# Ericonaldo/ILSwiss

Hardware: AMD Instinct MI355X
Metric: env-steps/s + SAC grad-steps/s, Hopper-v2 4096 envs (higher is better)
Workload: dtype f32

## Files before the change

### ilswiss_amd/csrc/fwd_split_tile.inc

```
  constexpr bool FINS = FIN_CT > 0;
  constexpr int NTH = 4 * H / CS, NWV = NTH / 64, NC = H / 16, SLW = H / CS, NCS = SLW / 16;
  constexpr int NT0 = PH == 1 ? 1 : CS;
  constexpr int LDH = H + ILSX_LDS_PAD, LDSL = SLW + ILSX_LDS_PAD;
  constexpr int MT = 1;
  constexpr int MR = 16;
  static_assert(NCS == NWV, "one k16 chunk of the slice per wave in the head phase");
  const DevScalars* scal = GRP ? GP->scal : A.scal;
  const NetView& N = T.net;
  int KP = N.KP;
  if constexpr (FINS) XCH_PIN(KP);
  const int LDX = KP + ILSX_LDS_PAD, NO = N.NO, NCH0 = KP >> 4, NOT = (NO + 15) >> 4;
  float* xs = smem;
  float* h0 = xs + MR * LDX;
  float* hs = h0 + MR * LDH;
  float* red = hs + MR * LDSL;
  constexpr int RNT = 4;
  if (bx & ((1u << A.xs) - 1u)) return;
  if ((int)(bx >> A.xs) * (A.rt > 0 ? A.rt : 1) * MR >= A.rows) return;
  const int tid = threadIdx.x, lane = tid & 63, wave = tid >> 6, li = lane & 15, g = lane >> 4;
  const int rows = A.rows;
  const int RT = A.rt > 0 ? A.rt : 1;
  const bool lead = cs == 0;
  ILSX_STAMP(A.dbg, 0);

  const int ct0 = PH == 1 ? cs * NWV + wave : wave * CS;
  const float* w0p = N.base + N.off_W[0] + (size_t)ct0 * NCH0 * 256 + 4 * lane;
  constexpr int L0D = 8;
  float4 b0[NT0], b0first[NT0];
  float4 l0first[PH == 1 ? L0D : 1];
  float bias0[NT0];
  if constexpr (PH == 1) {
#pragma unroll
    for (int d = 0; d < L0D; ++d) l0first[d] = *reinterpret_cast<const float4*>(w0p + (size_t)(d < NCH0 ? d : 0) * 256);
  }
  if constexpr (PH != 2) {
#pragma unroll
    for (int i = 0; i < NT0; ++i) b0[i] = *reinterpret_cast<const float4*>(w0p + (size_t)i * NCH0 * 256);
#pragma unroll
    for (int i = 0; i < NT0; ++i) b0first[i] = b0[i];
#pragma unroll
    for (int i = 0; i < NT0; ++i) bias0[i] = (N.base + N.off_b[0])[(ct0 + i) * 16 + li];
  }
  const int lc = wave * 16 + li, col1 = cs * SLW + lc;
  float bias1 = 0.0f;
  float4 whf[4];
  float4 wreg[NC];
  constexpr bool LATEW = GRP == 3 && PH == 0;
  if constexpr (PH != 1) {
    bias1 = (N.base + N.off_b[1])[col1];
#pragma unroll
    for (int t = 0; t < 4; ++t) {
      const int j = 16 * t + li;
      whf[t] = (t < NOT && j < NO) ? *reinterpret_cast<const float4*>(N.base + N.off_Wh + (size_t)j * H + cs * SLW + 16 * wave + 4 * g)
                                   : make_float4(0.f, 0.f, 0.f, 0.f);
    }
    if constexpr (!LATEW) {
      const float* wp = N.base + N.off_W[1] + (size_t)(cs * NWV + wave) * NC * 256 + 4 * lane;
#pragma unroll
      for (int c = 0; c < NC; ++c) wreg[c] = *reinterpret_cast<const float4*>(wp + 256 * c);
    }
  }
#ifdef XCH_FINE_DBG
  ILSX_STAMP_SYNC(XCH_FINE_DBG, 6);
#endif
  const bool fin = FIN_CT >= 0 && (GRP ? GP->fin_on : A.fin_on) != 0 && !T.no_fin && T.d1 > 0;
  const GatherSpec& G = GRP ? GP->gather : A.gather;
  for (int rt = 0; rt < RT; ++rt) {
  const int r0 = ((bx >> A.xs) * RT + rt) * MR;
  if (r0 >= rows) break;
  const bool full_tile = r0 + MR <= rows;
  bool fin_logp = false;
  int sf_a = 0; float* sf_logp = nullptr;
  if constexpr (PH != 2) {
#pragma unroll
  for (int i = 0; i < NT0; ++i) b0[i] = b0first[i];
  if constexpr (FINS) {
    static_assert(PH == 0 && GRP == 0 && XCH, "the static epilogue is phase A's target-critic stage");
    const PolicyFinishArgs& FP = A.fin;
    const bool pub = lead && first_task;
    int sf_d0 = T.d0, sf_s0 = T.s0, sf_ps = FP.part_stride;
    const float* sf_x0 = T.x0; const float* sf_part = FP.part; float* sf_xsave = lead ? T.xsave : nullptr;
    float* sf_raw = pub ? FP.raw : nullptr; float* sf_action = pub ? FP.action : nullptr; float* sf_epss = pub ? FP.eps_save : nullptr;
    sf_a = FP.a; sf_logp = pub ? FP.logp : nullptr;
    XCH_PIN(sf_d0); XCH_PIN(sf_s0); XCH_PIN(sf_ps); XCH_PIN(sf_x0); XCH_PIN(sf_part); XCH_PIN(sf_xsave);
    XCH_PIN(sf_raw); XCH_PIN(sf_action); XCH_PIN(sf_epss); XCH_PIN(sf_a); XCH_PIN(sf_logp);
    const int a = sf_a, NOp = 2 * a;
    const int fr = tid / a, fj = tid - fr * a, fgr = r0 + fr;
    const bool fon = tid < MR * a && fgr < rows;
    float fep = 0.0f;
    if (fon) {
      const unsigned long long fstep = FP.scal ? (FP.use_gather_step ? FP.scal->gather_step : FP.scal->step) : FP.step_host;
      float z4[4];
      philox_normal4(FP.seed, fstep, FP.rng_stream, fgr, fj >> 2, z4);
      const int q = fj & 3;
      fep = q == 0 ? z4[0] : q == 1 ? z4[1] : q == 2 ? z4[2] : z4[3];
    }
    constexpr int STG = 2;
    int sr[STG], sk[STG];
#pragma unroll
    for (int t = 0; t < STG; ++t) { const int e = tid + t * NTH; sr[t] = e / KP; sk[t] = e - sr[t] * KP; }
    XCH_HOOK_STAGE
    {
      float sv[STG];
#pragma unroll
      for (int t = 0; t < STG; ++t) {
        const int gr = r0 + sr[t];
        sv[t] = (tid + t * NTH < MR * KP && gr < rows && sk[t] < sf_d0) ? xg<true>(sf_x0)[(size_t)gr * sf_s0 + sk[t]] : 0.0f;
      }
      float pm[4], pl[4];
#pragma unroll
      for (int c = 0; c < 4; ++c) {
        const size_t at = ((size_t)(c < CS ? c : 0) * sf_ps + (fon ? fgr : r0)) * NOp + fj;
        pm[c] = fon ? ldx<XCH>(xg<true>(sf_part + at)) : 0.0f;
        pl[c] = fon ? ldx<XCH>(xg<true>(sf_part + at + a)) : 0.0f;
      }
#pragma unroll
      for (int t = 0; t < STG; ++t) {
        const int gr = r0 + sr[t];
        const bool act_col = sk[t] >= sf_d0 && sk[t] < sf_d0 + a;
        if (tid + t * NTH < MR * KP && !act_col) {
          if (sf_xsave && gr < rows) xg<true>(sf_xsave)[(size_t)gr * KP + sk[t]] = sv[t];
          xs[sr[t] * LDX + sk[t]] = sv[t];
        }
      }
      for (int e = tid + STG * NTH; e < MR * KP; e += NTH) {
        const int r = e / KP, k = e - r * KP, gr = r0 + r;
        if (k >= sf_d0 && k < sf_d0 + a) continue;
        float v = 0.0f;
        if (gr < rows) {
          if (k < sf_d0) v = xg<true>(sf_x0)[(size_t)gr * sf_s0 + k];
          if (sf_xsave) xg<true>(sf_xsave)[(size_t)gr * KP + k] = v;
        }
        xs[r * LDX + k] = v;
      }
      float* lp3 = red;
      float act = 0.0f, c0 = 0.0f, c1 = 0.0f, c2 = 0.0f;
      if (fon) {
        float mu = 0.f, lsr = 0.f;
#pragma unroll
        for (int c = 0; c < 4; ++c) { mu += c < CS ? pm[c] : 0.0f; lsr += c < CS ? pl[c] : 0.0f; }
        const float ls = fminf(fmaxf(lsr, LOG_SIG_MIN), LOG_SIG_MAX);
        const float sd = expf(ls);
        const float z = fep * sd + mu;
        act = tanhf(z);
        const float dm = mu - z;
        c0 = dm * dm / expf(2.0f * ls); c1 = ls; c2 = logf(1.0f - act * act + TANH_EPS);
        if (sf_raw) { stx<XCH>(xg<true>(sf_raw + (size_t)fgr * NOp + fj), mu); stx<XCH>(xg<true>(sf_raw + (size_t)fgr * NOp + a + fj), lsr); }
        if (sf_xsave) xg<true>(sf_xsave)[(size_t)fgr * KP + sf_d0 + fj] = act;
        if (sf_action) stx<XCH>(xg<true>(sf_action + (size_t)fgr * a + fj), act);
        if (sf_epss) stx<XCH>(xg<true>(sf_epss + (size_t)fgr * a + fj), fep);
      }
      if (tid < MR * a) {
        xs[fr * LDX + sf_d0 + fj] = act;
        lp3[(fr * 32 + fj) * 3 + 0] = c0; lp3[(fr * 32 + fj) * 3 + 1] = c1; lp3[(fr * 32 + fj) * 3 + 2] = c2;
      }
      fin_logp = sf_logp != nullptr;
    }
  } else {
  XCH_HOOK_STAGE
  if constexpr (PH == 0) {
    long long* ridx0 = reinterpret_cast<long long*>(hs);
    if constexpr (GRP != 0) {
      if (G.on) {
        if (tid < MR) ridx0[tid] = r0 + tid < rows ? replay_draw(G.seed, scal->gather_step, G.stream, (uint32_t)(r0 + tid), G.st->size) : 0;
        lds_barrier();
      }
    }
    for (int e = tid; e < MR * KP; e += NTH) {
      const int r = e / KP, k = e - r * KP, gr = r0 + r;
      const bool act_col = k >= T.d0 && k < T.d0 + T.d1;
      if (fin && act_col) continue;
      float v = 0.0f;
      if (gr < rows) {
        if (G.on) {
          long long idx;
          if constexpr (GRP != 0) idx = ridx0[r];
          else idx = replay_draw(G.seed, scal->gather_step, G.stream, (uint32_t)gr, G.st->size);
          const float* rec = G.records + (size_t)idx * G.rec;
          if (k < T.d0) v = rec[T.g0_off + k];
          else if (act_col) v = rec[T.g1_off + (k - T.d0)];
          if (lead && T.publish == 1) {
            if (k < T.d0) G.s[(size_t)gr * G.o + k] = v;
            else if (act_col) G.a[(size_t)gr * G.adim + (k - T.d0)] = v;
            if (k == 0) { stx<XCH>(G.r + gr, rec[G.o + G.adim]); stx<XCH>(G.d + gr, rec[G.o + G.adim + 1]); }
          } else if (lead && T.publish == 2 && k < T.d0) {
            G.s2[(size_t)gr * G.o + k] = v;
          }
        } else {
          if (k < T.d0) v = T.x0[(size_t)gr * T.s0 + k];
          else if (act_col) v = T.x1[(size_t)gr * T.s1 + (k - T.d0)];
        }
        if (T.xsave && lead) T.xsave[(size_t)gr * KP + k] = v;
      }
      xs[r * LDX + k] = v;
    }
  } else {
    auto stage = [&](int r, int k, int gr, const float* rec) {
      const bool act_col = k >= T.d0 && k < T.d0 + T.d1;
      if (fin && act_col) return;
      float v = 0.0f;
      if (gr < rows) {
        if (G.on) {
          if (k < T.d0) v = rec[T.g0_off + k];
          else if (act_col) v = rec[T.g1_off + (k - T.d0)];
          if (lead && T.publish == 1) {
            if (k < T.d0) G.s[(size_t)gr * G.o + k] = v;
            else if (act_col) G.a[(size_t)gr * G.adim + (k - T.d0)] = v;
            if (k == 0) { G.r[gr] = rec[G.o + G.adim]; G.d[gr] = rec[G.o + G.adim + 1]; }
          } else if (lead && T.publish == 2 && k < T.d0) {
            G.s2[(size_t)gr * G.o + k] = v;
          }
        } else {
          if (k < T.d0) v = T.x0[(size_t)gr * T.s0 + k];
          else if (act_col) v = T.x1[(size_t)gr * T.s1 + (k - T.d0)];
        }
        if (T.xsave && lead) T.xsave[(size_t)gr * KP + k] = v;
      }
      xs[r * LDX + k] = v;
    };
    long long* ridx = reinterpret_cast<long long*>(hs);
    if (G.on) {
      if (tid < MR) ridx[tid] = r0 + tid < rows ? replay_draw(G.seed, scal->gather_step, G.stream, (uint32_t)(r0 + tid), G.st->size) : 0;
      lds_barrier();
    }
    if (KP <= 512 && T.d1 <= 64) {
      constexpr int RW = 16 / NWV, U = 8;
      const bool acts = T.d1 > 0 && !fin;
#pragma unroll
      for (int mt = 0; mt < MT; ++mt) {
      float vo[RW][U], va[RW];
#pragma unroll
      for (int rr = 0; rr < RW; ++rr) {
        const int r = 16 * mt + wave + NWV * rr, grc = r0 + r < rows ? r0 + r : rows - 1;
        const float* rec = G.on ? G.records + (size_t)ridx[r] * G.rec : nullptr;
        const float* s0p = G.on ? rec + T.g0_off : T.x0 + (size_t)grc * T.s0;
#pragma unroll
        for (int u = 0; u < U; ++u) { const int k = lane + 64 * u; vo[rr][u] = s0p[k < T.d0 ? k : T.d0 - 1]; }
        va[rr] = 0.0f;
        if (acts) { const float* s1p = G.on ? rec + T.g1_off : T.x1 + (size_t)grc * T.s1; va[rr] = s1p[lane < T.d1 ? lane : T.d1 - 1]; }
      }
#pragma unroll
      for (int rr = 0; rr < RW; ++rr) {
        const int r = 16 * mt + wave + NWV * rr, gr = r0 + r;
// ... 65 lines not shown
            const int q = j & 3;
            ep = q == 0 ? z4[0] : q == 1 ? z4[1] : q == 2 ? z4[2] : z4[3];
          }
        }
        if (det) {
          act = P.max_act * (P.head == HEAD_DET_LIN_NOISE ? mu : tanhf(mu));
          if (P.noise != 0.0f) act += fminf(fmaxf(P.noise * ep, -P.noise_clip), P.noise_clip);
          if (pub && P.raw) stx<XCH>(P.raw + (size_t)gr * a + j, mu);
        } else {
          const float ls = fminf(fmaxf(lsr, LOG_SIG_MIN), LOG_SIG_MAX);
          const float sd = expf(ls);
          const float z = ep * sd + mu;
          act = tanhf(z);
          const float dm = mu - z;
          c0 = dm * dm / expf(2.0f * ls); c1 = ls; c2 = logf(1.0f - act * act + TANH_EPS);
          if (pub && P.raw) { stx<XCH>(P.raw + (size_t)gr * NOp + j, mu); stx<XCH>(P.raw + (size_t)gr * NOp + a + j, lsr); }
        }
        if (T.xsave && lead) T.xsave[(size_t)gr * KP + T.d0 + j] = act;
        if (pub) {
          if (P.action) stx<XCH>(P.action + (size_t)gr * a + j, act);
          if (P.eps_save) stx<XCH>(P.eps_save + (size_t)gr * a + j, ep);
        }
      }
      xs[row * LDX + T.d0 + j] = act;
      lp3[(row * LPS + j) * 3 + 0] = c0; lp3[(row * LPS + j) * 3 + 1] = c1; lp3[(row * LPS + j) * 3 + 2] = c2;
    }
    fin_logp = pub && P.logp && !det;
  }
  }
  }
  else {
    const float* hsrc = T.hsave[0];
    for (int e = tid; e < MR * (H / 4); e += NTH) {
      const int row = e / (H / 4), c4 = e - row * (H / 4), gr = r0 + row;
      const float4 v = gr < rows ? *reinterpret_cast<const float4*>(hsrc + (size_t)gr * H + 4 * c4) : make_float4(0.f, 0.f, 0.f, 0.f);
      *reinterpret_cast<float4*>(h0 + row * LDH + 4 * c4) = v;
    }
  }
  lds_barrier();
  XCH_STAMP(1);
  if (fin_logp && tid < MR && r0 + tid < rows) {
    const PolicyFinishArgs& P = GRP ? GP->fin : A.fin;
    float q = 0.f, l = 0.f, jc = 0.f;
    const int pa = FINS ? sf_a : P.a;
    constexpr int LPS = 32;
    for (int j = 0; j < pa; ++j) { q += red[(tid * LPS + j) * 3]; l += red[(tid * LPS + j) * 3 + 1]; jc += red[(tid * LPS + j) * 3 + 2]; }
    stx<XCH>(xg<FINS>((FINS ? sf_logp : P.logp) + r0 + tid), -0.5f * q - (l + HALF_LOG_2PI) - jc);
  }
  if constexpr (PH == 1) {
    f32x4 acc = (f32x4){0.f, 0.f, 0.f, 0.f};
    const float* ap = xs + li * LDX + 4 * g;
    float4 cur[L0D], nxt[L0D];
#pragma unroll
    for (int d = 0; d < L0D; ++d) cur[d] = l0first[d];
    for (int cb = 0; cb < NCH0; cb += L0D) {
#pragma unroll
      for (int d = 0; d < L0D; ++d) {
        const int c = cb + L0D + d;
        nxt[d] = *reinterpret_cast<const float4*>(w0p + (size_t)(c < NCH0 ? c : 0) * 256);
      }
#pragma unroll
      for (int d = 0; d < L0D; ++d) {
        if (cb + d < NCH0) {
          const float4 a = *reinterpret_cast<const float4*>(ap + 16 * (cb + d));
          acc = MFMA16(a.x, cur[d].x, acc); acc = MFMA16(a.y, cur[d].y, acc);
          acc = MFMA16(a.z, cur[d].z, acc); acc = MFMA16(a.w, cur[d].w, acc);
        }
      }
#pragma unroll
      for (int d = 0; d < L0D; ++d) cur[d] = nxt[d];
    }
    float* hsv = T.hsave[0];
    const int col = ct0 * 16 + li;
#pragma unroll
    for (int v = 0; v < 4; ++v) {
      const int row = 4 * g + v;
      if (r0 + row < rows) hsv[(size_t)(r0 + row) * H + col] = act_fn<ACT>(acc[v] + bias0[0]);
    }
  } else if constexpr (PH != 2) {
    f32x4 acc[NT0];
#pragma unroll
    for (int i = 0; i < NT0; ++i) acc[i] = (f32x4){0.f, 0.f, 0.f, 0.f};
    const float* ap = xs + li * LDX + 4 * g;
    for (int kc = 0; kc < KP; kc += 16) {
      float4 bn[NT0];
#pragma unroll
      for (int i = 0; i < NT0; ++i) {
        bn[i] = b0[i];
        if (kc + 16 < KP) bn[i] = *reinterpret_cast<const float4*>(w0p + (size_t)i * NCH0 * 256 + (kc + 16) * 16);
      }
      const float4 a = *reinterpret_cast<const float4*>(ap + kc);
#pragma unroll
      for (int i = 0; i < NT0; ++i) acc[i] = MFMA16(a.x, b0[i].x, acc[i]);
#pragma unroll
      for (int i = 0; i < NT0; ++i) acc[i] = MFMA16(a.y, b0[i].y, acc[i]);
#pragma unroll
      for (int i = 0; i < NT0; ++i) acc[i] = MFMA16(a.z, b0[i].z, acc[i]);
#pragma unroll
      for (int i = 0; i < NT0; ++i) acc[i] = MFMA16(a.w, b0[i].w, acc[i]);
#pragma unroll
      for (int i = 0; i < NT0; ++i) b0[i] = bn[i];
    }
    float* hsv = (PH == 1 || lead) ? T.hsave[0] : nullptr;
    float* const hrow = hsv ? hsv + (size_t)(r0 + 4 * g) * H + ct0 * 16 + li : nullptr;
#pragma unroll
    for (int i = 0; i < NT0; ++i) {
      const int col = (ct0 + i) * 16 + li;
#pragma unroll
      for (int v = 0; v < 4; ++v) {
        const int row = 4 * g + v;
        const float h = act_fn<ACT>(acc[i][v] + bias0[i]);
        if constexpr (PH == 0) h0[row * LDH + col] = h;
        acc[i][v] = h;
      }
    }
    if (hsv) {
      if (full_tile) {
#pragma unroll
        for (int i = 0; i < NT0; ++i)
#pragma unroll
          for (int v = 0; v < 4; ++v) stx<XCH>(hrow + v * H + i * 16, acc[i][v]);
      } else {
#pragma unroll
        for (int i = 0; i < NT0; ++i)
#pragma unroll
          for (int v = 0; v < 4; ++v)
            if (r0 + 4 * g + v < rows) stx<XCH>(hrow + v * H + i * 16, acc[i][v]);
      }
    }
  }
  if constexpr (PH == 1) {
    lds_barrier();
    continue;
  }
  if constexpr (PH == 0) lds_barrier();
  XCH_STAMP(2);
  if constexpr (LATEW) {
    const float* wp = N.base + N.off_W[1] + (size_t)(cs * NWV + wave) * NC * 256 + 4 * lane;
#pragma unroll
    for (int c = 0; c < NC; ++c) wreg[c] = *reinterpret_cast<const float4*>(wp + 256 * c);
  }
  {
    f32x4 acc0[MT], acc1[MT];
#pragma unroll
    for (int m = 0; m < MT; ++m) { acc0[m] = (f32x4){0.f, 0.f, 0.f, 0.f}; acc1[m] = acc0[m]; }
    const float* ap = h0 + li * LDH + 4 * g;
#pragma unroll
    for (int c = 0; c < NC; ++c) {
#pragma unroll
      for (int m = 0; m < MT; ++m) {
        const float4 a = *reinterpret_cast<const float4*>(ap + m * 16 * LDH + 16 * c);
        acc0[m] = MFMA16(a.x, wreg[c].x, acc0[m]); acc1[m] = MFMA16(a.y, wreg[c].y, acc1[m]);
        acc0[m] = MFMA16(a.z, wreg[c].z, acc0[m]); acc1[m] = MFMA16(a.w, wreg[c].w, acc1[m]);
      }
    }
    float* hsv = T.hsave[1];
#pragma unroll
    for (int m = 0; m < MT; ++m) {
      float* const hrow = hsv ? hsv + (size_t)(r0 + 16 * m + 4 * g) * H + col1 : nullptr;
#pragma unroll
      for (int v = 0; v < 4; ++v) {
        const int row = 16 * m + 4 * g + v;
        const float h = act_fn<ACT>(acc0[m][v] + acc1[m][v] + bias1);
        hs[row * LDSL + lc] = h;
        acc0[m][v] = h;
      }
      if (hsv) {
        if (full_tile) {
#pragma unroll
          for (int v = 0; v < 4; ++v) stx<XCH>(hrow + v * H, acc0[m][v]);
        } else {
#pragma unroll
          for (int v = 0; v < 4; ++v)
            if (r0 + 16 * m + 4 * g + v < rows) stx<XCH>(hrow + v * H, acc0[m][v]);
        }
      }
    }
  }
  lds_barrier();
  XCH_STAMP(3);
#pragma unroll
  for (int m = 0; m < MT; ++m) {
    const float4 a = *reinterpret_cast<const float4*>(hs + (16 * m + li) * LDSL + 16 * wave + 4 * g);
#pragma unroll
    for (int t = 0; t < 4; ++t) {
      if (t < NOT) {
        f32x4 acc = (f32x4){0.f, 0.f, 0.f, 0.f};
        acc = MFMA16(a.x, whf[t].x, acc); acc = MFMA16(a.y, whf[t].y, acc);
        acc = MFMA16(a.z, whf[t].z, acc); acc = MFMA16(a.w, whf[t].w, acc);
#pragma unroll
        for (int v = 0; v < 4; ++v) red[(((m * RNT + t) * NWV + wave) * 4 + v) * 64 + lane] = acc[v];
      }
    }
  }
  lds_barrier();
  const float* bh = N.base + N.off_bh;
#pragma unroll
  for (int m = 0; m < MT; ++m)
  for (int e = tid; e < NOT * 256; e += NTH) {
    const int t = e >> 8, v = (e >> 6) & 3, ol = e & 63;
    float sum = 0.0f;
#pragma unroll
    for (int w2 = 0; w2 < NWV; ++w2) sum += red[(((m * RNT + t) * NWV + w2) * 4 + v) * 64 + ol];
    const int row = 16 * m + 4 * (ol >> 4) + v, j = 16 * t + (ol & 15), gr = r0 + row;
    if (j < NO && gr < rows) stx<XCH>(T.part + ((size_t)cs * A.part_stride + gr) * NO + j, sum + (lead ? bh[j] : 0.0f));
  }
  lds_barrier();
  }
  ILSX_STAMP(A.dbg, 7);
```

### ilswiss_amd/csrc/host_common.h

```cpp
#pragma once
#include <hip/hip_runtime.h>
#include <hip/hip_ext.h>

#include <cstdarg>
#include <cstdio>
#include <cstring>
#include <deque>
#include <string>
#include <utility>
#include <vector>

#include "../../include/ilsx.h"
#include "dev_owner.h"
#include "kernels.h"

#define ILSX_FAIL(code, ...)   \
  do {                         \
    ilsx_set_err(__VA_ARGS__); \
    return (code);             \
  } while (0)

#define HIPCHK(expr)                                                                              \
  do {                                                                                            \
    hipError_t e_ = (expr);                                                                       \
// ... 33 lines not shown
  bool prof_on = false;
  struct ProfRec { int kid; hipEvent_t a, b; };
  std::vector<ProfRec> prof_pending;
  std::vector<hipEvent_t> prof_free;
  double prof_ms[ILSX_K_COUNT] = {0};
  uint64_t prof_n[ILSX_K_COUNT] = {0};
  const char* prof_name[ILSX_K_COUNT] = {nullptr};
};

struct ProfScope {
  ilsx_ctx* c; int kid; hipEvent_t a = nullptr, b = nullptr; bool launched = false;
  ProfScope(ilsx_ctx* ctx, int k);
  ~ProfScope();
};
#define ILSX_LAUNCH(ps, kernel, grid, block, lds, stream, ...)                                            \
  do {                                                                                                    \
    if ((ps).a) {                                                                                         \
      (ps).c->prof_name[(ps).kid] = #kernel; (ps).launched = true;                                        \
      hipExtLaunchKernelGGL(kernel, grid, block, lds, stream, (ps).a, (ps).b, 0, __VA_ARGS__);            \
    } else {                                                                                              \
      hipLaunchKernelGGL(kernel, grid, block, lds, stream, __VA_ARGS__);                                  \
    }                                                                                                     \
  } while (0)

int comm_allreduce_sum(ilsx_ctx* c, float* buf, size_t n);
int ctx_stage(ilsx_ctx* c, size_t bytes, void** out);

struct NetLayout {
  ilsx_mlp_cfg cfg;
  int KP = 0, NO = 0;
  int off_W[ILSX_MAX_HID], off_Wb[ILSX_MAX_HID], off_b[ILSX_MAX_HID], ld[ILSX_MAX_HID];
  int off_Wh = 0, off_bh = 0;
  size_t n_int = 0;
  size_t n_flat = 0;
  int hl[ILSX_MAX_HID] = {0, 0, 0};
  int out_of(int l) const { return hl[l] > 0 ? hl[l] : cfg.hidden; }
  int in_of(int l) const { return l == 0 ? cfg.in_dim : out_of(l - 1); }
};
int net_layout_build(const ilsx_mlp_cfg& cfg, NetLayout* L);
void net_flat_to_internal(const NetLayout& L, const float* flat, float* internal);
void net_internal_to_flat(const NetLayout& L, const float* internal, float* flat);
NetView net_view(const NetLayout& L, float* base);

struct ilsx_net {
  ilsx_ctx* ctx = nullptr;
  NetLayout lay;
  float* base = nullptr;
  bool owns = true;
  float* ws_out = nullptr;
  int ws_rows = 0;
  bool noise_policy = false;
  float noise = 0.f, noise_clip = 0.f, max_act = 1.f;
  bool out_linear = false;
  bool categorical = false;
  bool egreedy = false;
  float epsilon = 0.f;
  bool discrete() const { return categorical || egreedy; }
};
int launch_categorical_act(ilsx_ctx* ctx, const float* z, int rows, int n, int deterministic, unsigned long long step, float* act, float* logp);
int launch_egreedy_act(ilsx_ctx* ctx, const float* z, int rows, int n, int deterministic, float epsilon, unsigned long long step, float* act);

int net_adopt(ilsx_net* n, float* arena);
void net_give_back(ilsx_net* n);

int net_upload_flat(ilsx_ctx* ctx, const NetLayout& L, float* dev_base, const float* src, size_t n, int src_is_device);
int net_download_flat(ilsx_ctx* ctx, const NetLayout& L, const float* dev_base, float* dst, size_t n, int dst_is_device);

int launch_fwd(ilsx_ctx* ctx, const FwdArgs& A, int H, int act, int KP, int cs = 1);
int launch_bwd_dx(ilsx_ctx* ctx, const BwdArgs& A, int H, int act, int cs = 1);
int launch_policy_finish(ilsx_ctx* ctx, const PolicyFinishArgs& P);
bool phase_fits(ilsx_ctx* ctx, int rows, int H, int cs, int ntasks, bool own_rows = false);
bool phase_own_rows(ilsx_ctx* ctx, int rows, int H, int cs, int ntasks);
struct PhaseConst {
  int slot = -1, device = 0;
  bool tried = false, valid_a = false, valid_c = false;
  unsigned long long key_a = 0, key_c = 0;
  PhaseAArgs a; PhaseCArgs c;
};
int phase_const_alloc(int device);
void phase_const_prepare(ilsx_ctx* ctx, PhaseConst* ct);
void phase_const_free(int device, int slot);
bool phase_a_static_ok(const PhaseAArgs& P, int H, int cs);
bool phase_c_static_ok(const PhaseCArgs& P, int H, int cs);
int launch_phase_a(ilsx_ctx* ctx, const PhaseAArgs& P, int H, int act, int KPmax, int cs, PhaseConst* ct = nullptr, unsigned long long key = 0, bool upload_only = false);
int launch_phase_c(ilsx_ctx* ctx, const PhaseCArgs& P, int H, int act, int KPmax, int cs, PhaseConst* ct = nullptr, unsigned long long key = 0, bool upload_only = false);
int device_cus(ilsx_ctx* ctx);
int grp_const_alloc(int device, bool fwd, int n, int* base);
void grp_const_free(int device, bool fwd, int base);
int grp_const_upload(ilsx_ctx* ctx, bool fwd, int base, const void* host_records, size_t count);
struct ilsx_sac;
int sac_staged_batch(ilsx_sac* s, int B, float** obs, float** act, float** rew, float** done, float** nobs);
int sac_step_staged(ilsx_sac* s, ilsx_sac_stats* stats);
int sac_dims(const ilsx_sac* s, int* o, int* a);
int sac_window_begin(ilsx_sac* s, int B);
int sac_window_step(ilsx_sac* s);
int sac_window_end(ilsx_sac* s, bool teardown = false);
#define ILSX_RETRY_WINDOW (-1000)
int sac_snapshot_take(ilsx_sac* s);
int sac_snapshot_restore(ilsx_sac* s);
bool sac_window_may_use_phase(ilsx_sac* s, int B);
int mlp2_split_factor(int n_hidden, int H);
int launch_bwd_dw(ilsx_ctx* ctx, DevOwner& owner, const DwArgs& table, int rows, const AdamFuse* fuse = nullptr);
int dw_table_add(DwArgs* T, const float* A, int lda, int NA, const float* Bm, int ldb, int NB, float* dW, float* dWb, int ldw,
                 float* db, int mode, int rows = 0, int bias_rows = 0);
int launch_adam(ilsx_ctx* ctx, const AdamArgs& A);
int build_dw_jobs(const NetLayout& L, float* gbase, const float* xsave, float* const* hsave,
                  float* const* dsave, const float* dhead, DwArgs* table);

struct ilsx_replay {
  ilsx_ctx* ctx = nullptr;
  int64_t cap = 0;
  int o = 0, a = 0, rec = 0;
  float* data = nullptr;
  DevReplayState* dstate = nullptr;
  bool dstate_stale = false;
  uint64_t seed = 0;
  uint32_t rng_stream = 0;
  unsigned long long sample_ctr = 0;
  int64_t top = 0, size = 0, cur_start = 0;
  std::deque<std::pair<int64_t, int64_t>> trajs;
  std::vector<uint8_t> start_flag;
};
int replay_flush_state(ilsx_replay* rb);
int replay_advance_device_rows(ilsx_replay* rb, int n);
int replay_insert_paths(ilsx_replay* rb, const float* stage, int stage_len, const int* envs, const int* lens, const uint8_t* last_terminal,
                        int n_paths);
int replay_launch_sample(ilsx_replay* rb, int B, const int64_t* idx, const DevScalars* scal,
                         unsigned long long step_host, float* obs, float* act, float* rew, float* done,
                         float* nobs, int64_t* idx_out);
```

### ilswiss_amd/csrc/ilsx_core.hip

```cpp
#include <algorithm>
#include <cmath>
#include <cstdlib>
#include <random>

#define ILSX_KERNEL_IMPL 1
#include <mutex>
#include "host_common.h"

static thread_local std::string g_err = "";

void ilsx_set_err(const char* fmt, ...) {
  char buf[1024];
  va_list ap;
  va_start(ap, fmt);
  vsnprintf(buf, sizeof buf, fmt, ap);
  va_end(ap);
  g_err = buf;
}

static int kernels_init_once();
extern "C" int ilsx_abi_version(void) { return ILSX_ABI_VERSION; }
extern "C" const char* ilsx_last_error(void) { return g_err.c_str(); }

int ctx_alloc(ilsx_ctx* c, size_t bytes, void** out, bool zero) {
// ... 382 lines not shown
  if (cs > 1) {
    const size_t lds = fwd_split_lds_bytes(H, KPmax, cs);
    if (lds > 160 * 1024) ILSX_FAIL(ILSX_ERR_UNSUPPORTED, "forward tile needs %zu B of LDS (> 160 KiB)", lds);
    A.xs = ctx->xcd_shift;
    if (A.rt <= 0) A.rt = (A.tasks && ctx->rt_grouped > 0) ? ctx->rt_grouped : ctx->rt_single;
    const int tiles = (A.rows + 15) / 16;
    dim3 grid(((((tiles + A.rt - 1) / A.rt) + 7) & ~7) << A.xs, A.ntasks, cs), block(4 * H / cs);
    if (A.tail_mode) { if (!A.tail || A.tail_n < 1 || A.tail_n > (int)(grid.x * grid.z)) ILSX_FAIL(ILSX_ERR_ARG, "deferred tail: bad record table"); grid.y += 1; }
    if (A.late < 0) A.late = (long)tiles * A.ntasks * cs > 2L * device_cus(ctx);
    if (H == 256 && cs == 4 && A.l0_split) {
      FwdArgs A2 = A;
      A2.tail_mode = 0; A2.tail = nullptr; A2.tail_n = 0; A2.dbg = ctx->dbg_next();
      dim3 grid2(grid.x, A.ntasks, cs);
#define L0_CALL(AA, GG) do { ILSX_LAUNCH(ps, (k_mlp2_fwd_split<256, AA, 4, GG, 1>), grid, block, lds, ctx->stream, A); \
                             ILSX_LAUNCH(ps, (k_mlp2_fwd_split<256, AA, 4, GG, 2>), grid2, block, lds, ctx->stream, A2); } while (0)
      const int gg = A.tasks ? (A.ctab ? 2 : 1) : 0;
      if (act == ILSX_ACT_RELU) { if (gg == 2) L0_CALL(ACT_RELU, 2); else if (gg == 1) L0_CALL(ACT_RELU, 1); else L0_CALL(ACT_RELU, 0); }
      else { if (gg == 2) L0_CALL(ACT_TANH, 2); else if (gg == 1) L0_CALL(ACT_TANH, 1); else L0_CALL(ACT_TANH, 0); }
#undef L0_CALL
    } else if (H == 256 && cs == 4) {
#define FWD_GRP_CALL(HH, AA, CC) do { if (A.tasks && A.ctab && A.late) ILSX_LAUNCH(ps, (k_mlp2_fwd_split<HH, AA, CC, 3>), grid, block, lds, ctx->stream, A); \
        else if (A.tasks && A.ctab) ILSX_LAUNCH(ps, (k_mlp2_fwd_split<HH, AA, CC, 2>), grid, block, lds, ctx->stream, A); \
        else if (A.tasks) ILSX_LAUNCH(ps, (k_mlp2_fwd_split<HH, AA, CC, 1>), grid, block, lds, ctx->stream, A); \
        else ILSX_LAUNCH(ps, (k_mlp2_fwd_split<HH, AA, CC, 0>), grid, block, lds, ctx->stream, A); } while (0)
      if (act == ILSX_ACT_RELU) FWD_GRP_CALL(256, ACT_RELU, 4); else FWD_GRP_CALL(256, ACT_TANH, 4);
    } else if (H == 128 && cs == 2) {
      if (act == ILSX_ACT_RELU) FWD_GRP_CALL(128, ACT_RELU, 2); else FWD_GRP_CALL(128, ACT_TANH, 2);
#undef FWD_GRP_CALL
    } else {
      ILSX_FAIL(ILSX_ERR_UNSUPPORTED, "no column-split forward kernel for H=%d cs=%d", H, cs);
    }
    HIPCHK(hipGetLastError());
    return ILSX_OK;
  }
  const size_t lds = fwd_lds_bytes(H, KPmax);
  if (lds > 160 * 1024) ILSX_FAIL(ILSX_ERR_UNSUPPORTED, "forward tile needs %zu B of LDS (> 160 KiB)", lds);
  dim3 grid((A.rows + 15) / 16, A.ntasks), block(4 * H);
#define CALL_FWD(HH, AA) ILSX_LAUNCH(ps, (k_mlp_fwd<HH, AA>), grid, block, lds, ctx->stream, A)
  DISPATCH_H_ACT(H, act, CALL_FWD);
#undef CALL_FWD
  HIPCHK(hipGetLastError());
  return ILSX_OK;
}

int device_cus(ilsx_ctx* ctx) {
  static int n_cu = 0;
  if (!n_cu) {
    hipDeviceProp_t pr;
    n_cu = hipGetDeviceProperties(&pr, ctx->device) == hipSuccess ? pr.multiProcessorCount : 1;
  }
  return n_cu;
}
static size_t phase_lds_bytes(int H, int KP, int cs) { return std::max(fwd_split_lds_bytes(H, KP, cs), bwd_split_lds_bytes(H, cs)); }
void phase_wgs_per_cu(int H, int cs, int* occ_a, int* occ_c) {
  static int oa[2] = {-1, -1}, oc[2] = {-1, -1};
  const int i = H == 256 ? 0 : 1;
  if (oa[i] < 0) {
    int a = 0, c = 0;
    const size_t lds = phase_lds_bytes(H, 32, cs);
    hipError_t e1, e2;
    if (H == 256) { e1 = hipOccupancyMaxActiveBlocksPerMultiprocessor(&a, (const void*)k_sac_phase_a<256, ACT_RELU, 4>, 4 * H / cs, lds);
                    e2 = hipOccupancyMaxActiveBlocksPerMultiprocessor(&c, (const void*)k_sac_phase_c<256, ACT_RELU, 4>, 4 * H / cs, lds); }
    else { e1 = hipOccupancyMaxActiveBlocksPerMultiprocessor(&a, (const void*)k_sac_phase_a<128, ACT_RELU, 2>, 4 * H / cs, lds);
           e2 = hipOccupancyMaxActiveBlocksPerMultiprocessor(&c, (const void*)k_sac_phase_c<128, ACT_RELU, 2>, 4 * H / cs, lds); }
    oa[i] = e1 == hipSuccess ? std::max(a, 1) : 1;
    oc[i] = e2 == hipSuccess ? std::max(c, 1) : 1;
  }
  *occ_a = oa[i]; *occ_c = oc[i];
}
bool phase_fits(ilsx_ctx* ctx, int rows, int H, int cs, int ntasks, bool own_rows) {
  const int n_cu = device_cus(ctx);
  if (!((H == 256 && cs == 4) || (H == 128 && cs == 2))) return false;
  const int tiles = (rows + 15) / 16, work = tiles * ntasks * cs;
  int occ_a = 1, occ_c = 1;
  phase_wgs_per_cu(H, cs, &occ_a, &occ_c);
  const int work_a = work + (own_rows ? tiles * 2 * cs : 0);
  return tiles <= PHASE_MAX_TILES && work <= n_cu && work_a + 1 <= occ_a * n_cu && tiles * 3 * cs <= occ_c * n_cu;
}
bool phase_own_rows(ilsx_ctx* ctx, int rows, int H, int cs, int ntasks) {
  const char* e = getenv("ILSX_PHASE_OWN_ROWS");
  return !(e && atoi(e) == 0) && phase_fits(ctx, rows, H, cs, ntasks, true);
}

static std::vector<bool> g_phase_slots[16];
static std::mutex g_phase_slots_mu;
int phase_const_alloc(int device) {
  static const bool off = []() { const char* e = getenv("ILSX_PHASE_CT"); return e && atoi(e) == 0; }();
  if (off || device < 0 || device >= 16) return -1;
  std::lock_guard<std::mutex> lock(g_phase_slots_mu);
  auto& u = g_phase_slots[device];
  if (u.empty()) u.assign(PHASE_CONST_SLOTS, false);
  for (int i = 0; i < PHASE_CONST_SLOTS; ++i) if (!u[i]) { u[i] = true; return i; }
  return -1;
}
void phase_const_free(int device, int slot) {
  if (device < 0 || device >= 16 || slot < 0 || slot >= PHASE_CONST_SLOTS) return;
  std::lock_guard<std::mutex> lock(g_phase_slots_mu);
  if (!g_phase_slots[device].empty()) g_phase_slots[device][slot] = false;
}
void phase_const_prepare(ilsx_ctx* ctx, PhaseConst* ct) {
  if (!ct || ct->tried) return;
  ct->tried = true;
  ct->device = ctx->device;
  ct->slot = phase_const_alloc(ctx->device);
  if (ct->slot >= 0) ctx->phase_slots.push_back(ct->slot);
}
template <class Blk>
static bool phase_const_ready(ilsx_ctx* ctx, PhaseConst* ct, const Blk& blk, unsigned long long key, Blk& held, bool& valid, unsigned long long& held_key,
                              const void* symbol) {
  phase_const_prepare(ctx, ct);
  if (!ct || ct->slot < 0 || blk.dbg || !key) return false;
  if (valid && held_key == key) return true;
  hipStreamCaptureStatus cap = hipStreamCaptureStatusNone;
  if (hipStreamIsCapturing(ctx->stream, &cap) != hipSuccess || cap != hipStreamCaptureStatusNone) return false;
  if (hipStreamSynchronize(ctx->stream) != hipSuccess) return false;
  valid = false;
  memcpy(&held, &blk, sizeof blk);
  if (hipMemcpyToSymbolAsync(symbol, &held, sizeof blk, (size_t)ct->slot * sizeof blk, hipMemcpyHostToDevice, ctx->stream) != hipSuccess ||
      hipStreamSynchronize(ctx->stream) != hipSuccess) { (void)hipGetLastError(); return false; }
  valid = true; held_key = key;
  return true;
}

bool phase_a_static_ok(const PhaseAArgs& P, int H, int cs) {
  const int nth = 4 * H / cs;
  for (int i = 0; i < 2; ++i) {
    const BwdTask& t = P.b1.t[i];
    if (t.loss != LOSS_SAC_CRITIC || t.net.NO != 1 || t.q.cs != cs || t.tq1.cs != cs || t.tq2.cs != cs) return false;
  }
  if (P.f1.fin_on) return false;
  const FwdArgs& f = P.f2;
  if (f.gather.on || !f.fin_on || f.fin.head != HEAD_TANH_SAMPLE || f.fin.cs != cs || f.fin.a < 1 || 16 * f.fin.a > nth) return false;
  if (f.fin.scal && !f.fin.use_gather_step) return false;
  if (f.fin.eps || P.fin_pi.eps) return false;
  for (int i = 0; i < 2; ++i) {
    const FwdTask& t = f.t[i];
    if (t.no_fin || t.d1 != f.fin.a || !t.x0) return false;
  }
  return true;
}
bool phase_c_static_ok(const PhaseCArgs& P, int H, int cs) {
  (void)H;
  if (P.f3.fin_on) return false;
  for (int i = 0; i < 2; ++i) {
    const BwdTask& t = P.b2.t[i];
    if (t.loss != LOSS_SAC_ACTORQ || t.net.NO != 1 || t.q1n.cs != cs || t.q2n.cs != cs) return false;
  }
  const BwdTask& t = P.b3.t[0];
  return t.loss == LOSS_SAC_POLICY && t.net.NO >= 2 && t.net.NO % 2 == 0 && P.b3.ga_parts == cs;
}
extern "C" int ilsx_debug_phase_static_ok(int stage, int loss_critic, int loss_policy, int no_critic, int slabs, int fin_head, int a, int H, int cs, int flags) {
  if (stage == 0) {
    PhaseAArgs P; memset(&P, 0, sizeof P);
    static const float x = 0.0f;
    for (int i = 0; i < 2; ++i) {
      BwdTask& t = P.b1.t[i];
      t.loss = loss_critic; t.net.NO = no_critic; t.q.cs = t.tq1.cs = t.tq2.cs = slabs;
      P.f2.t[i].d1 = a; P.f2.t[i].x0 = &x;
    }
    P.f2.fin_on = 1; P.f2.fin.head = fin_head; P.f2.fin.cs = slabs; P.f2.fin.a = a;
    if (flags & 1) P.f2.fin.eps = &x;
    return phase_a_static_ok(P, H, cs) ? 1 : 0;
  }
  PhaseCArgs P; memset(&P, 0, sizeof P);
  for (int i = 0; i < 2; ++i) { BwdTask& t = P.b2.t[i]; t.loss = loss_critic; t.net.NO = no_critic; t.q1n.cs = t.q2n.cs = slabs; }
  P.b3.t[0].loss = loss_policy; P.b3.t[0].net.NO = 2 * a; P.b3.ga_parts = slabs;
  if (flags & 2) P.f3.fin_on = 1;
  return phase_c_static_ok(P, H, cs) ? 1 : 0;
}

int launch_phase_a(ilsx_ctx* ctx, const PhaseAArgs& P0, int H, int act, int KPmax, int cs, PhaseConst* ct, unsigned long long key, bool upload_only) {
  PhaseAArgs P = P0;
  P.f1.xs = P.f2.xs = P.b1.xs = 0; P.f1.rt = P.f2.rt = 1;
  P.f1.dbg = P.f2.dbg = nullptr; P.b1.dbg = nullptr;
  P.dbg = upload_only ? nullptr : ctx->dbg_next();
  if (P.b1.ga_parts < 1) P.b1.ga_parts = 1;
  if (!phase_a_static_ok(P, H, cs)) ILSX_FAIL(ILSX_ERR_UNSUPPORTED, "launch_phase_a: the stages' descriptors are not what the phase kernel is compiled for (loss kind, head, slab count)");
  const int tiles = (P.f1.rows + 15) / 16;
  dim3 grid((tiles + 7) & ~7, P.own_rows ? 7 : 5, cs), block(4 * H / cs);
  const size_t lds = phase_lds_bytes(H, KPmax, cs);
  const bool use_ct = ct && phase_const_ready(ctx, ct, P, key, ct->a, ct->valid_a, ct->key_a, HIP_SYMBOL(g_phase_a_tab));
  if (upload_only) return ILSX_OK;
  const int slot = use_ct ? ct->slot : 0;
  static const bool trace = getenv("ILSX_PHASE_CT_TRACE") != nullptr;
  if (trace) { hipStreamCaptureStatus cap = hipStreamCaptureStatusNone; hipStreamIsCapturing(ctx->stream, &cap);
               fprintf(stderr, "launch_phase_a: %s, slot %d, capturing %d\n", use_ct ? "constant table" : "kernel arguments", ct ? ct->slot : -9, (int)cap); }
  ProfScope ps(ctx, ILSX_K_SAC_PHASE_A);
#define PHASE_A(HH, AA, CC) do { if (use_ct) ILSX_LAUNCH(ps, (k_sac_phase_a<HH, AA, CC, true>), grid, block, lds, ctx->stream, P, slot); \
                                 else ILSX_LAUNCH(ps, (k_sac_phase_a<HH, AA, CC>), grid, block, lds, ctx->stream, P, slot); } while (0)
  if (H == 256 && act == ILSX_ACT_RELU) PHASE_A(256, ACT_RELU, 4);
  else if (H == 256) PHASE_A(256, ACT_TANH, 4);
  else if (act == ILSX_ACT_RELU) PHASE_A(128, ACT_RELU, 2);
  else PHASE_A(128, ACT_TANH, 2);
#undef PHASE_A
  HIPCHK(hipGetLastError());
  return ILSX_OK;
}

int launch_phase_c(ilsx_ctx* ctx, const PhaseCArgs& P0, int H, int act, int KPmax, int cs, PhaseConst* ct, unsigned long long key, bool upload_only) {
  PhaseCArgs P = P0;
  P.f3.xs = P.b2.xs = P.b3.xs = 0; P.f3.rt = 1;
  P.f3.dbg = nullptr; P.b2.dbg = P.b3.dbg = nullptr;
  P.dbg = upload_only ? nullptr : ctx->dbg_next();
  if (P.b2.ga_parts < 1) P.b2.ga_parts = 1;
  if (P.b3.ga_parts < 1) P.b3.ga_parts = 1;
  if (!phase_c_static_ok(P, H, cs)) ILSX_FAIL(ILSX_ERR_UNSUPPORTED, "launch_phase_c: the stages' descriptors are not what the phase kernel is compiled for (loss kind, head, slab count)");
  const int tiles = (P.f3.rows + 15) / 16;
  dim3 grid((tiles + 7) & ~7, 4, cs), block(4 * H / cs);
  const size_t lds = phase_lds_bytes(H, KPmax, cs);
  const bool use_ct = ct && phase_const_ready(ctx, ct, P, key, ct->c, ct->valid_c, ct->key_c, HIP_SYMBOL(g_phase_c_tab));
  if (upload_only) return ILSX_OK;
  const int slot = use_ct ? ct->slot : 0;
  ProfScope ps(ctx, ILSX_K_SAC_PHASE_C);
#define PHASE_C(HH, AA, CC) do { if (use_ct) ILSX_LAUNCH(ps, (k_sac_phase_c<HH, AA, CC, true>), grid, block, lds, ctx->stream, P, slot); \
                                 else ILSX_LAUNCH(ps, (k_sac_phase_c<HH, AA, CC>), grid, block, lds, ctx->stream, P, slot); } while (0)
  if (H == 256 && act == ILSX_ACT_RELU) PHASE_C(256, ACT_RELU, 4);
  else if (H == 256) PHASE_C(256, ACT_TANH, 4);
  else if (act == ILSX_ACT_RELU) PHASE_C(128, ACT_RELU, 2);
  else PHASE_C(128, ACT_TANH, 2);
#undef PHASE_C
  HIPCHK(hipGetLastError());
  return ILSX_OK;
}

int launch_bwd_dx(ilsx_ctx* ctx, const BwdArgs& A0, int H, int act, int cs) {
  if (A0.rows <= 0) return ILSX_OK;
  BwdArgs A = A0;
  A.dbg = ctx->dbg_next();
  if (A.ga_parts < 1) A.ga_parts = 1;
  ProfScope ps(ctx, ILSX_K_MLP_BWD_DX);
  if (cs > 1) {
    const size_t lds = bwd_split_lds_bytes(H, cs);
    A.xs = ctx->xcd_shift;
    dim3 grid(((((A.rows + 15) / 16) + 7) & ~7) << A.xs, A.ntasks, cs), block(4 * H / cs);
    if (A.late < 0) A.late = (long)((A.rows + 15) / 16) * A.ntasks * cs > 2L * device_cus(ctx);
    if (H == 256 && cs == 4) {
#define BWD_GRP_CALL(HH, AA, CC) do { if (A.tasks && A.ctab && A.late) ILSX_LAUNCH(ps, (k_mlp2_bwd_split<HH, AA, CC, 3>), grid, block, lds, ctx->stream, A); \
        else if (A.tasks && A.ctab) ILSX_LAUNCH(ps, (k_mlp2_bwd_split<HH, AA, CC, 2>), grid, block, lds, ctx->stream, A); \
        else if (A.tasks) ILSX_LAUNCH(ps, (k_mlp2_bwd_split<HH, AA, CC, 1>), grid, block, lds, ctx->stream, A); \
        else ILSX_LAUNCH(ps, (k_mlp2_bwd_split<HH, AA, CC, 0>), grid, block, lds, ctx->stream, A); } while (0)
      if (act == ILSX_ACT_RELU) BWD_GRP_CALL(256, ACT_RELU, 4); else BWD_GRP_CALL(256, ACT_TANH, 4);
    } else if (H == 128 && cs == 2) {
      if (act == ILSX_ACT_RELU) BWD_GRP_CALL(128, ACT_RELU, 2); else BWD_GRP_CALL(128, ACT_TANH, 2);
#undef BWD_GRP_CALL
    } else {
      ILSX_FAIL(ILSX_ERR_UNSUPPORTED, "no column-split backward kernel for H=%d cs=%d", H, cs);
    }
    HIPCHK(hipGetLastError());
    return ILSX_OK;
  }
  const size_t lds = bwd_lds_bytes(H);
  dim3 grid((A.rows + 15) / 16, A.ntasks), block(4 * H);
#define CALL_BWD(HH, AA) ILSX_LAUNCH(ps, (k_mlp_bwd_dx<HH, AA>), grid, block, lds, ctx->stream, A)
  DISPATCH_H_ACT(H, act, CALL_BWD);
#undef CALL_BWD
  HIPCHK(hipGetLastError());
  return ILSX_OK;
}

int launch_policy_finish(ilsx_ctx* ctx, const PolicyFinishArgs& P) {
  if (P.rows <= 0) return ILSX_OK;
  ProfScope ps(ctx, ILSX_K_POLICY_FINISH);
  ILSX_LAUNCH(ps, k_policy_finish, dim3((P.rows + 63) / 64), dim3(64), 0, ctx->stream, P);
  HIPCHK(hipGetLastError());
  return ILSX_OK;
}

void dw_split_plan(int rows, bool big, int* splits, int* rows_per_split) {
  const int unit = big ? DWB_RC : 128, cap = big ? 64 : 32;
  int s = rows / 512;
  if (s > cap) s = cap;
  if (s < 1) s = 1;
  const int rps = ((rows + s - 1) / s + unit - 1) / unit * unit;
  *rows_per_split = rps;
  *splits = (rows + rps - 1) / rps;
}
extern "C" int ilsx_debug_dw_split(int rows, int big, int* splits, int* rows_per_split) {
  if (rows < 1 || !splits || !rows_per_split) ILSX_FAIL(ILSX_ERR_ARG, "ilsx_debug_dw_split: bad argument");
  dw_split_plan(rows, big != 0, splits, rows_per_split);
  return ILSX_OK;
}

int launch_bwd_dw(ilsx_ctx* ctx, DevOwner& owner, const DwArgs& table, int rows, const AdamFuse* fuse) {
  if (table.ntiles <= 0 || rows <= 0) return ILSX_OK;
  DwArgs D = table;
  D.rows_all = rows;
  memset(&D.F, 0, sizeof D.F);
  if (fuse) D.F = *fuse;
  D.dbg = ctx->dbg_next();
  D.xs = ctx->xcd_shift;
  D.splits = 1; D.rows_per_split = rows; D.scratch = nullptr; D.span = 0;
  bool stacked = false;
  for (int i = 0; i < D.nmat && !D.gtiles; ++i) stacked = stacked || D.m[i].rows > 0;
  if (rows >= DW_SPLIT_MIN_ROWS && D.g_lo && !stacked) {
    static const int big_env = []() { const char* e = getenv("ILSX_DW_BIG"); return e ? atoi(e) : 1; }();
    const bool big = big_env && rows >= DW_BIG_MIN_ROWS;
    int splits, rps;
    dw_split_plan(rows, big, &splits, &rps);
// ... 328 lines not shown
```

### ilswiss_amd/csrc/ilsx_sac.hip

```cpp
#include <cmath>
#include <cstdlib>

#include <algorithm>
#include "host_common.h"

enum { W_PI = 0, W_Q1 = 1, W_Q2 = 2, W_TQ1 = 3, W_TQ2 = 4 };

struct SacWs {
  float *s, *a, *r, *d, *s2, *eps1, *eps2;
  float *a2, *logp2, *q1, *q2, *tq1, *tq2;
  float *xq[2], *hq[2][ILSX_MAX_HID], *dq[2][ILSX_MAX_HID], *dhq[2];
  float *raw, *an, *logp, *epss, *q1n, *q2n, *ga[2];
  float *xp, *hp[ILSX_MAX_HID], *dp[ILSX_MAX_HID], *dhp;
  float* ppart;
  float* ppart2;
};

struct StatsArgs {
  PartVal q1, q2, tq1, tq2, q1n, q2n;
  const float *logp2, *r, *d, *logp, *raw;
  int B, a;
  float gamma, reward_scale, w_mu, w_std, target_entropy, inv_B;
  DevScalars* scal;
  float* alpha_grad_slot;
  int slot_given;
};

struct SacTailItem { StatsArgs S; int train_alpha; float lr, b1, b2, eps, qf_lr, policy_lr; };
struct SacLaunch {
  int kind;
  FwdArgs f; int KP; BwdArgs b; DwArgs d; AdamFuse F; SacTailItem t;
};
struct SacCollector { std::vector<SacLaunch> L; };

struct ilsx_sac {
  ilsx_ctx* ctx = nullptr;
  DevOwner own;
  SacCollector* col = nullptr;
  ilsx_sac_cfg cfg;
  ilsx_net *pi = nullptr, *q1 = nullptr, *q2 = nullptr;
  NetLayout Lq, Lp;
  int o = 0, a = 0;
  size_t nq = 0, np = 0;
  void* slab = nullptr;
  float *P = nullptr, *G = nullptr, *M = nullptr, *V = nullptr;
  DevScalars* scal = nullptr;
  SacWs ws;
  DwArgs jobs_q, jobs_p;
  ilsx_replay* gather_rb = nullptr;
  bool fuse_now = false;
  int cs = 1;
  float* h0scr = nullptr;
  int B = 0;
  bool eps_explicit = false;
  float target_entropy = 0.f;
  uint32_t rng_stream = 0;
  hipGraphExec_t graph = nullptr;
  ilsx_replay* graph_rb = nullptr;
  int graph_B = 0;
  bool graph_defer = false, graph_phase = false, graph_own = false;
  bool defer_tail = false;
  TailLite* tail_dev = nullptr;
  int tail_B = 0;
  ilsx_sac_stats stats_cache; bool stats_cached = false;
  bool tail_split = false;
  unsigned* phase_flags = nullptr;
  int* phase_err = nullptr;
  PhaseConst pct;
  bool phase_args_only = false;
  bool phase_now = false;
  bool phase_broken = false;
  bool phase_last = false;
  bool debug_break = false;
  bool phase_check_only = false;
  int static_heads = -1;
  int phase_fallbacks = 0;
  float* vote = nullptr;
  bool snap_valid = false;
  void* snap = nullptr;
  size_t snap_bytes = 0;
  float* base(int which) const {
    switch (which) {
      case W_Q1: return P;
      case W_Q2: return P + nq;
      case W_PI: return P + 2 * nq;
      case W_TQ1: return P + 2 * nq + np;
      default: return P + 3 * nq + np;
    }
  }
  PartVal pv(const float* p) const { return PartVal{p, cs, cfg.max_batch}; }
  float* gbase(int which) const { return which == W_Q1 ? G : which == W_Q2 ? G + nq : G + 2 * nq; }
  size_t trainable_off(int which) const { return which == W_Q1 ? 0 : which == W_Q2 ? nq : 2 * nq; }
};


__device__ __forceinline__ void sac_alpha_grad_dev(const StatsArgs& S) {
  __shared__ float sh2[4];
  float lpe = 0.f;
  for (int r = threadIdx.x; r < S.B; r += 256) lpe += S.logp[r] + S.target_entropy;
  lpe = block256_sum(lpe, sh2);
  if (threadIdx.x == 0) {
    S.scal->alpha_used = S.scal->alpha;
    S.scal->log_alpha_used = S.scal->log_alpha;
    if (!S.slot_given) {
      S.alpha_grad_slot[0] = -lpe * S.inv_B;
      S.alpha_grad_slot[1] = 0.f; S.alpha_grad_slot[2] = 0.f; S.alpha_grad_slot[3] = 0.f;
    }
  }
}

__device__ __forceinline__ void sac_stats_dev(const StatsArgs& S) {
  __shared__ float sh[4];
  const float alpha = S.scal->alpha;
  float l1 = 0, l2 = 0, pl = 0, lp = 0, mu2 = 0, ls2 = 0, mus = 0, lss = 0, q1s = 0, q2s = 0, lpe = 0;
  float mx[5] = {-INFINITY, -INFINITY, -INFINITY, -INFINITY, -INFINITY}, mn[5] = {INFINITY, INFINITY, INFINITY, INFINITY, INFINITY};
  for (int r = threadIdx.x; r < S.B; r += 256) {
    const float y = S.reward_scale * S.r[r] +
                    (1.0f - S.d[r]) * S.gamma * (fminf(S.tq1.get(r), S.tq2.get(r)) - alpha * S.logp2[r]);
    const float q1v = S.q1.get(r), q2v = S.q2.get(r);
    const float e1 = q1v - y, e2 = q2v - y;
    l1 += e1 * e1; l2 += e2 * e2; q1s += q1v; q2s += q2v;
    mx[0] = fmaxf(mx[0], q1v); mn[0] = fminf(mn[0], q1v); mx[1] = fmaxf(mx[1], q2v); mn[1] = fminf(mn[1], q2v);
    mx[2] = fmaxf(mx[2], S.logp[r]); mn[2] = fminf(mn[2], S.logp[r]);
    pl += alpha * S.logp[r] - fminf(S.q1n.get(r), S.q2n.get(r));
    lp += S.logp[r];
    lpe += S.logp[r] + S.target_entropy;
    for (int j = 0; j < S.a; ++j) {
      const float mu = S.raw[(size_t)r * 2 * S.a + j];
      const float ls = fminf(fmaxf(S.raw[(size_t)r * 2 * S.a + S.a + j], LOG_SIG_MIN), LOG_SIG_MAX);
      mu2 += mu * mu; ls2 += ls * ls; mus += mu; lss += ls;
      mx[3] = fmaxf(mx[3], mu); mn[3] = fminf(mn[3], mu); mx[4] = fmaxf(mx[4], ls); mn[4] = fminf(mn[4], ls);
    }
  }
  l1 = block256_sum(l1, sh); l2 = block256_sum(l2, sh); pl = block256_sum(pl, sh); lp = block256_sum(lp, sh);
  mu2 = block256_sum(mu2, sh); ls2 = block256_sum(ls2, sh); mus = block256_sum(mus, sh); lss = block256_sum(lss, sh);
  q1s = block256_sum(q1s, sh); q2s = block256_sum(q2s, sh); lpe = block256_sum(lpe, sh);
#pragma unroll
  for (int i = 0; i < 5; ++i) {
    float a = mx[i], b = mn[i];
    for (int o = 32; o >= 1; o >>= 1) { a = fmaxf(a, __shfl_xor(a, o, 64)); b = fminf(b, __shfl_xor(b, o, 64)); }
    __syncthreads();
    if ((threadIdx.x & 63) == 0) sh[threadIdx.x >> 6] = a;
    __syncthreads();
// ... 12 lines not shown
    for (int j = 0; j < S.a; ++j) {
      const float dm = S.raw[(size_t)r * 2 * S.a + j] - means[3];
      const float dl = fminf(fmaxf(S.raw[(size_t)r * 2 * S.a + S.a + j], LOG_SIG_MIN), LOG_SIG_MAX) - means[4];
      cs[3] += dm * dm; cs[4] += dl * dl;
    }
  }
#pragma unroll
  for (int i = 0; i < 5; ++i) cs[i] = block256_sum(cs[i], sh);
  if (threadIdx.x == 0) {
    DevScalars* sc = S.scal;
    sc->qf1_loss = 0.5f * l1 * iB;
    sc->qf2_loss = 0.5f * l2 * iB;
    sc->policy_loss = pl * iB + S.w_mu * mu2 * iBa + S.w_std * ls2 * iBa;
    sc->alpha_loss = -(float)sc->log_alpha * (lpe * iB);
    sc->q1_mean = means[0]; sc->q2_mean = means[1]; sc->log_pi_mean = means[2];
    sc->mu_mean = means[3]; sc->log_std_mean = means[4];
    for (int i = 0; i < 5; ++i) {
      sc->ext_std[i] = sqrtf(cs[i] * (i < 3 ? iB : iBa));
      sc->ext_max[i] = mx[i]; sc->ext_min[i] = mn[i];
    }
    sc->alpha_used = alpha;
    sc->log_alpha_used = sc->log_alpha;
    if (!S.slot_given) {
      S.alpha_grad_slot[0] = -lpe * S.inv_B;
      S.alpha_grad_slot[1] = 0.f; S.alpha_grad_slot[2] = 0.f; S.alpha_grad_slot[3] = 0.f;
    }
  }
}

__global__ __launch_bounds__(256) void k_sac_stats(const StatsArgs S) { sac_stats_dev(S); }

__global__ void k_sac_finish(DevScalars* sc, const float* alpha_grad_slot, int train_alpha, float lr, float b1,
                             float b2, float eps, float qf_lr, float policy_lr) {
  sac_finish_dev(sc, alpha_grad_slot, train_alpha, lr, b1, b2, eps, qf_lr, policy_lr, 0);
}
__global__ __launch_bounds__(256) void k_sac_tail(const StatsArgs S, int train_alpha, float lr, float b1, float b2,
                                                  float eps, float qf_lr, float policy_lr, int deferred) {
  if (S.scal->want_stats) sac_stats_dev(S);
  else sac_alpha_grad_dev(S);
  if (threadIdx.x == 0) S.scal->want_stats = 0;
  if (threadIdx.x == 0) {
    sac_finish_dev(S.scal, S.alpha_grad_slot, train_alpha, lr, b1, b2, eps, qf_lr, policy_lr, deferred);
  }
}

__global__ __launch_bounds__(256) void k_sac_tail_group(const SacTailItem* items, int deferred) {
  const SacTailItem& T = items[blockIdx.x];
  if (T.S.scal->want_stats) sac_stats_dev(T.S);
  else sac_alpha_grad_dev(T.S);
  if (threadIdx.x == 0) {
    T.S.scal->want_stats = 0;
    sac_finish_dev(T.S.scal, T.S.alpha_grad_slot, T.train_alpha, T.lr, T.b1, T.b2, T.eps, T.qf_lr, T.policy_lr, deferred);
  }
}

__global__ void k_sac_refresh_adam(DevScalars* sc, float qf_lr, float policy_lr, float b1, float b2) {
  adam_scalars(qf_lr, b1, b2, sc->t_q + 1, &sc->adam_q_step, &sc->adam_q_bc2s);
  adam_scalars(policy_lr, b1, b2, sc->t_pi + 1, &sc->adam_pi_step, &sc->adam_pi_bc2s);
}
static int sac_refresh_adam(struct ilsx_sac* s);

static void sac_plan_ws(ilsx_sac* s, Slab& L) {
  const size_t B = (size_t)s->cfg.max_batch;
  const int o = s->o, a = s->a, H = s->Lq.cfg.hidden;
  SacWs& w = s->ws;
  auto A = [&](float** p, size_t n) { L.add(p, n); };
  A(&w.s, B * o); A(&w.a, B * a); A(&w.r, B); A(&w.d, B);
  A(&w.s2, B * o); A(&w.eps1, B * a); A(&w.eps2, B * a);
  const size_t CS = (size_t)s->cs;
  A(&w.a2, B * a); A(&w.logp2, B); A(&w.q1, CS * B); A(&w.q2, CS * B);
  A(&w.tq1, CS * B); A(&w.tq2, CS * B); A(&w.ppart, CS * B * 2 * a);
  A(&w.ppart2, CS * B * 2 * a);
  for (int i = 0; i < 2; ++i) {
    A(&w.xq[i], B * s->Lq.KP);
    for (int l = 0; l < s->Lq.cfg.n_hidden; ++l) { A(&w.hq[i][l], B * H); A(&w.dq[i][l], B * H); }
    A(&w.dhq[i], B * 4);
    A(&w.ga[i], CS * B * a);
  }
  A(&w.raw, B * 2 * a); A(&w.an, B * a); A(&w.logp, B); A(&w.epss, B * a);
  A(&w.q1n, CS * B); A(&w.q2n, CS * B);
  A(&w.xp, B * s->Lp.KP);
  for (int l = 0; l < s->Lp.cfg.n_hidden; ++l) { A(&w.hp[l], B * H); A(&w.dp[l], B * H); }
  A(&w.dhp, B * 2 * a);
  const char* e = getenv("ILSX_L0_SPLIT_KP");
  const int thr = e ? atoi(e) : 65;
  if (s->cs == 4 && H == 256 && std::max(s->Lq.KP, s->Lp.KP) >= thr) A(&s->h0scr, 4 * B * H);
}

static int sac_setup(ilsx_sac* s) {
  ilsx_net *pi = s->pi, *q1 = s->q1, *q2 = s->q2;
  hipStream_t st = s->ctx->stream;
  HIPCHK(hipMemcpyAsync(s->base(W_Q1), q1->base, s->nq * 4, hipMemcpyDeviceToDevice, st));
  HIPCHK(hipMemcpyAsync(s->base(W_Q2), q2->base, s->nq * 4, hipMemcpyDeviceToDevice, st));
  HIPCHK(hipMemcpyAsync(s->base(W_PI), pi->base, s->np * 4, hipMemcpyDeviceToDevice, st));
  HIPCHK(hipMemcpyAsync(s->base(W_TQ1), q1->base, s->nq * 4, hipMemcpyDeviceToDevice, st));
  HIPCHK(hipMemcpyAsync(s->base(W_TQ2), q2->base, s->nq * 4, hipMemcpyDeviceToDevice, st));
  HIPCHK(hipStreamSynchronize(st));
  ilsx_net* nets[3] = {pi, q1, q2};
  const int wh[3] = {W_PI, W_Q1, W_Q2};
  for (int i = 0; i < 3; ++i) ILSX_TRY(net_adopt(nets[i], s->base(wh[i])));
  DevScalars h;
  memset(&h, 0, sizeof h);
  h.log_alpha = std::log((double)s->cfg.alpha);
  h.alpha = (float)std::exp(h.log_alpha);
  h.alpha_used = h.alpha;
  h.log_alpha_used = h.log_alpha;
  HIPCHK(hipMemcpyAsync(s->scal, &h, sizeof h, hipMemcpyHostToDevice, st));
  HIPCHK(hipStreamSynchronize(st));
  ILSX_TRY(sac_refresh_adam(s));
  memset(&s->jobs_q, 0, sizeof s->jobs_q);
  memset(&s->jobs_p, 0, sizeof s->jobs_p);
  for (int i = 0; i < 2; ++i)
    ILSX_TRY(build_dw_jobs(s->Lq, s->gbase(i == 0 ? W_Q1 : W_Q2), s->ws.xq[i], s->ws.hq[i], s->ws.dq[i], s->ws.dhq[i], &s->jobs_q));
  ILSX_TRY(build_dw_jobs(s->Lp, s->gbase(W_PI), s->ws.xp, s->ws.hp, s->ws.dp, s->ws.dhp, &s->jobs_p));
  s->jobs_q.zero_flags = s->phase_flags;
  s->jobs_p.zero_flags = s->phase_flags;
  s->jobs_q.zero_err = s->phase_err; s->jobs_p.zero_err = s->phase_err;
  return ILSX_OK;
}

extern "C" int ilsx_sac_create(ilsx_ctx* ctx, const ilsx_sac_cfg* cfg, ilsx_net* pi, ilsx_net* q1, ilsx_net* q2,
                               ilsx_sac** out) {
  if (!ctx || !cfg || !pi || !q1 || !q2 || !out) ILSX_FAIL(ILSX_ERR_ARG, "ilsx_sac_create: NULL argument");
  if (pi->ctx != ctx || q1->ctx != ctx || q2->ctx != ctx) ILSX_FAIL(ILSX_ERR_ARG, "ilsx_sac_create: nets belong to another ctx");
  const ilsx_mlp_cfg &cp = pi->lay.cfg, &c1 = q1->lay.cfg, &c2 = q2->lay.cfg;
  if (cp.n_heads != 2) ILSX_FAIL(ILSX_ERR_ARG, "policy must have 2 heads (mean | log_std), policies.py:231-239");
  if (c1.n_heads != 1 || c1.out_dim != 1 || memcmp(&c1, &c2, sizeof c1) != 0)
    ILSX_FAIL(ILSX_ERR_ARG, "qf1/qf2 must be identical single-output FlattenMlp's");
  if (c1.in_dim != cp.in_dim + cp.out_dim) ILSX_FAIL(ILSX_ERR_ARG, "qf input %d != obs %d + act %d", c1.in_dim, cp.in_dim, cp.out_dim);
  if (c1.hidden != cp.hidden || c1.n_hidden != cp.n_hidden || c1.act != cp.act)
    ILSX_FAIL(ILSX_ERR_UNSUPPORTED, "policy and critics must share hidden width/depth/activation");
  if (!pi->owns || !q1->owns || !q2->owns) ILSX_FAIL(ILSX_ERR_STATE, "a network already belongs to an agent");
  if (cfg->max_batch < 1 || cfg->max_batch > (1 << 20)) ILSX_FAIL(ILSX_ERR_ARG, "max_batch=%d out of range", cfg->max_batch);
  HIPCHK(hipSetDevice(ctx->device));
  ilsx_sac* s = new ilsx_sac();
  s->ctx = s->own.ctx = ctx; s->cfg = *cfg; s->pi = pi; s->q1 = q1; s->q2 = q2;
  if (s->cfg.grad_world < 1) s->cfg.grad_world = 1;
  s->Lq = q1->lay; s->Lp = pi->lay;
  s->o = cp.in_dim; s->a = cp.out_dim;
  s->nq = s->Lq.n_int; s->np = s->Lp.n_int;
  s->cs = getenv("ILSX_NO_SPLIT") ? 1 : mlp2_split_factor(cp.n_hidden, cp.hidden);
  s->target_entropy = cfg->has_target_entropy ? cfg->target_entropy : -(float)s->a / 2.0f;
  s->rng_stream = ctx->next_rng_stream;
  ctx->next_rng_stream += 2;
  const size_t nP = 4 * s->nq + s->np, nT = 2 * s->nq + s->np;
  Slab L;
  L.add(&s->scal, 1);
  L.add(&s->P, nP); L.add(&s->G, nT + 4); L.add(&s->M, nT); L.add(&s->V, nT);
  L.add(&s->phase_flags, (size_t)PHASE_FLAG_WORDS); L.add(&s->phase_err, 32);
  sac_plan_ws(s, L);
  int rc = s->own.commit(L, &s->slab);
  if (rc == ILSX_OK) rc = sac_setup(s);
  if (rc != ILSX_OK) { ilsx_sac_destroy(s); return rc; }
  *out = s;
  return ILSX_OK;
}

extern "C" int ilsx_sac_destroy(ilsx_sac* s) {
  if (!s) return ILSX_OK;
  hipSetDevice(s->ctx->device);
  hipStreamSynchronize(s->ctx->stream);
  if (s->graph) hipGraphExecDestroy(s->graph);
  if (s->pct.slot >= 0) {
    phase_const_free(s->pct.device, s->pct.slot);
    auto& v = s->ctx->phase_slots;
    v.erase(std::remove(v.begin(), v.end(), s->pct.slot), v.end());
// ... 1 lines not shown
  }
  for (ilsx_net* n : {s->pi, s->q1, s->q2}) net_give_back(n);
  s->own.release();
  delete s;
  return ILSX_OK;
}

static float sac_inv_B(const ilsx_sac* s) { return 1.0f / ((float)s->B * (float)s->cfg.grad_world); }

static void sac_policy_task(ilsx_sac* s, FwdTask& t, const float* obs, const float* eps, uint32_t stream, bool save,
                            float* action, float* logp, float* part) {
  const SacWs& w = s->ws;
  t.net = net_view(s->Lp, s->base(W_PI));
  t.x0 = obs; t.d0 = s->o; t.s0 = s->o;
  if (save) {
    t.xsave = w.xp;
    for (int l = 0; l < s->Lp.cfg.n_hidden; ++l) t.hsave[l] = w.hp[l];
  }
  t.head = HEAD_TANH_SAMPLE; t.rng_stream = stream;
  if (s->cs > 1) {
    t.part = part;
  } else {
    t.eps = eps; t.action = action; t.logp = logp;
    if (save) { t.out = w.raw; t.eps_save = w.epss; }
  }
}
static void sac_policy_fin(ilsx_sac* s, FwdArgs& A, const float* eps, uint32_t stream, bool save, float* action, float* logp,
                           const float* part) {
  if (s->cs == 1) return;
  const SacWs& w = s->ws;
  PolicyFinishArgs& P = A.fin;
  memset(&P, 0, sizeof P);
  P.part = part; P.cs = s->cs; P.part_stride = s->cfg.max_batch; P.rows = s->B; P.a = s->a;
  P.head = HEAD_TANH_SAMPLE; P.rng_stream = stream; P.seed = s->ctx->seed; P.scal = s->scal;
  P.eps = eps; P.action = action; P.logp = logp;
  if (save) { P.raw = w.raw; P.eps_save = w.epss; }
  A.fin_on = 1;
}
static void sac_q_task(ilsx_sac* s, FwdTask& q, int which, const float* obs, const float* act, float* out, bool save_x,
                       bool save_h, int i) {
  const SacWs& w = s->ws;
  q.net = net_view(s->Lq, s->base(which));
  q.x0 = obs; q.d0 = s->o; q.s0 = s->o; q.x1 = act; q.d1 = s->a; q.s1 = s->a;
  if (save_x) q.xsave = w.xq[i];
  if (save_h) for (int l = 0; l < s->Lq.cfg.n_hidden; ++l) q.hsave[l] = w.hq[i][l];
  q.head = HEAD_RAW;
  if (s->cs > 1) q.part = out; else q.out = out;
}

static int sac_fwd(ilsx_sac* s, const FwdArgs& A0, int H, int act, int KP, int cs) {
  FwdArgs A = A0;
  if (s->h0scr) {
    A.l0_split = 1;
    for (int t = 0; t < A.ntasks; ++t)
      if (!A.t[t].hsave[0]) A.t[t].hsave[0] = s->h0scr + (size_t)t * s->cfg.max_batch * H;
  }
  if (!s->col) return launch_fwd(s->ctx, A, H, act, KP, cs);
  SacLaunch l; memset(&l, 0, sizeof l); l.kind = 0; l.f = A; l.KP = KP;
  s->col->L.push_back(l);
  return ILSX_OK;
}
static int sac_bwd(ilsx_sac* s, const BwdArgs& A, int H, int act, int cs) {
  if (!s->col) return launch_bwd_dx(s->ctx, A, H, act, cs);
  SacLaunch l; memset(&l, 0, sizeof l); l.kind = 1; l.b = A;
  s->col->L.push_back(l);
  return ILSX_OK;
}
static int sac_dw(ilsx_sac* s, const DwArgs& table, int rows, const AdamFuse* F) {
  if (!s->col) return launch_bwd_dw(s->ctx, s->own, table, rows, F);
  SacLaunch l; memset(&l, 0, sizeof l); l.kind = 2; l.d = table; l.F = *F;
  s->col->L.push_back(l);
  return ILSX_OK;
}

static bool sac_own_rows(const ilsx_sac* s) { return phase_own_rows(s->ctx, s->B, s->Lq.cfg.hidden, s->cs, 4); }
static unsigned long long sac_phase_key(const ilsx_sac* s) {
  unsigned long long k = 1469598103934665603ull;
  auto mix = [&k](unsigned long long v) { k = (k ^ v) * 1099511628211ull; };
  const ilsx_replay* rb = s->gather_rb;
  mix((unsigned long long)(uintptr_t)rb); mix(rb ? (unsigned long long)(uintptr_t)rb->data : 0); mix(rb ? (unsigned long long)(uintptr_t)rb->dstate : 0);
  mix(rb ? (unsigned long long)rb->rec : 0); mix(rb ? (unsigned long long)rb->seed : 0); mix(rb ? (unsigned long long)rb->rng_stream : 0);
  mix((unsigned long long)s->B); mix(s->defer_tail ? 1 : 0); mix(s->eps_explicit ? 1 : 0); mix(s->fuse_now ? 1 : 0); mix((unsigned long long)s->cs);
  mix((unsigned long long)(uintptr_t)s->tail_dev); mix((unsigned long long)(uintptr_t)s->slab);
  mix(sac_own_rows(s) ? 1 : 0);
  return k ? k : 1;
}

static int sac_critic_backward(ilsx_sac* s) {
  const SacWs& w = s->ws;
  const int B = s->B, H = s->Lq.cfg.hidden, act = s->Lq.cfg.act, cs = s->cs;
  const float* eps1 = s->eps_explicit ? w.eps1 : nullptr;
  const float* eps2 = s->eps_explicit ? w.eps2 : nullptr;
  PhaseAArgs PA;
  if (s->phase_now) memset(&PA, 0, sizeof PA);
  {
    FwdArgs A;
    memset(&A, 0, sizeof A);
    A.rows = B; A.ntasks = 4; A.seed = s->ctx->seed; A.scal = s->scal; A.part_stride = s->cfg.max_batch;
    sac_policy_task(s, A.t[0], w.s2, eps1, s->rng_stream, false, w.a2, w.logp2, w.ppart);
    sac_policy_task(s, A.t[3], w.s, eps2, s->rng_stream + 1, true, w.an, w.logp, w.ppart2);
    sac_q_task(s, A.t[1], W_Q1, w.s, w.a, w.q1, true, true, 0);
    sac_q_task(s, A.t[2], W_Q2, w.s, w.a, w.q2, true, true, 1);
    if (s->gather_rb && cs > 1) {
      ilsx_replay* rb = s->gather_rb;
      GatherSpec& G = A.gather;
      G.records = rb->data; G.st = rb->dstate; G.rec = rb->rec; G.seed = rb->seed; G.stream = rb->rng_stream;
      G.o = s->o; G.adim = s->a; G.on = 1;
      G.s = w.s; G.a = w.a; G.r = w.r; G.d = w.d; G.s2 = w.s2;
      A.t[0].g0_off = s->o + s->a + 2; A.t[0].publish = 2;
      A.t[1].g0_off = 0; A.t[1].g1_off = s->o; A.t[1].publish = 1;
      A.t[2].g0_off = 0; A.t[2].g1_off = s->o; A.t[2].publish = 0;
      A.t[3].g0_off = 0; A.t[3].publish = 0;
    }
    if (s->defer_tail) { A.tail = s->tail_dev; A.tail_mode = 1; A.tail_n = 1; }
    if (s->phase_now) PA.f1 = A;
    else ILSX_TRY(sac_fwd(s, A, H, act, std::max(s->Lq.KP, s->Lp.KP), cs));
  }
  {
    FwdArgs A;
    memset(&A, 0, sizeof A);
    A.rows = B; A.ntasks = 2; A.seed = s->ctx->seed; A.scal = s->scal; A.part_stride = s->cfg.max_batch;
    sac_q_task(s, A.t[0], W_TQ1, w.s2, w.a2, w.tq1, false, false, 0);
    sac_q_task(s, A.t[1], W_TQ2, w.s2, w.a2, w.tq2, false, false, 1);
    sac_policy_fin(s, A, eps1, s->rng_stream, false, w.a2, w.logp2, w.ppart);
    if (s->defer_tail) { A.tail = s->tail_dev; A.tail_mode = 2; A.tail_n = 1; }
    if (s->phase_now) {
      A.fin.use_gather_step = 1;
      A.tail_mode = 0;
      PA.f2 = A;
    } else {
      ILSX_TRY(sac_fwd(s, A, H, act, s->Lq.KP, cs));
    }
  }
  {
    BwdArgs A;
    memset(&A, 0, sizeof A);
    A.rows = B; A.ntasks = 2; A.inv_B = sac_inv_B(s);
    A.gamma = s->cfg.discount; A.reward_scale = s->cfg.reward_scale; A.scal = s->scal;
    A.part_stride = s->cfg.max_batch;
    for (int i = 0; i < 2; ++i) {
      BwdTask& t = A.t[i];
      t.net = net_view(s->Lq, s->base(i == 0 ? W_Q1 : W_Q2));
      for (int l = 0; l < s->Lq.cfg.n_hidden; ++l) { t.hsave[l] = w.hq[i][l]; t.dsave[l] = w.dq[i][l]; }
      t.dhead = w.dhq[i];
      t.loss = LOSS_SAC_CRITIC;
      t.q = s->pv(i == 0 ? w.q1 : w.q2); t.tq1 = s->pv(w.tq1); t.tq2 = s->pv(w.tq2);
      t.logp_next = w.logp2; t.rew = w.r; t.done = w.d;
    }
    if (s->phase_now) {
      PA.b1 = A; PA.flags = s->phase_flags; PA.err = s->phase_err;
      PA.own_rows = sac_own_rows(s) ? 1 : 0;
      {
        FwdArgs Fz;
        memset(&Fz, 0, sizeof Fz);
        sac_policy_fin(s, Fz, eps2, s->rng_stream + 1, true, w.an, w.logp, w.ppart2);
        PA.fin_pi = Fz.fin; PA.fin_pi.use_gather_step = 1; PA.fin_pi_on = 1;
      }
      ILSX_TRY(launch_phase_a(s->ctx, PA, H, act, std::max(s->Lq.KP, s->Lp.KP), cs, s->phase_check_only ? nullptr : &s->pct, sac_phase_key(s), s->phase_args_only));
      if (s->phase_args_only) return ILSX_OK;
    } else {
      ILSX_TRY(sac_bwd(s, A, H, act, cs));
    }
  }
  AdamFuse F;
  memset(&F, 0, sizeof F);
  if (s->fuse_now) {
    F.on = 1; F.Gbase = s->G; F.P = s->P; F.M = s->M; F.V = s->V; F.T = s->base(W_TQ1);
    F.b1 = s->cfg.beta_1; F.b2 = 0.999f; F.eps = 1e-8f; F.tau = s->cfg.soft_target_tau;
    F.step_size = &s->scal->adam_q_step; F.bc2_sqrt = &s->scal->adam_q_bc2s;
    if (s->phase_now) F.T = nullptr;
  }
  return sac_dw(s, s->jobs_q, B, &F);
}

static int sac_critic_update(ilsx_sac* s) {
  if (s->fuse_now) return ILSX_OK;
  AdamArgs A;
  A.p = s->P; A.g = s->G; A.m = s->M; A.v = s->V; A.tgt = s->base(W_TQ1);
  A.n = (int)(2 * s->nq);
  A.b1 = s->cfg.beta_1; A.b2 = 0.999f; A.eps = 1e-8f; A.tau = s->cfg.soft_target_tau;
  A.step_size = &s->scal->adam_q_step; A.bc2_sqrt = &s->scal->adam_q_bc2s;
  return launch_adam(s->ctx, A);
}

static StatsArgs sac_stats_args(ilsx_sac* s);
static int sac_actor_backward(ilsx_sac* s) {
  const SacWs& w = s->ws;
  const int B = s->B, H = s->Lq.cfg.hidden, act = s->Lq.cfg.act, cs = s->cs;
  const float* eps2 = s->eps_explicit ? w.eps2 : nullptr;
  PhaseCArgs PC;
  if (s->phase_now) memset(&PC, 0, sizeof PC);
  {
    FwdArgs A;
    memset(&A, 0, sizeof A);
    A.rows = B; A.ntasks = 2; A.seed = s->ctx->seed; A.scal = s->scal; A.part_stride = s->cfg.max_batch;
    sac_q_task(s, A.t[0], W_Q1, w.s, w.an, w.q1n, false, true, 0);
    sac_q_task(s, A.t[1], W_Q2, w.s, w.an, w.q2n, false, true, 1);
    if (!s->phase_now) sac_policy_fin(s, A, eps2, s->rng_stream + 1, true, w.an, w.logp, w.ppart2);
    if (s->phase_now) { A.tail = s->tail_dev; PC.f3 = A; }
    else ILSX_TRY(sac_fwd(s, A, H, act, s->Lq.KP, cs));
  }
  {
    BwdArgs A;
    memset(&A, 0, sizeof A);
    A.rows = B; A.ntasks = 2; A.inv_B = sac_inv_B(s); A.scal = s->scal; A.part_stride = s->cfg.max_batch;
    for (int i = 0; i < 2; ++i) {
      BwdTask& t = A.t[i];
      t.net = net_view(s->Lq, s->base(i == 0 ? W_Q1 : W_Q2));
      for (int l = 0; l < s->Lq.cfg.n_hidden; ++l) t.hsave[l] = w.hq[i][l];
      t.loss = LOSS_SAC_ACTORQ; t.which = i; t.q1n = s->pv(w.q1n); t.q2n = s->pv(w.q2n);
      t.dx = w.ga[i]; t.dx_col0 = s->o; t.dx_cols = s->a;
    }
    if (s->phase_now) PC.b2 = A;
    else ILSX_TRY(sac_bwd(s, A, H, act, cs));
  }
  {
    BwdArgs A;
    memset(&A, 0, sizeof A);
    A.rows = B; A.ntasks = 1; A.inv_B = sac_inv_B(s); A.scal = s->scal; A.part_stride = s->cfg.max_batch;
    A.w_mu = s->cfg.policy_mean_reg_weight; A.w_std = s->cfg.policy_std_reg_weight;
    A.ga_parts = cs; A.ga_stride = s->cfg.max_batch;
    BwdTask& t = A.t[0];
    t.net = net_view(s->Lp, s->base(W_PI));
    for (int l = 0; l < s->Lp.cfg.n_hidden; ++l) { t.hsave[l] = w.hp[l]; t.dsave[l] = w.dp[l]; }
    t.dhead = w.dhp;
    t.loss = LOSS_SAC_POLICY;
    t.raw = w.raw; t.eps = w.epss; t.action = w.an; t.ga1 = w.ga[0]; t.ga2 = w.ga[1];
    if (s->phase_now) {
      PC.b3 = A; PC.flags = s->phase_flags; PC.err = s->phase_err;
      if (s->fuse_now) { PC.polyak_T = s->base(W_TQ1); PC.polyak_P = s->base(W_Q1); PC.polyak_n = (int)(2 * s->nq); PC.polyak_tau = s->cfg.soft_target_tau; }
      else {
        PC.aslot = s->G + 2 * s->nq + s->np; PC.aslot_logp = w.logp; PC.aslot_B = B; PC.aslot_te = s->target_entropy; PC.aslot_invB = sac_inv_B(s);
      }
      ILSX_TRY(launch_phase_c(s->ctx, PC, H, act, std::max(s->Lq.KP, s->Lp.KP), cs, s->phase_check_only ? nullptr : &s->pct, sac_phase_key(s), s->phase_args_only));
      if (s->phase_args_only) return ILSX_OK;
    } else {
      ILSX_TRY(sac_bwd(s, A, H, act, cs));
    }
  }
  {
    AdamFuse F;
    memset(&F, 0, sizeof F);
    if (s->fuse_now) {
      F.on = 1; F.Gbase = s->G; F.P = s->P; F.M = s->M; F.V = s->V; F.T = nullptr;
      F.b1 = s->cfg.beta_1; F.b2 = 0.999f; F.eps = 1e-8f; F.tau = 0.f;
      F.step_size = &s->scal->adam_pi_step; F.bc2_sqrt = &s->scal->adam_pi_bc2s;
    }
    ILSX_TRY(sac_dw(s, s->jobs_p, B, &F));
  }
  if (s->fuse_now) return ILSX_OK;
  if (s->phase_now && s->defer_tail) return ILSX_OK;
  StatsArgs S = sac_stats_args(s);
  ProfScope ps(s->ctx, ILSX_K_SAC_STATS);
  ILSX_LAUNCH(ps, k_sac_stats, dim3(1), dim3(256), 0, s->ctx->stream, S);
  HIPCHK(hipGetLastError());
  return ILSX_OK;
}

static StatsArgs sac_stats_args(ilsx_sac* s) {
  const SacWs& w = s->ws;
  const int B = s->B;
  StatsArgs S;
  S.q1 = s->pv(w.q1); S.q2 = s->pv(w.q2); S.tq1 = s->pv(w.tq1); S.tq2 = s->pv(w.tq2);
  S.q1n = s->pv(w.q1n); S.q2n = s->pv(w.q2n);
  S.logp2 = w.logp2; S.r = w.r; S.d = w.d; S.logp = w.logp; S.raw = w.raw;
  S.B = B; S.a = s->a;
  S.gamma = s->cfg.discount; S.reward_scale = s->cfg.reward_scale;
  S.w_mu = s->cfg.policy_mean_reg_weight; S.w_std = s->cfg.policy_std_reg_weight;
  S.target_entropy = s->target_entropy; S.inv_B = sac_inv_B(s);
  S.scal = s->scal; S.alpha_grad_slot = s->G + 2 * s->nq + s->np;
  S.slot_given = 0;
  return S;
}

static int sac_actor_update(ilsx_sac* s) {
  AdamArgs A;
  const size_t off = 2 * s->nq;
  A.p = s->P + off; A.g = s->G + off; A.m = s->M + off; A.v = s->V + off; A.tgt = nullptr;
  A.n = (int)s->np;
  A.b1 = s->cfg.beta_1; A.b2 = 0.999f; A.eps = 1e-8f; A.tau = 0.f;
  A.step_size = &s->scal->adam_pi_step; A.bc2_sqrt = &s->scal->adam_pi_bc2s;
  if (s->fuse_now && s->col) {
    SacLaunch l; memset(&l, 0, sizeof l); l.kind = 3;
    l.t.S = sac_stats_args(s); l.t.train_alpha = s->cfg.train_alpha; l.t.lr = s->cfg.alpha_lr; l.t.b1 = s->cfg.beta_1;
    l.t.b2 = 0.999f; l.t.eps = 1e-8f; l.t.qf_lr = s->cfg.qf_lr; l.t.policy_lr = s->cfg.policy_lr;
    s->col->L.push_back(l);
    return ILSX_OK;
  }
  if (s->fuse_now && s->defer_tail) return ILSX_OK;
  if (s->fuse_now) {
    ProfScope ps(s->ctx, ILSX_K_SAC_FINISH);
    ILSX_LAUNCH(ps, k_sac_tail, dim3(1), dim3(256), 0, s->ctx->stream, sac_stats_args(s), s->cfg.train_alpha,
                       s->cfg.alpha_lr, s->cfg.beta_1, 0.999f, 1e-8f, s->cfg.qf_lr, s->cfg.policy_lr, 0);
    HIPCHK(hipGetLastError());
    return ILSX_OK;
  }
  ILSX_TRY(launch_adam(s->ctx, A));
  if (s->phase_now && s->defer_tail) return ILSX_OK;
  ProfScope ps(s->ctx, ILSX_K_SAC_FINISH);
  ILSX_LAUNCH(ps, k_sac_finish, dim3(1), dim3(1), 0, s->ctx->stream, s->scal, (const float*)(s->G + 2 * s->nq + s->np),
                     s->cfg.train_alpha, s->cfg.alpha_lr, s->cfg.beta_1, 0.999f, 1e-8f, s->cfg.qf_lr, s->cfg.policy_lr);
  HIPCHK(hipGetLastError());
  return ILSX_OK;
}

static int sac_refresh_adam(ilsx_sac* s) {
  hipLaunchKernelGGL(k_sac_refresh_adam, dim3(1), dim3(1), 0, s->ctx->stream, s->scal, s->cfg.qf_lr, s->cfg.policy_lr,
                     s->cfg.beta_1, 0.999f);
  HIPCHK(hipGetLastError());
  return ILSX_OK;
}

static bool sac_is_split(const ilsx_sac* s);
static TailLite sac_tail_lite(ilsx_sac* s, int B) {
  TailLite t;
  memset(&t, 0, sizeof t);
  const int keep = s->B;
  s->B = B;
  t.logp = s->ws.logp; t.B = B; t.target_entropy = s->target_entropy; t.inv_B = sac_inv_B(s);
  s->B = keep;
  t.alpha_grad_slot = s->G + 2 * s->nq + s->np; t.scal = s->scal;
  t.train_alpha = s->cfg.train_alpha; t.lr = s->cfg.alpha_lr; t.b1 = s->cfg.beta_1; t.b2 = 0.999f; t.eps = 1e-8f;
  t.qf_lr = s->cfg.qf_lr; t.policy_lr = s->cfg.policy_lr;
  t.slot_given = sac_is_split(s) ? 1 : 0;
  return t;
}
static int sac_split_on_phase(ilsx_sac* s, int B, bool* on) {
  const bool mine = getenv("ILSX_SPLIT_NO_PHASE") == nullptr && sac_window_may_use_phase(s, B);
  *on = mine;
  if (!(s->ctx->comm && s->ctx->comm_n > 1)) return ILSX_OK;
// ... 255 lines not shown
    }
  }
  return ILSX_OK;
}

static int sac_phase_const_prime(ilsx_sac* s, ilsx_replay* rb) {
  phase_const_prepare(s->ctx, &s->pct);
  if (s->pct.slot < 0 || s->cs <= 1) return ILSX_OK;
  static const bool no_fuse = getenv("ILSX_NO_FUSE") != nullptr;
  s->gather_rb = rb; s->phase_now = true; s->fuse_now = !no_fuse && !sac_is_split(s);
  s->phase_args_only = true;
  int rc = sac_critic_backward(s);
  if (rc == ILSX_OK) rc = sac_actor_backward(s);
  s->phase_args_only = false;
  s->gather_rb = nullptr; s->phase_now = false; s->fuse_now = false;
  return rc;
}

static int sac_sample_and_step(ilsx_sac* s, ilsx_replay* rb, int B) {
  const SacWs& w = s->ws;
  if (s->cs > 1) {
    s->gather_rb = rb;
    s->phase_now = sac_phase_ok(s, B);
    s->phase_last = s->phase_now;
    const int rc = sac_full_step(s);
    s->gather_rb = nullptr;
    s->phase_now = false;
    return rc;
  }
  ILSX_TRY(replay_launch_sample(rb, B, nullptr, s->scal, 0, w.s, w.a, w.r, w.d, w.s2, nullptr));
  return sac_full_step(s);
}

static int sac_train_from_replay_once(ilsx_sac* s, ilsx_replay* rb, int n_steps, int B, ilsx_sac_stats* stats);
extern "C" int ilsx_sac_train_from_replay(ilsx_sac* s, ilsx_replay* rb, int n_steps, int B, ilsx_sac_stats* stats) {
  if (stats && n_steps > 1) {
    ILSX_TRY(ilsx_sac_train_from_replay(s, rb, 1, B, stats));
    return ilsx_sac_train_from_replay(s, rb, n_steps - 1, B, nullptr);
  }
  int rc = sac_train_from_replay_once(s, rb, n_steps, B, stats);
  if (rc == ILSX_RETRY_WINDOW) {
    ILSX_TRY(sac_snapshot_restore(s));
    rc = sac_train_from_replay_once(s, rb, n_steps, B, stats);
    if (rc == ILSX_RETRY_WINDOW) ILSX_FAIL(ILSX_ERR_STATE, "ilsx_sac_train_from_replay: the fallback path asked for a retry");
  }
  return rc;
}
void phase_wgs_per_cu(int H, int cs, int* occ_a, int* occ_c);
extern "C" int ilsx_sac_phase_state(ilsx_sac* s, int* fallbacks, int* disabled, int* last_window_on_phase, int* wgs_per_cu_a, int* wgs_per_cu_c) {
  if (!s) ILSX_FAIL(ILSX_ERR_ARG, "ilsx_sac_phase_state: NULL agent");
  if (fallbacks) *fallbacks = s->phase_fallbacks;
  if (disabled) *disabled = s->phase_broken ? 1 : 0;
  if (last_window_on_phase) *last_window_on_phase = s->phase_last ? 1 : 0;
  int oa = 0, oc = 0;
  if (s->cs > 1 && (s->Lq.cfg.hidden == 256 || s->Lq.cfg.hidden == 128)) phase_wgs_per_cu(s->Lq.cfg.hidden, s->cs, &oa, &oc);
  if (wgs_per_cu_a) *wgs_per_cu_a = oa;
  if (wgs_per_cu_c) *wgs_per_cu_c = oc;
  return ILSX_OK;
}
extern "C" int ilsx_sac_debug_break_phase(ilsx_sac* s) {
  if (!s) ILSX_FAIL(ILSX_ERR_ARG, "ilsx_sac_debug_break_phase: NULL agent");
  static const int one = 1;
  HIPCHK(hipSetDevice(s->ctx->device));
  HIPCHK(hipMemcpyAsync(s->phase_err, &one, sizeof one, hipMemcpyHostToDevice, s->ctx->stream));
  s->debug_break = true;
  return ILSX_OK;
}
static int sac_train_from_replay_once(ilsx_sac* s, ilsx_replay* rb, int n_steps, int B, ilsx_sac_stats* stats) {
  if (!s || !rb || n_steps < 0) ILSX_FAIL(ILSX_ERR_ARG, "ilsx_sac_train_from_replay: bad argument");
  if (B < 1 || B > s->cfg.max_batch) ILSX_FAIL(ILSX_ERR_ARG, "batch %d not in 1..max_batch=%d", B, s->cfg.max_batch);
  if (rb->o != s->o || rb->a != s->a) ILSX_FAIL(ILSX_ERR_ARG, "replay dims (%d,%d) != agent dims (%d,%d)", rb->o, rb->a, s->o, s->a);
  if (rb->size < 1) ILSX_FAIL(ILSX_ERR_STATE, "replay buffer is empty");
  ILSX_TRY(sac_check_world(s, "ilsx_sac_train_from_replay"));
  HIPCHK(hipSetDevice(s->ctx->device));
  ILSX_TRY(replay_flush_state(rb));
  hipStream_t st = s->ctx->stream;
  s->B = B;
  s->eps_explicit = false;
  static const bool split_graph = getenv("ILSX_SPLIT_GRAPH") != nullptr;
  static const bool no_graph_env = getenv("ILSX_NO_GRAPH") != nullptr;
  const bool no_graph = no_graph_env || (sac_is_split(s) && !split_graph);
  if (n_steps == 0) return stats ? sac_read_stats(s, stats) : ILSX_OK;
  ILSX_TRY(sac_defer_begin(s, B));
  struct DeferGuard { ilsx_sac* s; ~DeferGuard() { s->defer_tail = false; } } guard{s};
  const bool deferred = s->defer_tail;
  if (deferred && sac_window_may_use_phase(s, B)) ILSX_TRY(sac_snapshot_take(s));
  if (no_graph || s->ctx->prof_on) {
    for (int i = 0; i < n_steps; ++i) {
      if (stats && i == n_steps - 1) ILSX_TRY(sac_request_stats(s));
      const int rc = sac_sample_and_step(s, rb, B);
      if (rc != ILSX_OK) return rc;
    }
  } else {
    const bool phase = sac_phase_ok(s, B);
    s->phase_last = phase;
    const bool own = phase && sac_own_rows(s);
    static const bool no_reprime = getenv("ILSX_PHASE_CT_NO_REPRIME") != nullptr;
    const bool rebuild = !s->graph || s->graph_rb != rb || s->graph_B != B || s->graph_defer != s->defer_tail || s->graph_phase != phase || s->graph_own != own;
    if (phase && (rebuild || !no_reprime)) ILSX_TRY(sac_phase_const_prime(s, rb));
    if (rebuild) {
      if (s->graph) { hipGraphExecDestroy(s->graph); s->graph = nullptr; }
      hipGraph_t g = nullptr;
      HIPCHK(hipStreamBeginCapture(st, hipStreamCaptureModeThreadLocal));
      int rc = sac_sample_and_step(s, rb, B);
      hipError_t e = hipStreamEndCapture(st, &g);
      if (rc != ILSX_OK) { if (g) hipGraphDestroy(g); return rc; }
      if (e != hipSuccess) ILSX_FAIL(ILSX_ERR_HIP, "hipStreamEndCapture failed: %s", hipGetErrorString(e));
      e = hipGraphInstantiate(&s->graph, g, nullptr, nullptr, 0);
      hipGraphDestroy(g);
      if (e != hipSuccess) { s->graph = nullptr; ILSX_FAIL(ILSX_ERR_HIP, "hipGraphInstantiate failed: %s", hipGetErrorString(e)); }
      s->graph_rb = rb; s->graph_B = B; s->graph_defer = s->defer_tail; s->graph_phase = phase; s->graph_own = own;
    }
    for (int i = 0; i < n_steps; ++i) {
      if (stats && i == n_steps - 1) ILSX_TRY(sac_request_stats(s));
      HIPCHK(hipGraphLaunch(s->graph, st));
    }
  }
  s->defer_tail = false;
  ILSX_TRY(sac_flush_tail(s, deferred));
  ILSX_TRY(sac_phase_check(s, B, deferred, "ilsx_sac_train_from_replay"));
  if (stats) return sac_read_stats(s, stats);
  return ILSX_OK;
}

static const NetLayout* sac_layout(const ilsx_sac* s, int which) { return which == W_PI ? &s->Lp : &s->Lq; }

extern "C" int ilsx_sac_get_params(ilsx_sac* s, int which, float* dst, size_t n, int dst_is_device) {
  if (!s || !dst || which < 0 || which > 4) ILSX_FAIL(ILSX_ERR_ARG, "ilsx_sac_get_params: bad argument");
  HIPCHK(hipSetDevice(s->ctx->device));
  return net_download_flat(s->ctx, *sac_layout(s, which), s->base(which), dst, n, dst_is_device);
}
extern "C" int ilsx_sac_set_params(ilsx_sac* s, int which, const float* src, size_t n, int src_is_device) {
  if (!s || !src || which < 0 || which > 4) ILSX_FAIL(ILSX_ERR_ARG, "ilsx_sac_set_params: bad argument");
  HIPCHK(hipSetDevice(s->ctx->device));
  return net_upload_flat(s->ctx, *sac_layout(s, which), s->base(which), src, n, src_is_device);
}
extern "C" int ilsx_sac_get_grads(ilsx_sac* s, int which, float* dst, size_t n, int dst_is_device) {
  if (!s || !dst || which < 0 || which > 2) ILSX_FAIL(ILSX_ERR_ARG, "ilsx_sac_get_grads: bad argument");
  HIPCHK(hipSetDevice(s->ctx->device));
  return net_download_flat(s->ctx, *sac_layout(s, which), s->gbase(which), dst, n, dst_is_device);
}
extern "C" int ilsx_sac_grads_ptr(ilsx_sac* s, int segment, float** dev_ptr, size_t* n) {
  if (!s || !dev_ptr || !n || segment < 0 || segment > 1) ILSX_FAIL(ILSX_ERR_ARG, "ilsx_sac_grads_ptr: bad argument");
  if (segment == 0) { *dev_ptr = s->G; *n = 2 * s->nq; }
  else { *dev_ptr = s->G + 2 * s->nq; *n = s->np + 4; }
  return ILSX_OK;
}
extern "C" int ilsx_sac_get_log_alpha(ilsx_sac* s, double* out) {
  if (!s || !out) ILSX_FAIL(ILSX_ERR_ARG, "NULL argument");
  HIPCHK(hipSetDevice(s->ctx->device));
  DevScalars h;
  HIPCHK(hipMemcpyAsync(&h, s->scal, sizeof h, hipMemcpyDeviceToHost, s->ctx->stream));
  HIPCHK(hipStreamSynchronize(s->ctx->stream));
  *out = h.log_alpha;
  return ILSX_OK;
}
extern "C" int ilsx_sac_set_log_alpha(ilsx_sac* s, double v) {
  if (!s) ILSX_FAIL(ILSX_ERR_ARG, "NULL argument");
  HIPCHK(hipSetDevice(s->ctx->device));
  DevScalars h;
  HIPCHK(hipMemcpyAsync(&h, s->scal, sizeof h, hipMemcpyDeviceToHost, s->ctx->stream));
  HIPCHK(hipStreamSynchronize(s->ctx->stream));
  h.log_alpha = v;
  h.alpha = (float)std::exp(v);
  HIPCHK(hipMemcpyAsync(s->scal, &h, sizeof h, hipMemcpyHostToDevice, s->ctx->stream));
  HIPCHK(hipStreamSynchronize(s->ctx->stream));
  return ILSX_OK;
}
extern "C" int ilsx_sac_get_adam(ilsx_sac* s, int which, float* m_host, float* v_host, size_t n, int64_t* t) {
  if (!s || !m_host || !v_host || which < 0 || which > 2) ILSX_FAIL(ILSX_ERR_ARG, "ilsx_sac_get_adam: bad argument");
  HIPCHK(hipSetDevice(s->ctx->device));
  const size_t off = s->trainable_off(which);
  ILSX_TRY(net_download_flat(s->ctx, *sac_layout(s, which), s->M + off, m_host, n, 0));
  ILSX_TRY(net_download_flat(s->ctx, *sac_layout(s, which), s->V + off, v_host, n, 0));
  if (t) {
    DevScalars h;
    HIPCHK(hipMemcpyAsync(&h, s->scal, sizeof h, hipMemcpyDeviceToHost, s->ctx->stream));
    HIPCHK(hipStreamSynchronize(s->ctx->stream));
    *t = which == W_PI ? h.t_pi : h.t_q;
  }
  return ILSX_OK;
}
extern "C" int ilsx_sac_set_adam(ilsx_sac* s, int which, const float* m_host, const float* v_host, size_t n, int64_t t) {
  if (!s || !m_host || !v_host || which < 0 || which > 2) ILSX_FAIL(ILSX_ERR_ARG, "ilsx_sac_set_adam: bad argument");
  HIPCHK(hipSetDevice(s->ctx->device));
  const size_t off = s->trainable_off(which);
  ILSX_TRY(net_upload_flat(s->ctx, *sac_layout(s, which), s->M + off, m_host, n, 0));
  ILSX_TRY(net_upload_flat(s->ctx, *sac_layout(s, which), s->V + off, v_host, n, 0));
  DevScalars h;
  HIPCHK(hipMemcpyAsync(&h, s->scal, sizeof h, hipMemcpyDeviceToHost, s->ctx->stream));
  HIPCHK(hipStreamSynchronize(s->ctx->stream));
  if (which == W_PI) h.t_pi = (int)t; else h.t_q = (int)t;
  HIPCHK(hipMemcpyAsync(s->scal, &h, sizeof h, hipMemcpyHostToDevice, s->ctx->stream));
  HIPCHK(hipStreamSynchronize(s->ctx->stream));
// ... 377 lines not shown
```

### ilswiss_amd/csrc/kernels.h

```cpp
#pragma once
#include <hip/hip_runtime.h>
#include <stdint.h>

typedef float f32x4 __attribute__((ext_vector_type(4)));

#define ILSX_LDS_PAD 4
#ifndef ILSX_LATE_WAVES
#define ILSX_LATE_WAVES 4
#endif
#define ILSX_MAX_HID 3
#define ILSX_MAX_NO 64

enum { HEAD_RAW = 0, HEAD_TANH_SAMPLE = 1, HEAD_TANH_DET = 2, HEAD_TANH_LOGP_OF_ACT = 3,
       HEAD_GAUSS_SAMPLE = 4, HEAD_GAUSS_LOGP_OF_ACT = 5,
       HEAD_DET_TANH_NOISE = 6,
       HEAD_DET_LIN_NOISE = 7 };
enum { LOSS_GIVEN = 0, LOSS_SAC_CRITIC = 1, LOSS_SAC_ACTORQ = 2, LOSS_SAC_POLICY = 3, LOSS_MSE = 4, LOSS_PPO_POLICY = 5,
       LOSS_TD_CRITIC = 6, LOSS_SACV_VALUE = 7, LOSS_CONST = 8, LOSS_TD3_POLICY = 9, LOSS_BC_MLE = 10, LOSS_BC_MSE = 11 };
enum { ACT_RELU = 0, ACT_TANH = 1 };

#define LOG_SIG_MIN (-20.0f)
#define LOG_SIG_MAX (2.0f)
#define TANH_EPS (1e-6f)
#define HALF_LOG_2PI (0.91893853320467274178f)
// ... 98 lines not shown
  if (T.scal->gather_step != T.scal->step + 1) return;
  float lpe = 0.f;
  if (!T.slot_given) {
    for (int r = threadIdx.x; r < T.B; r += 256) lpe += T.logp[r] + T.target_entropy;
    lpe = block256_sum(lpe, sh4);
  }
  if (threadIdx.x == 0) {
    T.scal->alpha_used = T.scal->alpha;
    T.scal->log_alpha_used = T.scal->log_alpha;
    if (!T.slot_given) {
      T.alpha_grad_slot[0] = -lpe * T.inv_B;
      T.alpha_grad_slot[1] = 0.f; T.alpha_grad_slot[2] = 0.f; T.alpha_grad_slot[3] = 0.f;
    }
    sac_finish_dev(T.scal, T.alpha_grad_slot, T.train_alpha, T.lr, T.b1, T.b2, T.eps, T.qf_lr, T.policy_lr, 1);
  }
}

template <int ACT> __device__ __forceinline__ float act_fn(float z) {
  if (ACT == ACT_RELU) return fmaxf(z, 0.0f);
  return tanhf(z);
}
template <int ACT> __device__ __forceinline__ float act_grad_from_out(float h) {
  if (ACT == ACT_RELU) return h > 0.0f ? 1.0f : 0.0f;
  return 1.0f - h * h;
}


#define ILSX_TRACE_SLOTS 8
#define ILSX_TRACE_MAXWG 2048
#define ILSX_WG_LINEAR (blockIdx.x + gridDim.x * (blockIdx.y + gridDim.y * blockIdx.z))
#if defined(ILSX_STAMPS) && defined(ILSX_STAMPS_FINE)
#define ILSX_STAMP_SYNC(dbg, i) do { asm volatile("s_waitcnt vmcnt(0) lgkmcnt(0)" ::: "memory"); if ((dbg) && threadIdx.x == 0 && ILSX_WG_LINEAR < ILSX_TRACE_MAXWG) (dbg)[(size_t)ILSX_WG_LINEAR * ILSX_TRACE_SLOTS + (i)] = wall_clock64(); asm volatile("" ::: "memory"); } while (0)
#else
#define ILSX_STAMP_SYNC(dbg, i) ((void)0)
#endif
#ifdef ILSX_STAMPS
#define ILSX_STAMP(dbg, i) do { if ((dbg) && threadIdx.x == 0 && ILSX_WG_LINEAR < ILSX_TRACE_MAXWG) (dbg)[(size_t)ILSX_WG_LINEAR * ILSX_TRACE_SLOTS + (i)] = wall_clock64(); } while (0)
#else
#define ILSX_STAMP(dbg, i) ((void)0)
#endif

__host__ __device__ __forceinline__ int pack_f(int n, int k, int K) {
  return (((n >> 4) * (K >> 4) + (k >> 4)) * 64 + ((k & 15) >> 2) * 16 + (n & 15)) * 4 + (k & 3);
}
__host__ __device__ __forceinline__ int pack_b(int n, int k, int N) {
  return (((k >> 4) * (N >> 4) + (n >> 4)) * 64 + ((n & 15) >> 2) * 16 + (k & 15)) * 4 + (n & 3);
}

#define MFMA16(a, b, c) __builtin_amdgcn_mfma_f32_16x16x4f32((a), (b), (c), 0, 0, 0)

template <int CTL> __device__ __forceinline__ float wave_dpp(float v) {
  return __int_as_float(__builtin_amdgcn_update_dpp(0, __float_as_int(v), CTL, 0xf, 0xf, false));
}
__device__ __forceinline__ float wave_sum(float v) {
  v += wave_dpp<0xB1>(v);
  v += wave_dpp<0x4E>(v);
  v += wave_dpp<0x141>(v);
  v += wave_dpp<0x140>(v);
  const int b = __float_as_int(v);
  const float r0 = __int_as_float(__builtin_amdgcn_readlane(b, 0)), r1 = __int_as_float(__builtin_amdgcn_readlane(b, 16));
  const float r2 = __int_as_float(__builtin_amdgcn_readlane(b, 32)), r3 = __int_as_float(__builtin_amdgcn_readlane(b, 48));
  return ((r0 + r1) + r2) + r3;
}
template <int N> __device__ __forceinline__ void load_vec(const float* p, float (&v)[N]) {
  if constexpr (N == 4) { const float4 t = *reinterpret_cast<const float4*>(p); v[0] = t.x; v[1] = t.y; v[2] = t.z; v[3] = t.w; }
  else if constexpr (N == 2) { const float2 t = *reinterpret_cast<const float2*>(p); v[0] = t.x; v[1] = t.y; }
  else { v[0] = p[0]; }
}

struct DevReplayState {
  long long size, top;
};
__device__ __forceinline__ long long replay_draw(uint64_t seed, uint64_t step, uint32_t stream, uint32_t r, long long size) {
  uint32_t c[4] = {r >> 2, 0x52425546u , (uint32_t)step, (uint32_t)(step >> 32) ^ (stream * 0x9E3779B9u)};
  philox4x32_10(c, (uint32_t)seed, (uint32_t)(seed >> 32) ^ stream);
  const uint32_t u = c[r & 3];
  return (long long)(((unsigned long long)u * (unsigned long long)size) >> 32);
}
struct GatherSpec {
  const float* records; const DevReplayState* st;
  float *s, *a, *r, *d, *s2;
  uint64_t seed; uint32_t stream; int rec, o, adim, on;
};

struct FwdTask {
  NetView net;
  const float* x0; const float* x1;
  int d0, s0, d1, s1;
  float* xsave;
  float* hsave[ILSX_MAX_HID];
  float* out;
  int head;
  uint32_t rng_stream;
  const float* eps;
  const float* act_in;
  float* eps_save;
  float* action;
  float* logp;
  union {
    struct {
      float* part;
      int g0_off, g1_off;
    };
    struct {
      uint64_t seed_t, step_t;
    };
  };
  int publish;
  const int* rows_idx;
  const float* log_std;
  float noise, noise_clip, max_act;
  int no_fin;
  int agent, first;
  int out_cols;
};
static_assert(offsetof(FwdTask, step_t) == offsetof(FwdTask, g0_off) && sizeof(float*) == 8, "FwdTask: the generic kernel's per-task key overlays part | g0_off | g1_off");
typedef __attribute__((address_space(1))) float gfloat;
template <bool X> __device__ __forceinline__ float ldx(const float* p) { return *p; }
template <bool X> __device__ __forceinline__ void stx(float* p, float v) { *p = v; }
template <bool X> __device__ __forceinline__ float ldx(const gfloat* p) { return *p; }
template <bool X> __device__ __forceinline__ void stx(gfloat* p, float v) { *p = v; }
template <bool X> __device__ __forceinline__ float ldx_uniform(const float* p) {
  if constexpr (X) return __hip_atomic_load(p, __ATOMIC_RELAXED, __HIP_MEMORY_SCOPE_AGENT);
  else return *p;
}
struct PartVal {
  const float* p; int cs; int stride;
  template <bool X = false>
  __device__ __forceinline__ float get(int r) const {
    const float v0 = ldx<X>(p + r);
    const float v1 = cs > 1 ? ldx<X>(p + (size_t)stride + r) : 0.0f;
    const float v2 = cs > 2 ? ldx<X>(p + (size_t)2 * stride + r) : 0.0f;
    const float v3 = cs > 3 ? ldx<X>(p + (size_t)3 * stride + r) : 0.0f;
    float s = v0;
    if (cs > 1) s += v1;
    if (cs > 2) s += v2;
    if (cs > 3) s += v3;
    return s;
  }
};
template <bool X, int CSV>
__device__ __forceinline__ float partval_get(const float* pp, int stride, int r) {
  static_assert(CSV >= 1 && CSV <= 4, "cs <= 4");
  const gfloat* p = (const gfloat*)pp;
  const float v0 = ldx<X>(p + r);
  const float v1 = CSV > 1 ? ldx<X>(p + (size_t)stride + r) : 0.0f;
  const float v2 = CSV > 2 ? ldx<X>(p + (size_t)2 * stride + r) : 0.0f;
  const float v3 = CSV > 3 ? ldx<X>(p + (size_t)3 * stride + r) : 0.0f;
  float s = v0;
  if (CSV > 1) s += v1;
  if (CSV > 2) s += v2;
  if (CSV > 3) s += v3;
  return s;
}
#define XCH_PIN(v) asm volatile("" : "+s"(v))
template <bool G> __device__ __forceinline__ auto xg(const float* p) { if constexpr (G) return (const gfloat*)p; else return p; }
template <bool G> __device__ __forceinline__ auto xg(float* p) { if constexpr (G) return (gfloat*)p; else return p; }
struct PolicyFinishArgs {
  const float* part; int cs, part_stride, rows, a, head;
  uint32_t rng_stream; uint64_t seed; const DevScalars* scal; uint64_t step_host;
  const float* eps; const float* act_in;
  float *raw, *eps_save, *action, *logp;
  float noise, noise_clip, max_act;
  int use_gather_step;
};
struct FwdGroup;
struct FwdArgs {
  FwdTask t[4];
  int rows, ntasks;
  uint64_t seed;
  const DevScalars* scal;
  uint64_t step_host;
  unsigned long long* dbg;
  int part_stride;
  int fin_on;
  PolicyFinishArgs fin;
  GatherSpec gather;
  int xs;
  const struct FwdTaskG* tasks;
  int rt;
  const struct TailLite* tail;
  int tail_mode, tail_n;
  int l0_split;
  int reserved_mt[7];
  int ctab;
  int late;
};
static_assert(sizeof(FwdArgs) == 1456 && offsetof(FwdArgs, ctab) == 1448, "FwdArgs keeps the layout it had with the macro-tile fields (reserved_mt)");
struct FwdGroup { PolicyFinishArgs fin; GatherSpec gather; const DevScalars* scal; int fin_on; };
struct FwdTaskG { FwdTask t; FwdGroup g; };

#ifdef ILSX_KERNEL_IMPL
template <int H>
__device__ __forceinline__ void fwd_heads_row(const float* hrow, const float* Wh, const float* bh, int NO, float* hout_row, int lane) {
  constexpr int KPL = H / 64;
  float hv[KPL];
  load_vec<KPL>(hrow + KPL * lane, hv);
  for (int j0 = 0; j0 < NO; j0 += 4) {
    float s[4];
#pragma unroll
    for (int u = 0; u < 4; ++u) {
      const int j = min(j0 + u, NO - 1);
      float wv[KPL];
      load_vec<KPL>(Wh + (size_t)j * H + KPL * lane, wv);
      float t = 0.0f;
#pragma unroll
      for (int c = 0; c < KPL; ++c) t = fmaf(hv[c], wv[c], t);
      s[u] = t;
    }
#pragma unroll
    for (int u = 0; u < 4; ++u) s[u] = wave_sum(s[u]);
    if (lane == 0) {
#pragma unroll
      for (int u = 0; u < 4; ++u)
        if (j0 + u < NO) hout_row[j0 + u] = s[u] + bh[j0 + u];
    }
  }
}
__device__ __forceinline__ void fwd_head_row(const FwdTask& T, const FwdArgs& A, const float* ho, int gr, int lane, int NO) {
  const int oc = T.out_cols > 0 ? T.out_cols : NO;
  if (T.out && lane < oc) T.out[(size_t)gr * oc + lane] = ho[lane];
  if (T.head == HEAD_RAW) return;
  if (T.head == HEAD_DET_TANH_NOISE || T.head == HEAD_DET_LIN_NOISE) {
    const int j = lane;
    if (j < NO && T.action) {
      float act = T.max_act * (T.head == HEAD_DET_LIN_NOISE ? ho[j] : tanhf(ho[j]));
      if (T.noise != 0.0f) {
        float e;
        if (T.eps) {
          e = T.eps[(size_t)gr * NO + j];
        } else {
          float z4[4];
          philox_normal4(T.step_t ? T.seed_t : A.seed, T.step_t ? T.step_t : (A.scal ? A.scal->step : A.step_host), T.rng_stream, gr, j >> 2, z4);
          const int qd = j & 3;
          e = qd == 0 ? z4[0] : qd == 1 ? z4[1] : qd == 2 ? z4[2] : z4[3];
        }
        act += fminf(fmaxf(T.noise * e, -T.noise_clip), T.noise_clip);
      }
      T.action[(size_t)gr * NO + j] = act;
    }
    return;
  }
  if (T.head >= HEAD_GAUSS_SAMPLE) {
    const bool cond = T.log_std == nullptr;
    const int a = cond ? NO >> 1 : NO, j = lane;
    float q = 0.f, l = 0.f;
    if (j < a) {
      const float mu = ho[j], ls = cond ? fminf(fmaxf(ho[a + j], LOG_SIG_MIN), LOG_SIG_MAX) : T.log_std[j];
      float act;
      if (T.head == HEAD_GAUSS_LOGP_OF_ACT) {
        const size_t sr = T.rows_idx ? (size_t)T.rows_idx[gr] : (size_t)gr;
        act = T.act_in[sr * a + j];
      } else {
        float e;
        if (T.eps) {
          e = T.eps[(size_t)gr * a + j];
        } else {
          float z4[4];
          philox_normal4(T.step_t ? T.seed_t : A.seed, T.step_t ? T.step_t : (A.scal ? A.scal->step : A.step_host), T.rng_stream, gr, j >> 2, z4);
          const int qd = j & 3;
          e = qd == 0 ? z4[0] : qd == 1 ? z4[1] : qd == 2 ? z4[2] : z4[3];
        }
        act = e * expf(ls) + mu;
        if (T.action) T.action[(size_t)gr * a + j] = act;
      }
      const float dm = mu - act;
      q = dm * dm / expf(2.0f * ls);
// ... 372 lines not shown
    const int col = c0 + li;
    float hpv[4];
    {
      const float* const hpp = T.hsave[l - 1] + (size_t)(r0 + 4 * g) * H + col;
#pragma unroll
      for (int v = 0; v < 4; ++v) hpv[v] = (full_tile || r0 + 4 * g + v < rows) ? hpp[(size_t)v * H] : 0.0f;
    }
    f32x4 acc0 = (f32x4){0.f, 0.f, 0.f, 0.f}, acc1 = acc0;
    const float* ap = cur + li * LDH + 4 * g;
#pragma unroll
    for (int c = 0; c < NC; ++c) {
      const float4 a = *reinterpret_cast<const float4*>(ap + 16 * c);
      acc0 = MFMA16(a.x, wreg[c].x, acc0); acc1 = MFMA16(a.y, wreg[c].y, acc1);
      acc0 = MFMA16(a.z, wreg[c].z, acc0); acc1 = MFMA16(a.w, wreg[c].w, acc1);
    }
    if (l - 1 >= 1) {
      const float* wp = N.base + N.off_Wb[l - 1] + (size_t)wave * NC * 256 + 4 * lane;
#pragma unroll
      for (int c = 0; c < NC; ++c) wreg[c] = *reinterpret_cast<const float4*>(wp + 256 * c);
    }
    float* ds = T.dsave[l - 1];
    float* const dsp = ds ? ds + (size_t)(r0 + 4 * g) * H + col : nullptr;
#pragma unroll
    for (int v = 0; v < 4; ++v) {
      const int row = 4 * g + v;
      const bool ok = full_tile || r0 + row < rows;
      const float dv = ok ? (acc0[v] + acc1[v]) * act_grad_from_out<ACT>(hpv[v]) : 0.0f;
      if (ds && ok) dsp[(size_t)v * H] = dv;
      nxt[row * LDH + col] = dv;
    }
    lds_barrier();
    cur = nxt;
  }

  if (T.dx) {
    const float* W0 = N.base + N.off_W[0];
    const int ld0 = N.ld[0];
#pragma unroll
    for (int rr = 0; rr < RPW; ++rr) {
      const int row = wave * RPW + rr, gr = r0 + row;
      float dv[KPL];
#pragma unroll
      for (int i = 0; i < KPL; ++i) dv[i] = cur[row * LDH + lane + 64 * i];
      for (int c = 0; c < T.dx_cols; ++c) {
        float s = 0.0f;
#pragma unroll
        for (int i = 0; i < KPL; ++i) s = fmaf(dv[i], W0[pack_f(lane + 64 * i, T.dx_col0 + c, ld0)], s);
        s = wave_sum(s);
        if (lane == 0 && gr < rows) T.dx[(size_t)gr * T.dx_cols + c] = s;
      }
    }
  }
}
#endif

#define GRP_CONST_SLOTS 768
#ifdef ILSX_KERNEL_IMPL
__constant__ FwdTaskG g_fwd_tab[GRP_CONST_SLOTS];
__constant__ BwdTask g_bwd_tab[GRP_CONST_SLOTS];
#endif
#ifdef ILSX_KERNEL_IMPL
template <int H, int ACT, int CS, int GRP, int PH = 0>
__global__ __launch_bounds__(4 * H / CS, (GRP == 3 ? ILSX_LATE_WAVES : 1)) void k_mlp2_fwd_split(const FwdArgs A) {
  extern __shared__ __attribute__((aligned(16))) float smem[];
  if (A.tail_mode && (int)blockIdx.y == A.ntasks) {
    const int ag = blockIdx.x + gridDim.x * blockIdx.z;
    if (ag < A.tail_n) {
      const TailLite& TL = A.tail[ag];
      if (A.tail_mode == 1) tail_lite_run(TL, smem);
      else if (threadIdx.x == 0) TL.scal->gather_step += 1;
    }
    return;
  }
  FwdTaskG Rg;
  const int ty = (int)blockIdx.y;
  if (GRP == 1) Rg = A.tasks[ty];
  const FwdTaskG& Rc = g_fwd_tab[GRP >= 2 ? A.ctab - 1 + ty : 0];
  const FwdTask& T = GRP >= 2 ? Rc.t : GRP == 1 ? Rg.t : A.t[ty];
  const FwdGroup* GP = GRP >= 2 ? &Rc.g : GRP == 1 ? &Rg.g : nullptr;
  constexpr bool XCH = false;
  const int bx = (int)blockIdx.x, cs = (int)blockIdx.z;
  const bool first_task = ty == 0;
  constexpr int FIN_CT = 0;
#define XCH_HOOK_STAGE
#define XCH_HOOK_FIN
#define XCH_STAMP(i) ILSX_STAMP(A.dbg, i)
#include "fwd_split_tile.inc"
#undef XCH_STAMP
#undef XCH_HOOK_STAGE
#undef XCH_HOOK_FIN
}
#endif
#ifdef ILSX_KERNEL_IMPL
__global__ __launch_bounds__(64) void k_policy_finish(const PolicyFinishArgs P) {
  const int gr = blockIdx.x * 64 + threadIdx.x;
  if (gr >= P.rows) return;
  const int a = P.a, NO = 2 * a;
  float lp_quad = 0.f, lp_ls = 0.f, lp_jac = 0.f;
  const uint64_t step = P.scal ? P.scal->step : P.step_host;
  for (int j0 = 0; j0 < a; j0 += 4) {
    float z4[4] = {0.f, 0.f, 0.f, 0.f};
    if (P.head == HEAD_TANH_SAMPLE && !P.eps) philox_normal4(P.seed, step, P.rng_stream, gr, j0 >> 2, z4);
    for (int jj = 0; jj < 4 && j0 + jj < a; ++jj) {
      const int j = j0 + jj;
      float mu = 0.f, lsr = 0.f;
      for (int c = 0; c < P.cs; ++c) {
        mu += P.part[((size_t)c * P.part_stride + gr) * NO + j];
        lsr += P.part[((size_t)c * P.part_stride + gr) * NO + a + j];
      }
      if (P.raw) { P.raw[(size_t)gr * NO + j] = mu; P.raw[(size_t)gr * NO + a + j] = lsr; }
      const float ls = fminf(fmaxf(lsr, LOG_SIG_MIN), LOG_SIG_MAX);
      const float sd = expf(ls);
      float e = 0.f, z, act;
      if (P.head == HEAD_TANH_DET) {
        z = mu; act = tanhf(mu);
      } else if (P.head == HEAD_TANH_LOGP_OF_ACT) {
        act = P.act_in[(size_t)gr * a + j];
        z = 0.5f * (logf(1.0f + act + TANH_EPS) - logf(1.0f - act + TANH_EPS));
      } else {
        e = P.eps ? P.eps[(size_t)gr * a + j] : z4[jj];
        z = e * sd + mu;
        act = tanhf(z);
      }
      const float dm = mu - z;
      lp_quad += dm * dm / expf(2.0f * ls);
      lp_ls += ls;
      lp_jac += logf(1.0f - act * act + TANH_EPS);
      if (P.action) P.action[(size_t)gr * a + j] = act;
      if (P.eps_save) P.eps_save[(size_t)gr * a + j] = e;
    }
  }
  if (P.logp) P.logp[gr] = -0.5f * lp_quad - (lp_ls + HALF_LOG_2PI) - lp_jac;
}

template <int H, int ACT, int CS, int GRP>
__global__ __launch_bounds__(4 * H / CS, (GRP == 3 ? ILSX_LATE_WAVES : 1)) void k_mlp2_bwd_split(const BwdArgs A) {
  extern __shared__ __attribute__((aligned(16))) float smem[];
  const int ty = (int)blockIdx.y;
  BwdTask Tg;
  if (GRP == 1) Tg = A.tasks[ty];
  const BwdTask& T = GRP >= 2 ? g_bwd_tab[A.ctab - 1 + ty] : GRP == 1 ? Tg : A.t[ty];
  constexpr bool XCH = false;
  const int bx = (int)blockIdx.x, cs = (int)blockIdx.z;
  constexpr int LOSS_CT = -1, NO_CT = 0;
#define XCH_HOOK_ACT
#define XCH_HOOK_HEAD
#define XCH_STAMP(i) ILSX_STAMP(A.dbg, i)
#include "bwd_split_tile.inc"
#undef XCH_STAMP
#undef XCH_HOOK_ACT
#undef XCH_HOOK_HEAD
}
#endif

#define PHASE_MAX_TILES 64
#define PHASE_TAIL_FLAG (3 * PHASE_MAX_TILES)
#define PHASE_NFLAGS (3 * PHASE_MAX_TILES + 1)
#define PHASE_MASK_WORD(t) ((PHASE_NFLAGS + (t)) * 32)
#define PHASE_FLAG_WORDS ((PHASE_NFLAGS + PHASE_MAX_TILES) * 32)
struct PhaseAArgs {
  FwdArgs f1, f2; BwdArgs b1; unsigned* flags; int* err; unsigned long long* dbg;
  PolicyFinishArgs fin_pi; int fin_pi_on;
  int own_rows;
};
struct PhaseCArgs {
  FwdArgs f3; BwdArgs b2, b3; unsigned* flags; int* err; unsigned long long* dbg;
// ... 10 lines not shown
#endif

#ifdef ILSX_KERNEL_IMPL
__device__ __forceinline__ void xch_arrive(unsigned* flag) {
  asm volatile("s_waitcnt vmcnt(0)" ::: "memory");
  __syncthreads();
  if (threadIdx.x == 0) __hip_atomic_fetch_add(flag, 1u, __ATOMIC_RELAXED, __HIP_MEMORY_SCOPE_AGENT);
}
#define PHASE_FLAG_DEAD 0x40000000u
__device__ __forceinline__ void xch_wait(const unsigned* flag, unsigned target, int* err) {
  if (threadIdx.x == 0) {
    int spins = 0;
    while (__hip_atomic_load(flag, __ATOMIC_RELAXED, __HIP_MEMORY_SCOPE_AGENT) < target) {
      __builtin_amdgcn_s_sleep(2);
      if (++spins > (1 << 16)) { __hip_atomic_store(err, 1, __ATOMIC_RELAXED, __HIP_MEMORY_SCOPE_AGENT); break; }
    }
  }
  __syncthreads();
  asm volatile("buffer_inv sc0" ::: "memory");
}
__device__ __forceinline__ unsigned xcc_id() {
  unsigned v;
  asm volatile("s_getreg_b32 %0, hwreg(HW_REG_XCC_ID)" : "=s"(v));
  return v & 15u;
}
__device__ __forceinline__ unsigned cu_key() {
  unsigned v;
  asm volatile("s_getreg_b32 %0, hwreg(HW_REG_HW_ID)" : "=s"(v));
  return (xcc_id() << 8) | ((v >> 8) & 255u);
}
__device__ __forceinline__ void xch_mark_xcd(unsigned* mask) {
  if (threadIdx.x == 0) __hip_atomic_fetch_or(mask, 1u << xcc_id(), __ATOMIC_RELAXED, __HIP_MEMORY_SCOPE_AGENT);
}

__device__ __forceinline__ void policy_fin_tile(const PolicyFinishArgs& P, int r0, int rows, float* lp3, int nth) {
  const int a = P.a, NOp = 2 * a, tid = threadIdx.x;
  const unsigned long long fstep = P.scal ? (P.use_gather_step ? P.scal->gather_step : P.scal->step) : P.step_host;
  for (int e = tid; e < 16 * a; e += nth) {
    const int row = e / a, j = e - row * a, gr = r0 + row;
    float c0 = 0.0f, c1 = 0.0f, c2 = 0.0f;
    if (gr < rows) {
      float pm[4], pl[4];
#pragma unroll
      for (int c = 0; c < 4; ++c) {
        const size_t at = ((size_t)(c < P.cs ? c : 0) * P.part_stride + gr) * NOp + j;
        pm[c] = P.part[at];
        pl[c] = P.part[at + a];
      }
      float mu = 0.f, lsr = 0.f;
#pragma unroll
      for (int c = 0; c < 4; ++c) { mu += c < P.cs ? pm[c] : 0.0f; lsr += c < P.cs ? pl[c] : 0.0f; }
      float ep;
      if (P.eps) {
        ep = P.eps[(size_t)gr * a + j];
      } else {
        float z4[4];
        philox_normal4(P.seed, fstep, P.rng_stream, gr, j >> 2, z4);
        const int q = j & 3;
        ep = q == 0 ? z4[0] : q == 1 ? z4[1] : q == 2 ? z4[2] : z4[3];
      }
      const float ls = fminf(fmaxf(lsr, LOG_SIG_MIN), LOG_SIG_MAX);
      const float sd = expf(ls);
      const float z = ep * sd + mu;
      const float act = tanhf(z);
      const float dm = mu - z;
      c0 = dm * dm / expf(2.0f * ls); c1 = ls; c2 = logf(1.0f - act * act + TANH_EPS);
      if (P.raw) { P.raw[(size_t)gr * NOp + j] = mu; P.raw[(size_t)gr * NOp + a + j] = lsr; }
      if (P.action) P.action[(size_t)gr * a + j] = act;
      if (P.eps_save) P.eps_save[(size_t)gr * a + j] = ep;
    }
    lp3[(row * 32 + j) * 3 + 0] = c0; lp3[(row * 32 + j) * 3 + 1] = c1; lp3[(row * 32 + j) * 3 + 2] = c2;
  }
  lds_barrier();
  if (P.logp && tid < 16 && r0 + tid < rows) {
    float q = 0.f, l = 0.f, jc = 0.f;
    for (int j = 0; j < a; ++j) { q += lp3[(tid * 32 + j) * 3]; l += lp3[(tid * 32 + j) * 3 + 1]; jc += lp3[(tid * 32 + j) * 3 + 2]; }
    P.logp[r0 + tid] = -0.5f * q - (l + HALF_LOG_2PI) - jc;
  }
  lds_barrier();
}

template <int H, int ACT, int CS, bool CT = false>
__global__ __launch_bounds__(4 * H / CS) void k_sac_phase_a(const PhaseAArgs Pk, int slot) {
  const PhaseAArgs& P = CT ? g_phase_a_tab[slot] : Pk;
  constexpr int GRP = 0; constexpr bool XCH = true;
  constexpr int PH = 0;
  extern __shared__ __attribute__((aligned(16))) float smem[];
  const FwdGroup* GP = nullptr;
  const int bx = blockIdx.x, cs = blockIdx.z, y = blockIdx.y;
  unsigned* tflag = P.flags + PHASE_TAIL_FLAG * 32;
  if (y == 4) {
    if (bx == 0 && cs == 0) {
      const TailLite& TL = P.f1.tail[0];
      tail_lite_run(TL, smem);
      if (threadIdx.x == 0) {
        __hip_atomic_store(&TL.scal->alpha, TL.scal->alpha, __ATOMIC_RELAXED, __HIP_MEMORY_SCOPE_AGENT);
        asm volatile("s_waitcnt vmcnt(0)" ::: "memory");
        __hip_atomic_store(tflag, 1u, __ATOMIC_RELAXED, __HIP_MEMORY_SCOPE_AGENT);
      }
    }
    return;
  }
  if (bx * 16 >= P.f1.rows) return;
  unsigned* f1 = P.flags + (3 * bx) * 32;
  unsigned* f2 = P.flags + (3 * bx + 1) * 32;
  unsigned* f0 = P.flags + (3 * bx + 2) * 32;
  const bool own = y >= 5;
  ILSX_STAMP(P.dbg, 0);
#if defined(ILSX_STAMPS) && defined(ILSX_STAMPS_FINE)
  if (P.dbg && threadIdx.x == 0 && (y == 1 || y == 2)) P.dbg[(size_t)ILSX_WG_LINEAR * ILSX_TRACE_SLOTS + 5] = clock64();
#endif
  xch_mark_xcd(P.flags + PHASE_MASK_WORD(bx));
#if defined(ILSX_STAMPS) && !defined(ILSX_STAMPS_FINE)
  if (P.dbg && threadIdx.x == 0 && ILSX_WG_LINEAR < ILSX_TRACE_MAXWG) P.dbg[(size_t)ILSX_WG_LINEAR * ILSX_TRACE_SLOTS + 7] = 0x10000u | cu_key();
#endif
  if (!own) {
    {
      const FwdArgs& A = P.f1;
      const FwdTask& T = A.t[y];
      const bool first_task = y == 0;
      constexpr int FIN_CT = -1;
#define XCH_HOOK_STAGE
#define XCH_HOOK_FIN
#define XCH_STAMP(i) ((void)0)
#include "fwd_split_tile.inc"
#undef XCH_STAMP
#undef XCH_HOOK_STAGE
#undef XCH_HOOK_FIN
    }
    ILSX_STAMP(P.dbg, 1);
    if (y == 0) {
      asm volatile("s_waitcnt vmcnt(0)" ::: "memory");
      __syncthreads();
      if (threadIdx.x == 0) {
        __hip_atomic_fetch_add(f0, 1u, __ATOMIC_RELAXED, __HIP_MEMORY_SCOPE_AGENT);
        __hip_atomic_fetch_add(f1, 1u, __ATOMIC_RELAXED, __HIP_MEMORY_SCOPE_AGENT);
      }
    } else {
      xch_arrive(f1);
    }
    ILSX_STAMP(P.dbg, 2);
    if (P.own_rows && (y == 0 || y == 3)) return;
  }
  if (y == 0 || y == 3 || own) {
    {
      const FwdArgs& A = P.f2;
      const int tq = own ? y - 5 : (y == 0 ? 0 : 1);
      const FwdTask& T = A.t[tq];
      const bool first_task = tq == 0;
      constexpr int FIN_CT = 1;
#define XCH_HOOK_STAGE ILSX_STAMP_SYNC(P.dbg, 7); xch_wait(f0, CS, P.err); ILSX_STAMP(P.dbg, 3);
#define XCH_HOOK_FIN
#define XCH_FINE_DBG P.dbg
#define XCH_STAMP(i) do { if (own) ILSX_STAMP(P.dbg, (i) == 3 ? 6 : (i)); } while (0)
#include "fwd_split_tile.inc"
#undef XCH_STAMP
#undef XCH_FINE_DBG
#undef XCH_HOOK_STAGE
#undef XCH_HOOK_FIN
    }
    ILSX_STAMP(P.dbg, 4);
    xch_arrive(f2);
    ILSX_STAMP(P.dbg, 5);
  } else {
    xch_wait(f1, 4 * CS, P.err);
    xch_wait(tflag, 1u, P.err);
    if (P.fin_pi_on && y == 1 && cs == 0) {
      policy_fin_tile(P.fin_pi, bx * 16, P.f1.rows, smem, 4 * H / CS);
    }
    {
      const BwdArgs& A = P.b1;
      const BwdTask& T = A.t[y - 1];
      constexpr int LOSS_CT = LOSS_SAC_CRITIC, NO_CT = 1;
#define XCH_HOOK_ACT
#define XCH_HOOK_HEAD xch_wait(f2, 2 * CS, P.err); ILSX_STAMP(P.dbg, 3);
#if defined(ILSX_STAMPS_FINE)
#define XCH_STAMP(i) ((void)0)
#else
#define XCH_STAMP(i) do { if ((i) < 3) ILSX_STAMP(P.dbg, 4 + (i)); } while (0)
#endif
#include "bwd_split_tile.inc"
#undef XCH_STAMP
#undef XCH_HOOK_ACT
#undef XCH_HOOK_HEAD
    }
    ILSX_STAMP(P.dbg, 4);
#if defined(ILSX_STAMPS) && defined(ILSX_STAMPS_FINE)
    if (P.dbg && threadIdx.x == 0) P.dbg[(size_t)ILSX_WG_LINEAR * ILSX_TRACE_SLOTS + 6] = clock64();
#endif
  }
}

template <int H, int ACT, int CS, bool CT = false>
__global__ __launch_bounds__(4 * H / CS) void k_sac_phase_c(const PhaseCArgs Pk, int slot) {
  const PhaseCArgs& P = CT ? g_phase_c_tab[slot] : Pk;
  constexpr int GRP = 0; constexpr bool XCH = true;
  constexpr int PH = 0;
  extern __shared__ __attribute__((aligned(16))) float smem[];
  const FwdGroup* GP = nullptr;
  const int bx = blockIdx.x, cs = blockIdx.z, y = blockIdx.y;
  if (y == 3) {
    if (bx == 0 && cs == 0 && threadIdx.x == 0) P.f3.tail[0].scal->gather_step += 1;
    if (P.aslot && bx == 1 && cs == 0) alpha_slot_run(P.aslot_logp, P.aslot_B, P.aslot_te, P.aslot_invB, P.aslot, smem);
    const float tau = P.polyak_tau;
    for (int i = ((int)(cs * gridDim.x + bx) * (int)blockDim.x + (int)threadIdx.x) * 4; i < P.polyak_n; i += (int)(gridDim.x * gridDim.z * blockDim.x) * 4) {
      const float4 p = *reinterpret_cast<const float4*>(P.polyak_P + i);
      float4 t = *reinterpret_cast<const float4*>(P.polyak_T + i);
      t.x = t.x * (1.0f - tau) + p.x * tau; t.y = t.y * (1.0f - tau) + p.y * tau;
      t.z = t.z * (1.0f - tau) + p.z * tau; t.w = t.w * (1.0f - tau) + p.w * tau;
      *reinterpret_cast<float4*>(P.polyak_T + i) = t;
    }
    return;
  }
  if (bx * 16 >= P.f3.rows) return;
  unsigned* f1 = P.flags + (3 * bx) * 32;
  unsigned* f2 = P.flags + (3 * bx + 1) * 32;
  ILSX_STAMP(P.dbg, 0);
  xch_mark_xcd(P.flags + PHASE_MASK_WORD(bx));
  if (y == 2) {
    {
      const BwdArgs& A = P.b3;
      const BwdTask& T = A.t[0];
      constexpr int LOSS_CT = LOSS_SAC_POLICY, NO_CT = 0;
#define XCH_HOOK_ACT
#define XCH_HOOK_HEAD xch_wait(f2, 2 * CS, P.err); ILSX_STAMP(P.dbg, 4);
#define XCH_STAMP(i) ILSX_STAMP(P.dbg, i)
#include "bwd_split_tile.inc"
#undef XCH_STAMP
#undef XCH_HOOK_ACT
#undef XCH_HOOK_HEAD
    }
    ILSX_STAMP(P.dbg, 5);
    return;
  }
  {
    const FwdArgs& A = P.f3;
    const FwdTask& T = A.t[y];
    const bool first_task = y == 0;
    constexpr int FIN_CT = -1;
#define XCH_HOOK_STAGE
#define XCH_HOOK_FIN
#define XCH_STAMP(i) ((void)0)
#include "fwd_split_tile.inc"
#undef XCH_STAMP
#undef XCH_HOOK_STAGE
#undef XCH_HOOK_FIN
  }
  ILSX_STAMP(P.dbg, 1);
  xch_arrive(f1);
  {
    const BwdArgs& A = P.b2;
    const BwdTask& T = A.t[y];
    constexpr int LOSS_CT = LOSS_SAC_ACTORQ, NO_CT = 1;
#define XCH_HOOK_ACT xch_wait(f1, 2 * CS, P.err); ILSX_STAMP(P.dbg, 2);
#define XCH_HOOK_HEAD
#define XCH_STAMP(i) ILSX_STAMP(P.dbg, 3 + (i))
#include "bwd_split_tile.inc"
#undef XCH_STAMP
#undef XCH_HOOK_ACT
#undef XCH_HOOK_HEAD
  }
  ILSX_STAMP(P.dbg, 3);
  xch_arrive(f2);
}
#endif

enum { DW_OUT_NATURAL = 0, DW_OUT_PACK_F = 1, DW_OUT_PACK_FB = 2 };
struct DwMat {
  const float* A; const float* Bm; float* dW; float* dWb; float* db;
  int lda, NA, ldb, NB, ldw, mode;
  int rows, bias_rows;
  int tile0, ktiles;
  int agent;
};
#define DW_MAX_MATS 10
struct AdamFuse {
  const float* Gbase; float* P; float* M; float* V; float* T;
  float b1, b2, eps, tau;
  const float* step_size; const float* bc2_sqrt;
  int on;
  float l2x2;
};
struct DwArgs {
  DwMat m[DW_MAX_MATS];
  int nmat, rows_all, ntiles, pad;
  AdamFuse F;
  unsigned long long* dbg;
  int xs;
  int splits, rows_per_split;
  float* g_lo; float* g_hi;
  float* scratch; size_t span;
  const struct DwTileG* gtiles;
  unsigned* zero_flags;
  const int* zero_err;
  int tile_nh, tile_kt;
  int reserved_strip;
};
static_assert(sizeof(DwArgs) == 1072 && offsetof(DwArgs, reserved_strip) == 1064, "DwArgs keeps the layout it had with the strip flag (reserved_strip)");
struct DwTileG { DwMat J; AdamFuse F; };
#define DW_SPLIT_MIN_ROWS 1024
#define DW_BIG_MIN_ROWS 4096
#define DW_TILE_N 32
#define DW_TILE_K 64

#ifdef ILSX_KERNEL_IMPL
#define ILSX_ST(ptr, val) (*(ptr) = (val))
typedef float __attribute__((address_space(1))) ilsx_gfloat;
#ifdef ILSX_FLAT_TABLE_PTRS
#define ILSX_G(G) false
#else
#define ILSX_G(G) (G)
#endif
template <bool G>
__device__ __forceinline__ float ld_f(const float* p) {
  if (ILSX_G(G)) return *(const ilsx_gfloat*)p;
  return *p;
}
template <bool G>
__device__ __forceinline__ void st_f(float* p, float v) {
  if (ILSX_G(G)) *(ilsx_gfloat*)p = v;
  else ILSX_ST(p, v);
}
struct AdamOperands { float p, m, v, t; };
template <bool G = false>
__device__ __forceinline__ AdamOperands adam_prefetch(const AdamFuse& F, size_t i0) {
  AdamOperands o;
  o.p = ld_f<G>(F.P + i0); o.m = ld_f<G>(F.M + i0); o.v = ld_f<G>(F.V + i0); o.t = F.T ? ld_f<G>(F.T + i0) : 0.0f;
  return o;
}
template <bool G = false>
__device__ __forceinline__ void adam_apply(const AdamFuse& F, float step, float bc2s, const AdamOperands& o, size_t i0,
                                           size_t i1, bool two, float g) {
  g = g + F.l2x2 * o.p;
  const float m = o.m * F.b1 + (1.0f - F.b1) * g;
  const float v = o.v * F.b2 + (1.0f - F.b2) * g * g;
  const float p = o.p - step * (m / (sqrtf(v) / bc2s + F.eps));
  st_f<G>(F.M + i0, m); st_f<G>(F.V + i0, v); st_f<G>(F.P + i0, p);
  float tg = 0.0f;
  if (F.T) { tg = o.t * (1.0f - F.tau) + p * F.tau; st_f<G>(F.T + i0, tg); }
  if (two) {
    st_f<G>(F.M + i1, m); st_f<G>(F.V + i1, v); st_f<G>(F.P + i1, p);
    if (F.T) st_f<G>(F.T + i1, tg);
  }
}

#define DW_LDS_BYTES_OF(NH, KT) ((8 * (NH) * 4 * (KT) * 64 + 8 * (NH) * 16) * 4)
template <bool GRP, int NH, int KT, bool LOW>
__device__ __forceinline__ void dw_tile_body(const DwArgs& D, float* smem) {
  constexpr int NW = 8 * NH, NT = 512 * NH, TN = 16 * NH, TK = 16 * KT, EPT = (KT + 1) / 2;
  float* part = smem;
  float* bpart = smem + NW * 4 * KT * 64;
  if (blockIdx.x & ((1u << D.xs) - 1u)) return;
  const int bx = blockIdx.x >> D.xs;
  if (D.zero_flags && bx == 0 && blockIdx.y == 0 && threadIdx.x < PHASE_NFLAGS)
    D.zero_flags[threadIdx.x * 32] = (D.zero_err && *D.zero_err) ? PHASE_FLAG_DEAD : 0u;
  int mi = 0;
  if (!GRP) {
#pragma unroll
    for (int i = 1; i < DW_MAX_MATS; ++i)
      if (i < D.nmat && bx >= D.m[i].tile0) mi = i;
  }
  DwTileG Rg;
  if (GRP) {
    Rg = D.gtiles[bx];
  } else { Rg.J = D.m[mi]; Rg.F = D.F; }
  const DwMat& J = Rg.J;
  const AdamFuse& F = Rg.F;
  const int local = bx - J.tile0;
  const int n0 = (local / J.ktiles) * TN, k0 = (local % J.ktiles) * TK;
  int rows = J.rows > 0 ? J.rows : D.rows_all, brows = J.rows > 0 ? J.bias_rows : D.rows_all;
  int r_begin = 0;
  float* out_shift = nullptr;
  if (D.splits > 1) {
    r_begin = blockIdx.y * D.rows_per_split;
    rows = min(rows, r_begin + D.rows_per_split);
    brows = rows;
    out_shift = D.scratch + (size_t)blockIdx.y * D.span;
  }
  const int tid = threadIdx.x, lane = tid & 63, wave = tid >> 6, li = lane & 15, g = lane >> 4;
  const int wn = wave % NH, wr = wave / NH;
  const int nsub = n0 + 16 * wn;
  const bool n_ok = nsub + li < J.NA;
  int ntk = (J.NB - k0 + 15) / 16;
  if (ntk > KT) ntk = KT;
  ILSX_STAMP(D.dbg, 0);
  const bool packed = J.mode != DW_OUT_NATURAL;
  float* g0p[EPT]; float* g1p[EPT]; bool live[EPT];
  AdamOperands ao[EPT];
  float ad_step = 0.f, ad_bc2s = 1.f;
  bool bias_thread = false;
  float* gbp = nullptr;
  AdamOperands aob;
#define DW_OUTPUT_ELEMS()                                                                                                          \
  {                                                                                                                                \
    if (F.on) { ad_step = ld_f<GRP>(F.step_size); ad_bc2s = ld_f<GRP>(F.bc2_sqrt); }                                                                   \
    _Pragma("unroll") for (int h = 0; h < EPT; ++h) {                                                                              \
      const int e = tid + NT * h, ee = e % (256 * NH * KT);                                                                        \
      const int on = ee / (256 * KT), rest = ee % (256 * KT), t = rest >> 8, q = rest & 255;                                       \
                                                                                                   \
      const int v = packed ? (q >> 2) & 3 : (q >> 6) & 3;                                                                          \
      const int ol = packed ? ((q >> 4) & 3) * 16 + 4 * (q >> 6) + (q & 3) : q & 63;                                               \
      const int n = n0 + 16 * on + 4 * (ol >> 4) + v, k = k0 + 16 * t + (ol & 15);                                                 \
      live[h] = e < 256 * NH * KT && t < ntk && n < J.NA && k < J.NB;                                                              \
      g0p[h] = nullptr; g1p[h] = nullptr;                                                                                          \
      if (live[h]) {                                                                                                               \
        g0p[h] = J.mode == DW_OUT_NATURAL ? J.dW + (size_t)n * J.ldw + k : J.dW + pack_f(n, k, J.ldw);                             \
        g1p[h] = J.mode == DW_OUT_PACK_FB ? J.dWb + pack_b(n, k, J.NA) : nullptr;                                                  \
        if (out_shift) {                                                                                                           \
          g0p[h] = out_shift + (g0p[h] - D.g_lo);                                                                                  \
          if (g1p[h]) g1p[h] = out_shift + (g1p[h] - D.g_lo);                                                                      \
        }                                                                                                                          \
        if (F.on) ao[h] = adam_prefetch<GRP>(F, (size_t)(g0p[h] - F.Gbase));                                                            \
      }                                                                                                                            \
    }                                                                                                                              \
    bias_thread = J.db && k0 == 0 && tid < 16 * NH && n0 + 16 * (tid >> 4) + (tid & 15) < J.NA;                                    \
    gbp = bias_thread ? J.db + n0 + 16 * (tid >> 4) + (tid & 15) : nullptr;                                                        \
    if (gbp && out_shift) gbp = out_shift + (gbp - D.g_lo);                                                                        \
    if (bias_thread && F.on) aob = adam_prefetch<GRP>(F, (size_t)(gbp - F.Gbase));                                                      \
  }
  if (!LOW) DW_OUTPUT_ELEMS();

  f32x4 acc[KT];
#pragma unroll
  for (int t = 0; t < KT; ++t) acc[t] = (f32x4){0.f, 0.f, 0.f, 0.f};
  float bsum = 0.0f;
  bool k_ok[KT];
#pragma unroll
  for (int t = 0; t < KT; ++t) k_ok[t] = k0 + 16 * t + li < J.NB;
  const bool tile_in = n0 + TN <= J.NA && k0 + TK <= J.NB;
  for (int rc = r_begin + 16 * wr; rc < rows; rc += 256) {
    float a[2][4], b[2][KT][4];
    const int rbase = rc - 16 * wr;
    if (tile_in && rbase + 256 <= rows && rbase + 256 <= brows) {
      const float* const pa = J.A + (size_t)(rc + 4 * g) * J.lda + nsub + li;
      const float* const pb = J.Bm + (size_t)(rc + 4 * g) * J.ldb + k0 + li;
      if (LOW) {
#pragma unroll
        for (int u = 0; u < 2; ++u) {
// ... 336 lines not shown
```

Before: 20090.

## Pre-stage replay rows into dense buffers ahead of the phase kernels

Replay-buffer gathering is moved out of the phase-A first stage. Rows for the next step are staged into dense workspace buffers (ns/na/nr/nd/ns2) by phase C's idle y==3 blocks, or by a standalone staging kernel at the start of the window. A specialised row path (SROW) in the forward tile then loads plain rows into registers early, peels the layer-0 K loop, and preloads head bias. The goal is to take random-gather latency off phase A's critical path, at the cost of extra workspace, extra template instantiations, and a gather-step bump moved into the dw kernel that must stay consistent.

```diff
diff --git a/ilswiss_amd/csrc/fwd_split_tile.inc b/ilswiss_amd/csrc/fwd_split_tile.inc
--- a/ilswiss_amd/csrc/fwd_split_tile.inc
+++ b/ilswiss_amd/csrc/fwd_split_tile.inc
@@ -1,4 +1,6 @@
   constexpr bool FINS = FIN_CT > 0;
+  constexpr bool SROW = ROWS_CT == 1;
+  constexpr bool BHPRE = ROWS_CT > 0;
   constexpr int NTH = 4 * H / CS, NWV = NTH / 64, NC = H / 16, SLW = H / CS, NCS = SLW / 16;
   constexpr int NT0 = PH == 1 ? 1 : CS;
   constexpr int LDH = H + ILSX_LDS_PAD, LDSL = SLW + ILSX_LDS_PAD;
@@ -19,9 +21,27 @@
   if ((int)(bx >> A.xs) * (A.rt > 0 ? A.rt : 1) * MR >= A.rows) return;
   const int tid = threadIdx.x, lane = tid & 63, wave = tid >> 6, li = lane & 15, g = lane >> 4;
   const int rows = A.rows;
-  const int RT = A.rt > 0 ? A.rt : 1;
+  const int RT = SROW ? 1 : (A.rt > 0 ? A.rt : 1);
   const bool lead = cs == 0;
   ILSX_STAMP(A.dbg, 0);
+
+  constexpr int SRT = 2;
+  float srv[SRT];
+  if constexpr (SROW) {
+    static_assert(FIN_CT == -1 && PH == 0 && GRP == 0 && NTH == 16 * MR, "plain rows of a phase kernel's first stage, one 16 x 16 block of the tile per trip");
+    const int sgr = (int)(bx >> A.xs) * MR + (tid >> 4);
+#pragma unroll
+    for (int t = 0; t < SRT; ++t) {
+      const int k = (tid & 15) + 16 * t;
+      const float* src = k < T.d0 ? T.x0 + (size_t)sgr * T.s0 + k : T.x1 + (size_t)sgr * T.s1 + (k - T.d0);
+      srv[t] = (k < T.d0 + T.d1 && sgr < rows) ? *src : 0.0f;
+    }
+  }
+  const bool spub = SROW && lead && T.publish == 1 && (tid & 15) == 0 && (int)(bx >> A.xs) * MR + (tid >> 4) < rows;
+  float spr = 0.0f, spd = 0.0f;
+  if constexpr (SROW) {
+    if (spub) { spr = A.stg_r[(int)(bx >> A.xs) * MR + (tid >> 4)]; spd = A.stg_d[(int)(bx >> A.xs) * MR + (tid >> 4)]; }
+  }
 
   const int ct0 = PH == 1 ? cs * NWV + wave : wave * CS;
   const float* w0p = N.base + N.off_W[0] + (size_t)ct0 * NCH0 * 256 + 4 * lane;
@@ -46,18 +66,29 @@
   float4 whf[4];
   float4 wreg[NC];
   constexpr bool LATEW = GRP == 3 && PH == 0;
+  float bhv[4] = {0.0f, 0.0f, 0.0f, 0.0f};
+  if constexpr (BHPRE) {
+    static_assert(NTH == 256 && PH == 0, "one head-output tile per trip of the final sum");
+#pragma unroll
+    for (int i = 0; i < 4; ++i) { const int j = 16 * i + (tid & 15); bhv[i] = (N.base + N.off_bh)[j < NO ? j : NO - 1]; }
+  }
   if constexpr (PH != 1) {
     bias1 = (N.base + N.off_b[1])[col1];
 #pragma unroll
     for (int t = 0; t < 4; ++t) {
       const int j = 16 * t + li;
+      if constexpr (SROW) whf[t] = *reinterpret_cast<const float4*>(N.base + N.off_Wh + (size_t)(j < NO ? j : NO - 1) * H + cs * SLW + 16 * wave + 4 * g);
+      else
       whf[t] = (t < NOT && j < NO) ? *reinterpret_cast<const float4*>(N.base + N.off_Wh + (size_t)j * H + cs * SLW + 16 * wave + 4 * g)
                                    : make_float4(0.f, 0.f, 0.f, 0.f);
     }
     if constexpr (!LATEW) {
       const float* wp = N.base + N.off_W[1] + (size_t)(cs * NWV + wave) * NC * 256 + 4 * lane;
 #pragma unroll
-      for (int c = 0; c < NC; ++c) wreg[c] = *reinterpret_cast<const float4*>(wp + 256 * c);
+      for (int c = 0; c < NC; ++c) {
+        wreg[c] = *reinterpret_cast<const float4*>(wp + 256 * c);
+        if constexpr (SROW) asm volatile("" ::: "memory");
+      }
     }
   }
 #ifdef XCH_FINE_DBG
@@ -158,7 +189,39 @@
     }
   } else {
   XCH_HOOK_STAGE
-  if constexpr (PH == 0) {
+  if constexpr (SROW) {
+    const int r = tid >> 4, gr = r0 + r;
+    float* const xsv = (T.xsave && lead && gr < rows) ? T.xsave + (size_t)gr * KP : nullptr;
+    const int pub = (lead && gr < rows) ? T.publish : 0;
+    auto publish = [&](int k, float v) {
+      if (pub == 1) {
+        if (k < T.d0) G.s[(size_t)gr * G.o + k] = v;
+        else if (k < T.d0 + T.d1) G.a[(size_t)gr * G.adim + (k - T.d0)] = v;
+      } else if (pub == 2 && k < T.d0) {
+        G.s2[(size_t)gr * G.o + k] = v;
+      }
+    };
+#pragma unroll
+    for (int t = 0; t < SRT; ++t) {
+      const int k = (tid & 15) + 16 * t;
+      if (k < KP) {
+        if (xsv) xsv[k] = srv[t];
+        xs[r * LDX + k] = srv[t];
+        publish(k, srv[t]);
+      }
+    }
+    if (spub) { stx<XCH>(G.r + gr, spr); stx<XCH>(G.d + gr, spd); }
+    for (int k = (tid & 15) + 16 * SRT; k < KP; k += 16) {
+      float v = 0.0f;
+      if (gr < rows) {
+        if (k < T.d0) v = T.x0[(size_t)gr * T.s0 + k];
+        else if (k < T.d0 + T.d1) v = T.x1[(size_t)gr * T.s1 + (k - T.d0)];
+        if (xsv) xsv[k] = v;
+        publish(k, v);
+      }
+      xs[r * LDX + k] = v;
+    }
+  } else if constexpr (PH == 0) {
     long long* ridx0 = reinterpret_cast<long long*>(hs);
     if constexpr (GRP != 0) {
       if (G.on) {
@@ -390,6 +453,30 @@
 #pragma unroll
     for (int i = 0; i < NT0; ++i) acc[i] = (f32x4){0.f, 0.f, 0.f, 0.f};
     const float* ap = xs + li * LDX + 4 * g;
+    auto l0_chunk = [&](int kc) {
+      const float4 a = *reinterpret_cast<const float4*>(ap + kc);
+#pragma unroll
+      for (int i = 0; i < NT0; ++i) acc[i] = MFMA16(a.x, b0[i].x, acc[i]);
+#pragma unroll
+      for (int i = 0; i < NT0; ++i) acc[i] = MFMA16(a.y, b0[i].y, acc[i]);
+#pragma unroll
+      for (int i = 0; i < NT0; ++i) acc[i] = MFMA16(a.z, b0[i].z, acc[i]);
+#pragma unroll
+      for (int i = 0; i < NT0; ++i) acc[i] = MFMA16(a.w, b0[i].w, acc[i]);
+    };
+    if (SROW && KP == 16) {
+      l0_chunk(0);
+    } else if constexpr (SROW) {
+      for (int kc = 0; kc + 16 < KP; kc += 16) {
+        float4 bn[NT0];
+#pragma unroll
+        for (int i = 0; i < NT0; ++i) bn[i] = *reinterpret_cast<const float4*>(w0p + (size_t)i * NCH0 * 256 + (kc + 16) * 16);
+        l0_chunk(kc);
+#pragma unroll
+        for (int i = 0; i < NT0; ++i) b0[i] = bn[i];
+      }
+      l0_chunk(KP - 16);
+    } else
     for (int kc = 0; kc < KP; kc += 16) {
       float4 bn[NT0];
 #pragma unroll
@@ -503,6 +590,20 @@
   }
   lds_barrier();
   const float* bh = N.base + N.off_bh;
+  if constexpr (BHPRE) {
+#pragma unroll
+    for (int i = 0; i < 4; ++i) {
+      if (i < NOT) {
+        const int e = tid + 256 * i;
+        const int t = e >> 8, v = (e >> 6) & 3, ol = e & 63;
+        float sum = 0.0f;
+#pragma unroll
+        for (int w2 = 0; w2 < NWV; ++w2) sum += red[((t * NWV + w2) * 4 + v) * 64 + ol];
+        const int row = 4 * (ol >> 4) + v, j = 16 * t + (ol & 15), gr = r0 + row;
+        if (j < NO && gr < rows) stx<XCH>(T.part + ((size_t)cs * A.part_stride + gr) * NO + j, sum + (lead ? bhv[i] : 0.0f));
+      }
+    }
+  } else
 #pragma unroll
   for (int m = 0; m < MT; ++m)
   for (int e = tid; e < NOT * 256; e += NTH) {
diff --git a/ilswiss_amd/csrc/host_common.h b/ilswiss_amd/csrc/host_common.h
--- a/ilswiss_amd/csrc/host_common.h
+++ b/ilswiss_amd/csrc/host_common.h
@@ -139,6 +139,7 @@
 void phase_const_free(int device, int slot);
 bool phase_a_static_ok(const PhaseAArgs& P, int H, int cs);
 bool phase_c_static_ok(const PhaseCArgs& P, int H, int cs);
+bool phase_staged_rows();
 int launch_phase_a(ilsx_ctx* ctx, const PhaseAArgs& P, int H, int act, int KPmax, int cs, PhaseConst* ct = nullptr, unsigned long long key = 0, bool upload_only = false);
 int launch_phase_c(ilsx_ctx* ctx, const PhaseCArgs& P, int H, int act, int KPmax, int cs, PhaseConst* ct = nullptr, unsigned long long key = 0, bool upload_only = false);
 int device_cus(ilsx_ctx* ctx);
diff --git a/ilswiss_amd/csrc/ilsx_core.hip b/ilswiss_amd/csrc/ilsx_core.hip
--- a/ilswiss_amd/csrc/ilsx_core.hip
+++ b/ilswiss_amd/csrc/ilsx_core.hip
@@ -488,6 +488,11 @@
   return !(e && atoi(e) == 0) && phase_fits(ctx, rows, H, cs, ntasks, true);
 }
 
+bool phase_staged_rows() {
+  const char* e = getenv("ILSX_PHASE_STAGED_ROWS");
+  return !(e && atoi(e) == 0);
+}
+
 static std::vector<bool> g_phase_slots[16];
 static std::mutex g_phase_slots_mu;
 int phase_const_alloc(int device) {
@@ -546,8 +551,8 @@
   return true;
 }
 bool phase_c_static_ok(const PhaseCArgs& P, int H, int cs) {
-  (void)H;
   if (P.f3.fin_on) return false;
+  if (P.f3.gather.on == 1 || 4 * H / cs != 256) return false;
   for (int i = 0; i < 2; ++i) {
     const BwdTask& t = P.b2.t[i];
     if (t.loss != LOSS_SAC_ACTORQ || t.net.NO != 1 || t.q1n.cs != cs || t.q2n.cs != cs) return false;
@@ -592,8 +597,11 @@
   if (trace) { hipStreamCaptureStatus cap = hipStreamCaptureStatusNone; hipStreamIsCapturing(ctx->stream, &cap);
                fprintf(stderr, "launch_phase_a: %s, slot %d, capturing %d\n", use_ct ? "constant table" : "kernel arguments", ct ? ct->slot : -9, (int)cap); }
   ProfScope ps(ctx, ILSX_K_SAC_PHASE_A);
-#define PHASE_A(HH, AA, CC) do { if (use_ct) ILSX_LAUNCH(ps, (k_sac_phase_a<HH, AA, CC, true>), grid, block, lds, ctx->stream, P, slot); \
-                                 else ILSX_LAUNCH(ps, (k_sac_phase_a<HH, AA, CC>), grid, block, lds, ctx->stream, P, slot); } while (0)
+  const bool rows_first = phase_staged_rows() && !P.f1.gather.on;
+#define PHASE_A(HH, AA, CC) do { if (use_ct && rows_first) ILSX_LAUNCH(ps, (k_sac_phase_a<HH, AA, CC, true>), grid, block, lds, ctx->stream, P, slot); \
+                                 else if (rows_first) ILSX_LAUNCH(ps, (k_sac_phase_a<HH, AA, CC>), grid, block, lds, ctx->stream, P, slot); \
+                                 else if (use_ct) ILSX_LAUNCH(ps, (k_sac_phase_a_late<HH, AA, CC, true>), grid, block, lds, ctx->stream, P, slot); \
+                                 else ILSX_LAUNCH(ps, (k_sac_phase_a_late<HH, AA, CC>), grid, block, lds, ctx->stream, P, slot); } while (0)
   if (H == 256 && act == ILSX_ACT_RELU) PHASE_A(256, ACT_RELU, 4);
   else if (H == 256) PHASE_A(256, ACT_TANH, 4);
   else if (act == ILSX_ACT_RELU) PHASE_A(128, ACT_RELU, 2);
@@ -618,8 +626,12 @@
   if (upload_only) return ILSX_OK;
   const int slot = use_ct ? ct->slot : 0;
   ProfScope ps(ctx, ILSX_K_SAC_PHASE_C);
-#define PHASE_C(HH, AA, CC) do { if (use_ct) ILSX_LAUNCH(ps, (k_sac_phase_c<HH, AA, CC, true>), grid, block, lds, ctx->stream, P, slot); \
-                                 else ILSX_LAUNCH(ps, (k_sac_phase_c<HH, AA, CC>), grid, block, lds, ctx->stream, P, slot); } while (0)
+  const bool rows_first = phase_staged_rows();
+  if (P.f3.gather.on == 2 && !rows_first) ILSX_FAIL(ILSX_ERR_STATE, "launch_phase_c: a staging spec with ILSX_PHASE_STAGED_ROWS=0");
+#define PHASE_C(HH, AA, CC) do { if (use_ct && rows_first) ILSX_LAUNCH(ps, (k_sac_phase_c<HH, AA, CC, true>), grid, block, lds, ctx->stream, P, slot); \
+                                 else if (rows_first) ILSX_LAUNCH(ps, (k_sac_phase_c<HH, AA, CC>), grid, block, lds, ctx->stream, P, slot); \
+                                 else if (use_ct) ILSX_LAUNCH(ps, (k_sac_phase_c_late<HH, AA, CC, true>), grid, block, lds, ctx->stream, P, slot); \
+                                 else ILSX_LAUNCH(ps, (k_sac_phase_c_late<HH, AA, CC>), grid, block, lds, ctx->stream, P, slot); } while (0)
   if (H == 256 && act == ILSX_ACT_RELU) PHASE_C(256, ACT_RELU, 4);
   else if (H == 256) PHASE_C(256, ACT_TANH, 4);
   else if (act == ILSX_ACT_RELU) PHASE_C(128, ACT_RELU, 2);
diff --git a/ilswiss_amd/csrc/ilsx_sac.hip b/ilswiss_amd/csrc/ilsx_sac.hip
--- a/ilswiss_amd/csrc/ilsx_sac.hip
+++ b/ilswiss_amd/csrc/ilsx_sac.hip
@@ -14,6 +14,7 @@
   float *xp, *hp[ILSX_MAX_HID], *dp[ILSX_MAX_HID], *dhp;
   float* ppart;
   float* ppart2;
+  float *ns, *na, *nr, *nd, *ns2;
 };
 
 struct StatsArgs {
@@ -47,6 +48,7 @@
   DevScalars* scal = nullptr;
   SacWs ws;
   DwArgs jobs_q, jobs_p;
+  bool staged_now = false;
   ilsx_replay* gather_rb = nullptr;
   bool fuse_now = false;
   int cs = 1;
@@ -58,7 +60,7 @@
   hipGraphExec_t graph = nullptr;
   ilsx_replay* graph_rb = nullptr;
   int graph_B = 0;
-  bool graph_defer = false, graph_phase = false, graph_own = false;
+  bool graph_defer = false, graph_phase = false, graph_own = false, graph_rows_first = false;
   bool defer_tail = false;
   TailLite* tail_dev = nullptr;
   int tail_B = 0;
@@ -237,6 +239,7 @@
   A(&w.xp, B * s->Lp.KP);
   for (int l = 0; l < s->Lp.cfg.n_hidden; ++l) { A(&w.hp[l], B * H); A(&w.dp[l], B * H); }
   A(&w.dhp, B * 2 * a);
+  A(&w.ns, B * o); A(&w.na, B * a); A(&w.nr, B); A(&w.nd, B); A(&w.ns2, B * o);
   const char* e = getenv("ILSX_L0_SPLIT_KP");
   const int thr = e ? atoi(e) : 65;
   if (s->cs == 4 && H == 256 && std::max(s->Lq.KP, s->Lp.KP) >= thr) A(&s->h0scr, 4 * B * H);
@@ -404,7 +407,7 @@
   mix(rb ? (unsigned long long)rb->rec : 0); mix(rb ? (unsigned long long)rb->seed : 0); mix(rb ? (unsigned long long)rb->rng_stream : 0);
   mix((unsigned long long)s->B); mix(s->defer_tail ? 1 : 0); mix(s->eps_explicit ? 1 : 0); mix(s->fuse_now ? 1 : 0); mix((unsigned long long)s->cs);
   mix((unsigned long long)(uintptr_t)s->tail_dev); mix((unsigned long long)(uintptr_t)s->slab);
-  mix(sac_own_rows(s) ? 1 : 0);
+  mix(sac_own_rows(s) ? 1 : 0); mix(s->staged_now ? 1 : 0);
   return k ? k : 1;
 }
 
@@ -415,19 +418,22 @@
   const float* eps2 = s->eps_explicit ? w.eps2 : nullptr;
   PhaseAArgs PA;
   if (s->phase_now) memset(&PA, 0, sizeof PA);
+  const bool staged = s->staged_now && s->phase_now && s->gather_rb && cs > 1;
+  const float* in_s = staged ? w.ns : w.s; const float* in_a = staged ? w.na : w.a; const float* in_s2 = staged ? w.ns2 : w.s2;
   {
     FwdArgs A;
     memset(&A, 0, sizeof A);
     A.rows = B; A.ntasks = 4; A.seed = s->ctx->seed; A.scal = s->scal; A.part_stride = s->cfg.max_batch;
-    sac_policy_task(s, A.t[0], w.s2, eps1, s->rng_stream, false, w.a2, w.logp2, w.ppart);
-    sac_policy_task(s, A.t[3], w.s, eps2, s->rng_stream + 1, true, w.an, w.logp, w.ppart2);
-    sac_q_task(s, A.t[1], W_Q1, w.s, w.a, w.q1, true, true, 0);
-    sac_q_task(s, A.t[2], W_Q2, w.s, w.a, w.q2, true, true, 1);
+    sac_policy_task(s, A.t[0], in_s2, eps1, s->rng_stream, false, w.a2, w.logp2, w.ppart);
+    sac_policy_task(s, A.t[3], in_s, eps2, s->rng_stream + 1, true, w.an, w.logp, w.ppart2);
+    sac_q_task(s, A.t[1], W_Q1, in_s, in_a, w.q1, true, true, 0);
+    sac_q_task(s, A.t[2], W_Q2, in_s, in_a, w.q2, true, true, 1);
     if (s->gather_rb && cs > 1) {
       ilsx_replay* rb = s->gather_rb;
       GatherSpec& G = A.gather;
       G.records = rb->data; G.st = rb->dstate; G.rec = rb->rec; G.seed = rb->seed; G.stream = rb->rng_stream;
-      G.o = s->o; G.adim = s->a; G.on = 1;
+      G.o = s->o; G.adim = s->a; G.on = staged ? 0 : 1;
+      if (staged) { A.stg_r = w.nr; A.stg_d = w.nd; }
       G.s = w.s; G.a = w.a; G.r = w.r; G.d = w.d; G.s2 = w.s2;
       A.t[0].g0_off = s->o + s->a + 2; A.t[0].publish = 2;
       A.t[1].g0_off = 0; A.t[1].g1_off = s->o; A.t[1].publish = 1;
@@ -505,6 +511,25 @@
   return launch_adam(s->ctx, A);
 }
 
+static GatherSpec sac_stage_spec(const ilsx_sac* s, const ilsx_replay* rb) {
+  GatherSpec G;
+  memset(&G, 0, sizeof G);
+  const SacWs& w = s->ws;
+  G.records = rb->data; G.st = rb->dstate; G.rec = rb->rec; G.seed = rb->seed; G.stream = rb->rng_stream;
+  G.o = s->o; G.adim = s->a; G.on = 2;
+  G.s = w.ns; G.a = w.na; G.r = w.nr; G.d = w.nd; G.s2 = w.ns2;
+  return G;
+}
+__global__ __launch_bounds__(256) void k_sac_stage_rows(const GatherSpec G, const DevScalars* scal, int rows) {
+  stage_rows_tile(G, scal->gather_step, (int)blockIdx.x, rows);
+}
+static int sac_stage_window_start(ilsx_sac* s, ilsx_replay* rb, int B) {
+  ProfScope ps(s->ctx, ILSX_K_REPLAY_SAMPLE);
+  ILSX_LAUNCH(ps, k_sac_stage_rows, dim3((B + 15) / 16), dim3(256), 0, s->ctx->stream, sac_stage_spec(s, rb), s->scal, B);
+  HIPCHK(hipGetLastError());
+  return ILSX_OK;
+}
+
 static StatsArgs sac_stats_args(ilsx_sac* s);
 static int sac_actor_backward(ilsx_sac* s) {
   const SacWs& w = s->ws;
@@ -519,7 +544,11 @@
     sac_q_task(s, A.t[0], W_Q1, w.s, w.an, w.q1n, false, true, 0);
     sac_q_task(s, A.t[1], W_Q2, w.s, w.an, w.q2n, false, true, 1);
     if (!s->phase_now) sac_policy_fin(s, A, eps2, s->rng_stream + 1, true, w.an, w.logp, w.ppart2);
-    if (s->phase_now) { A.tail = s->tail_dev; PC.f3 = A; }
+    if (s->phase_now) {
+      A.tail = s->tail_dev;
+      if (s->staged_now && s->gather_rb) A.gather = sac_stage_spec(s, s->gather_rb);
+      PC.f3 = A;
+    }
     else ILSX_TRY(sac_fwd(s, A, H, act, s->Lq.KP, cs));
   }
   {
@@ -568,6 +597,11 @@
       F.b1 = s->cfg.beta_1; F.b2 = 0.999f; F.eps = 1e-8f; F.tau = 0.f;
       F.step_size = &s->scal->adam_pi_step; F.bc2_sqrt = &s->scal->adam_pi_bc2s;
     }
+    if (s->phase_now && s->staged_now && s->gather_rb) {
+      DwArgs jp = s->jobs_p;
+      jp.bump_step = &s->scal->gather_step;
+      ILSX_TRY(sac_dw(s, jp, B, &F));
+    } else
     ILSX_TRY(sac_dw(s, s->jobs_p, B, &F));
   }
   if (s->fuse_now) return ILSX_OK;
@@ -989,8 +1023,10 @@
   const bool no_graph = no_graph_env || (sac_is_split(s) && !split_graph);
   if (n_steps == 0) return stats ? sac_read_stats(s, stats) : ILSX_OK;
   ILSX_TRY(sac_defer_begin(s, B));
-  struct DeferGuard { ilsx_sac* s; ~DeferGuard() { s->defer_tail = false; } } guard{s};
+  struct DeferGuard { ilsx_sac* s; ~DeferGuard() { s->defer_tail = false; s->staged_now = false; } } guard{s};
   const bool deferred = s->defer_tail;
+  s->staged_now = deferred && n_steps > 0 && !sac_is_split(s) && phase_staged_rows() && sac_phase_ok(s, B);
+  if (s->staged_now) ILSX_TRY(sac_stage_window_start(s, rb, B));
   if (deferred && sac_window_may_use_phase(s, B)) ILSX_TRY(sac_snapshot_take(s));
   if (no_graph || s->ctx->prof_on) {
     for (int i = 0; i < n_steps; ++i) {
@@ -1002,8 +1038,10 @@
     const bool phase = sac_phase_ok(s, B);
     s->phase_last = phase;
     const bool own = phase && sac_own_rows(s);
+    const bool rows_first = phase && phase_staged_rows();
     static const bool no_reprime = getenv("ILSX_PHASE_CT_NO_REPRIME") != nullptr;
-    const bool rebuild = !s->graph || s->graph_rb != rb || s->graph_B != B || s->graph_defer != s->defer_tail || s->graph_phase != phase || s->graph_own != own;
+    const bool rebuild = !s->graph || s->graph_rb != rb || s->graph_B != B || s->graph_defer != s->defer_tail || s->graph_phase != phase || s->graph_own != own ||
+                         s->graph_rows_first != rows_first;
     if (phase && (rebuild || !no_reprime)) ILSX_TRY(sac_phase_const_prime(s, rb));
     if (rebuild) {
       if (s->graph) { hipGraphExecDestroy(s->graph); s->graph = nullptr; }
@@ -1016,7 +1054,7 @@
       e = hipGraphInstantiate(&s->graph, g, nullptr, nullptr, 0);
       hipGraphDestroy(g);
       if (e != hipSuccess) { s->graph = nullptr; ILSX_FAIL(ILSX_ERR_HIP, "hipGraphInstantiate failed: %s", hipGetErrorString(e)); }
-      s->graph_rb = rb; s->graph_B = B; s->graph_defer = s->defer_tail; s->graph_phase = phase; s->graph_own = own;
+      s->graph_rb = rb; s->graph_B = B; s->graph_defer = s->defer_tail; s->graph_phase = phase; s->graph_own = own; s->graph_rows_first = rows_first;
     }
     for (int i = 0; i < n_steps; ++i) {
       if (stats && i == n_steps - 1) ILSX_TRY(sac_request_stats(s));
diff --git a/ilswiss_amd/csrc/kernels.h b/ilswiss_amd/csrc/kernels.h
--- a/ilswiss_amd/csrc/kernels.h
+++ b/ilswiss_amd/csrc/kernels.h
@@ -204,6 +204,21 @@
   float *s, *a, *r, *d, *s2;
   uint64_t seed; uint32_t stream; int rec, o, adim, on;
 };
+__device__ __forceinline__ void stage_rows_tile(const GatherSpec& G, unsigned long long step, int tile, int rows) {
+  const int gr = tile * 16 + ((int)threadIdx.x >> 4);
+  if (gr >= rows) return;
+  const long long idx = replay_draw(G.seed, step, G.stream, (uint32_t)gr, G.st->size);
+  const float* rec = G.records + (size_t)idx * G.rec;
+  const int o = G.o, a = G.adim, used = 2 * o + a + 2;
+  for (int c = (int)threadIdx.x & 15; c < used; c += 16) {
+    const float v = rec[c];
+    if (c < o) G.s[(size_t)gr * o + c] = v;
+    else if (c < o + a) G.a[(size_t)gr * a + (c - o)] = v;
+    else if (c == o + a) G.r[gr] = v;
+    else if (c == o + a + 1) G.d[gr] = v;
+    else G.s2[(size_t)gr * o + (c - o - a - 2)] = v;
+  }
+}
 
 struct FwdTask {
   NetView net;
@@ -304,7 +319,9 @@
   const struct TailLite* tail;
   int tail_mode, tail_n;
   int l0_split;
-  int reserved_mt[7];
+  int reserved_mt[3];
+  const float* stg_r;
+  const float* stg_d;
   int ctab;
   int late;
 };
@@ -843,6 +860,7 @@
   const int bx = (int)blockIdx.x, cs = (int)blockIdx.z;
   const bool first_task = ty == 0;
   constexpr int FIN_CT = 0;
+  constexpr int ROWS_CT = 0;
 #define XCH_HOOK_STAGE
 #define XCH_HOOK_FIN
 #define XCH_STAMP(i) ILSX_STAMP(A.dbg, i)
@@ -1019,186 +1037,24 @@
 
 template <int H, int ACT, int CS, bool CT = false>
 __global__ __launch_bounds__(4 * H / CS) void k_sac_phase_a(const PhaseAArgs Pk, int slot) {
-  const PhaseAArgs& P = CT ? g_phase_a_tab[slot] : Pk;
-  constexpr int GRP = 0; constexpr bool XCH = true;
-  constexpr int PH = 0;
-  extern __shared__ __attribute__((aligned(16))) float smem[];
-  const FwdGroup* GP = nullptr;
-  const int bx = blockIdx.x, cs = blockIdx.z, y = blockIdx.y;
-  unsigned* tflag = P.flags + PHASE_TAIL_FLAG * 32;
-  if (y == 4) {
-    if (bx == 0 && cs == 0) {
-      const TailLite& TL = P.f1.tail[0];
-      tail_lite_run(TL, smem);
-      if (threadIdx.x == 0) {
-        __hip_atomic_store(&TL.scal->alpha, TL.scal->alpha, __ATOMIC_RELAXED, __HIP_MEMORY_SCOPE_AGENT);
-        asm volatile("s_waitcnt vmcnt(0)" ::: "memory");
-        __hip_atomic_store(tflag, 1u, __ATOMIC_RELAXED, __HIP_MEMORY_SCOPE_AGENT);
-      }
-    }
-    return;
-  }
-  if (bx * 16 >= P.f1.rows) return;
-  unsigned* f1 = P.flags + (3 * bx) * 32;
-  unsigned* f2 = P.flags + (3 * bx + 1) * 32;
-  unsigned* f0 = P.flags + (3 * bx + 2) * 32;
-  const bool own = y >= 5;
-  ILSX_STAMP(P.dbg, 0);
-#if defined(ILSX_STAMPS) && defined(ILSX_STAMPS_FINE)
-  if (P.dbg && threadIdx.x == 0 && (y == 1 || y == 2)) P.dbg[(size_t)ILSX_WG_LINEAR * ILSX_TRACE_SLOTS + 5] = clock64();
-#endif
-  xch_mark_xcd(P.flags + PHASE_MASK_WORD(bx));
-#if defined(ILSX_STAMPS) && !defined(ILSX_STAMPS_FINE)
-  if (P.dbg && threadIdx.x == 0 && ILSX_WG_LINEAR < ILSX_TRACE_MAXWG) P.dbg[(size_t)ILSX_WG_LINEAR * ILSX_TRACE_SLOTS + 7] = 0x10000u | cu_key();
-#endif
-  if (!own) {
-    {
-      const FwdArgs& A = P.f1;
-      const FwdTask& T = A.t[y];
-      const bool first_task = y == 0;
-      constexpr int FIN_CT = -1;
-#define XCH_HOOK_STAGE
-#define XCH_HOOK_FIN
-#define XCH_STAMP(i) ((void)0)
-#include "fwd_split_tile.inc"
-#undef XCH_STAMP
-#undef XCH_HOOK_STAGE
-#undef XCH_HOOK_FIN
-    }
-    ILSX_STAMP(P.dbg, 1);
-    if (y == 0) {
-      asm volatile("s_waitcnt vmcnt(0)" ::: "memory");
-      __syncthreads();
-      if (threadIdx.x == 0) {
-        __hip_atomic_fetch_add(f0, 1u, __ATOMIC_RELAXED, __HIP_MEMORY_SCOPE_AGENT);
-        __hip_atomic_fetch_add(f1, 1u, __ATOMIC_RELAXED, __HIP_MEMORY_SCOPE_AGENT);
-      }
-    } else {
-      xch_arrive(f1);
-    }
-    ILSX_STAMP(P.dbg, 2);
-    if (P.own_rows && (y == 0 || y == 3)) return;
-  }
-  if (y == 0 || y == 3 || own) {
-    {
-      const FwdArgs& A = P.f2;
-      const int tq = own ? y - 5 : (y == 0 ? 0 : 1);
-      const FwdTask& T = A.t[tq];
-      const bool first_task = tq == 0;
-      constexpr int FIN_CT = 1;
-#define XCH_HOOK_STAGE ILSX_STAMP_SYNC(P.dbg, 7); xch_wait(f0, CS, P.err); ILSX_STAMP(P.dbg, 3);
-#define XCH_HOOK_FIN
-#define XCH_FINE_DBG P.dbg
-#define XCH_STAMP(i) do { if (own) ILSX_STAMP(P.dbg, (i) == 3 ? 6 : (i)); } while (0)
-#include "fwd_split_tile.inc"
-#undef XCH_STAMP
-#undef XCH_FINE_DBG
-#undef XCH_HOOK_STAGE
-#undef XCH_HOOK_FIN
-    }
-    ILSX_STAMP(P.dbg, 4);
-    xch_arrive(f2);
-    ILSX_STAMP(P.dbg, 5);
-  } else {
-    xch_wait(f1, 4 * CS, P.err);
-    xch_wait(tflag, 1u, P.err);
-    if (P.fin_pi_on && y == 1 && cs == 0) {
-      policy_fin_tile(P.fin_pi, bx * 16, P.f1.rows, smem, 4 * H / CS);
-    }
-    {
-      const BwdArgs& A = P.b1;
-      const BwdTask& T = A.t[y - 1];
-      constexpr int LOSS_CT = LOSS_SAC_CRITIC, NO_CT = 1;
-#define XCH_HOOK_ACT
-#define XCH_HOOK_HEAD xch_wait(f2, 2 * CS, P.err); ILSX_STAMP(P.dbg, 3);
-#if defined(ILSX_STAMPS_FINE)
-#define XCH_STAMP(i) ((void)0)
-#else
-#define XCH_STAMP(i) do { if ((i) < 3) ILSX_STAMP(P.dbg, 4 + (i)); } while (0)
-#endif
-#include "bwd_split_tile.inc"
-#undef XCH_STAMP
-#undef XCH_HOOK_ACT
-#undef XCH_HOOK_HEAD
-    }
-    ILSX_STAMP(P.dbg, 4);
-#if defined(ILSX_STAMPS) && defined(ILSX_STAMPS_FINE)
-    if (P.dbg && threadIdx.x == 0) P.dbg[(size_t)ILSX_WG_LINEAR * ILSX_TRACE_SLOTS + 6] = clock64();
-#endif
-  }
+  constexpr int ROWS_A_CT = 1;
+#include "sac_phase_a_body.inc"
+}
+template <int H, int ACT, int CS, bool CT = false>
+__global__ __launch_bounds__(4 * H / CS) void k_sac_phase_a_late(const PhaseAArgs Pk, int slot) {
+  constexpr int ROWS_A_CT = 0;
+#include "sac_phase_a_body.inc"
 }
 
 template <int H, int ACT, int CS, bool CT = false>
 __global__ __launch_bounds__(4 * H / CS) void k_sac_phase_c(const PhaseCArgs Pk, int slot) {
-  const PhaseCArgs& P = CT ? g_phase_c_tab[slot] : Pk;
-  constexpr int GRP = 0; constexpr bool XCH = true;
-  constexpr int PH = 0;
-  extern __shared__ __attribute__((aligned(16))) float smem[];
-  const FwdGroup* GP = nullptr;
-  const int bx = blockIdx.x, cs = blockIdx.z, y = blockIdx.y;
-  if (y == 3) {
-    if (bx == 0 && cs == 0 && threadIdx.x == 0) P.f3.tail[0].scal->gather_step += 1;
-    if (P.aslot && bx == 1 && cs == 0) alpha_slot_run(P.aslot_logp, P.aslot_B, P.aslot_te, P.aslot_invB, P.aslot, smem);
-    const float tau = P.polyak_tau;
-    for (int i = ((int)(cs * gridDim.x + bx) * (int)blockDim.x + (int)threadIdx.x) * 4; i < P.polyak_n; i += (int)(gridDim.x * gridDim.z * blockDim.x) * 4) {
-      const float4 p = *reinterpret_cast<const float4*>(P.polyak_P + i);
-      float4 t = *reinterpret_cast<const float4*>(P.polyak_T + i);
-      t.x = t.x * (1.0f - tau) + p.x * tau; t.y = t.y * (1.0f - tau) + p.y * tau;
-      t.z = t.z * (1.0f - tau) + p.z * tau; t.w = t.w * (1.0f - tau) + p.w * tau;
-      *reinterpret_cast<float4*>(P.polyak_T + i) = t;
-    }
-    return;
-  }
-  if (bx * 16 >= P.f3.rows) return;
-  unsigned* f1 = P.flags + (3 * bx) * 32;
-  unsigned* f2 = P.flags + (3 * bx + 1) * 32;
-  ILSX_STAMP(P.dbg, 0);
-  xch_mark_xcd(P.flags + PHASE_MASK_WORD(bx));
-  if (y == 2) {
-    {
-      const BwdArgs& A = P.b3;
-      const BwdTask& T = A.t[0];
-      constexpr int LOSS_CT = LOSS_SAC_POLICY, NO_CT = 0;
-#define XCH_HOOK_ACT
-#define XCH_HOOK_HEAD xch_wait(f2, 2 * CS, P.err); ILSX_STAMP(P.dbg, 4);
-#define XCH_STAMP(i) ILSX_STAMP(P.dbg, i)
-#include "bwd_split_tile.inc"
-#undef XCH_STAMP
-#undef XCH_HOOK_ACT
-#undef XCH_HOOK_HEAD
-    }
-    ILSX_STAMP(P.dbg, 5);
-    return;
-  }
-  {
-    const FwdArgs& A = P.f3;
-    const FwdTask& T = A.t[y];
-    const bool first_task = y == 0;
-    constexpr int FIN_CT = -1;
-#define XCH_HOOK_STAGE
-#define XCH_HOOK_FIN
-#define XCH_STAMP(i) ((void)0)
-#include "fwd_split_tile.inc"
-#undef XCH_STAMP
-#undef XCH_HOOK_STAGE
-#undef XCH_HOOK_FIN
-  }
-  ILSX_STAMP(P.dbg, 1);
-  xch_arrive(f1);
-  {
-    const BwdArgs& A = P.b2;
-    const BwdTask& T = A.t[y];
-    constexpr int LOSS_CT = LOSS_SAC_ACTORQ, NO_CT = 1;
-#define XCH_HOOK_ACT xch_wait(f1, 2 * CS, P.err); ILSX_STAMP(P.dbg, 2);
-#define XCH_HOOK_HEAD
-#define XCH_STAMP(i) ILSX_STAMP(P.dbg, 3 + (i))
-#include "bwd_split_tile.inc"
-#undef XCH_STAMP
-#undef XCH_HOOK_ACT
-#undef XCH_HOOK_HEAD
-  }
-  ILSX_STAMP(P.dbg, 3);
-  xch_arrive(f2);
+  constexpr int ROWS_CT = 1;
+#include "sac_phase_c_body.inc"
+}
+template <int H, int ACT, int CS, bool CT = false>
+__global__ __launch_bounds__(4 * H / CS) void k_sac_phase_c_late(const PhaseCArgs Pk, int slot) {
+  constexpr int ROWS_CT = 0;
+#include "sac_phase_c_body.inc"
 }
 #endif
 
@@ -1232,8 +1088,9 @@
   const int* zero_err;
   int tile_nh, tile_kt;
   int reserved_strip;
-};
-static_assert(sizeof(DwArgs) == 1072 && offsetof(DwArgs, reserved_strip) == 1064, "DwArgs keeps the layout it had with the strip flag (reserved_strip)");
+  unsigned long long* bump_step;
+};
+static_assert(sizeof(DwArgs) == 1080 && offsetof(DwArgs, reserved_strip) == 1064, "DwArgs keeps the layout it had with the strip flag (reserved_strip)");
 struct DwTileG { DwMat J; AdamFuse F; };
 #define DW_SPLIT_MIN_ROWS 1024
 #define DW_BIG_MIN_ROWS 4096
@@ -1291,6 +1148,7 @@
   const int bx = blockIdx.x >> D.xs;
   if (D.zero_flags && bx == 0 && blockIdx.y == 0 && threadIdx.x < PHASE_NFLAGS)
     D.zero_flags[threadIdx.x * 32] = (D.zero_err && *D.zero_err) ? PHASE_FLAG_DEAD : 0u;
+  if (D.bump_step && bx == 0 && blockIdx.y == 0 && threadIdx.x == 0) *D.bump_step += 1;
   int mi = 0;
   if (!GRP) {
 #pragma unroll
diff --git a/ilswiss_amd/csrc/sac_phase_a_body.inc b/ilswiss_amd/csrc/sac_phase_a_body.inc
--- /dev/null
+++ b/ilswiss_amd/csrc/sac_phase_a_body.inc
@@ -0,0 +1,109 @@
+  const PhaseAArgs& P = CT ? g_phase_a_tab[slot] : Pk;
+  constexpr int GRP = 0; constexpr bool XCH = true;
+  constexpr int PH = 0;
+  extern __shared__ __attribute__((aligned(16))) float smem[];
+  const FwdGroup* GP = nullptr;
+  const int bx = blockIdx.x, cs = blockIdx.z, y = blockIdx.y;
+  unsigned* tflag = P.flags + PHASE_TAIL_FLAG * 32;
+  if (y == 4) {
+    if (bx == 0 && cs == 0) {
+      const TailLite& TL = P.f1.tail[0];
+      tail_lite_run(TL, smem);
+      if (threadIdx.x == 0) {
+        __hip_atomic_store(&TL.scal->alpha, TL.scal->alpha, __ATOMIC_RELAXED, __HIP_MEMORY_SCOPE_AGENT);
+        asm volatile("s_waitcnt vmcnt(0)" ::: "memory");
+        __hip_atomic_store(tflag, 1u, __ATOMIC_RELAXED, __HIP_MEMORY_SCOPE_AGENT);
+      }
+    }
+    return;
+  }
+  if (bx * 16 >= P.f1.rows) return;
+  unsigned* f1 = P.flags + (3 * bx) * 32;
+  unsigned* f2 = P.flags + (3 * bx + 1) * 32;
+  unsigned* f0 = P.flags + (3 * bx + 2) * 32;
+  const bool own = y >= 5;
+  ILSX_STAMP(P.dbg, 0);
+#if defined(ILSX_STAMPS) && defined(ILSX_STAMPS_FINE)
+  if (P.dbg && threadIdx.x == 0 && (y == 1 || y == 2)) P.dbg[(size_t)ILSX_WG_LINEAR * ILSX_TRACE_SLOTS + 5] = clock64();
+#endif
+  xch_mark_xcd(P.flags + PHASE_MASK_WORD(bx));
+#if defined(ILSX_STAMPS) && !defined(ILSX_STAMPS_FINE)
+  if (P.dbg && threadIdx.x == 0 && ILSX_WG_LINEAR < ILSX_TRACE_MAXWG) P.dbg[(size_t)ILSX_WG_LINEAR * ILSX_TRACE_SLOTS + 7] = 0x10000u | cu_key();
+#endif
+  if (!own) {
+    {
+      const FwdArgs& A = P.f1;
+      const FwdTask& T = A.t[y];
+      const bool first_task = y == 0;
+      constexpr int FIN_CT = -1;
+      constexpr int ROWS_CT = ROWS_A_CT;
+#define XCH_HOOK_STAGE
+#define XCH_HOOK_FIN
+#define XCH_STAMP(i) ((void)0)
+#include "fwd_split_tile.inc"
+#undef XCH_STAMP
+#undef XCH_HOOK_STAGE
+#undef XCH_HOOK_FIN
+    }
+    ILSX_STAMP(P.dbg, 1);
+    if (y == 0) {
+      asm volatile("s_waitcnt vmcnt(0)" ::: "memory");
+      __syncthreads();
+      if (threadIdx.x == 0) {
+        __hip_atomic_fetch_add(f0, 1u, __ATOMIC_RELAXED, __HIP_MEMORY_SCOPE_AGENT);
+        __hip_atomic_fetch_add(f1, 1u, __ATOMIC_RELAXED, __HIP_MEMORY_SCOPE_AGENT);
+      }
+    } else {
+      xch_arrive(f1);
+    }
+    ILSX_STAMP(P.dbg, 2);
+    if (P.own_rows && (y == 0 || y == 3)) return;
+  }
+  if (y == 0 || y == 3 || own) {
+    {
+      const FwdArgs& A = P.f2;
+      const int tq = own ? y - 5 : (y == 0 ? 0 : 1);
+      const FwdTask& T = A.t[tq];
+      const bool first_task = tq == 0;
+      constexpr int FIN_CT = 1;
+      constexpr int ROWS_CT = ROWS_A_CT ? 2 : 0;
+#define XCH_HOOK_STAGE ILSX_STAMP_SYNC(P.dbg, 7); xch_wait(f0, CS, P.err); ILSX_STAMP(P.dbg, 3);
+#define XCH_HOOK_FIN
+#define XCH_FINE_DBG P.dbg
+#define XCH_STAMP(i) do { if (own) ILSX_STAMP(P.dbg, (i) == 3 ? 6 : (i)); } while (0)
+#include "fwd_split_tile.inc"
+#undef XCH_STAMP
+#undef XCH_FINE_DBG
+#undef XCH_HOOK_STAGE
+#undef XCH_HOOK_FIN
+    }
+    ILSX_STAMP(P.dbg, 4);
+    xch_arrive(f2);
+    ILSX_STAMP(P.dbg, 5);
+  } else {
+    xch_wait(f1, 4 * CS, P.err);
+    xch_wait(tflag, 1u, P.err);
+    if (P.fin_pi_on && y == 1 && cs == 0) {
+      policy_fin_tile(P.fin_pi, bx * 16, P.f1.rows, smem, 4 * H / CS);
+    }
+    {
+      const BwdArgs& A = P.b1;
+      const BwdTask& T = A.t[y - 1];
+      constexpr int LOSS_CT = LOSS_SAC_CRITIC, NO_CT = 1;
+#define XCH_HOOK_ACT
+#define XCH_HOOK_HEAD xch_wait(f2, 2 * CS, P.err); ILSX_STAMP(P.dbg, 3);
+#if defined(ILSX_STAMPS_FINE)
+#define XCH_STAMP(i) ((void)0)
+#else
+#define XCH_STAMP(i) do { if ((i) < 3) ILSX_STAMP(P.dbg, 4 + (i)); } while (0)
+#endif
+#include "bwd_split_tile.inc"
+#undef XCH_STAMP
+#undef XCH_HOOK_ACT
+#undef XCH_HOOK_HEAD
+    }
+    ILSX_STAMP(P.dbg, 4);
+#if defined(ILSX_STAMPS) && defined(ILSX_STAMPS_FINE)
+    if (P.dbg && threadIdx.x == 0) P.dbg[(size_t)ILSX_WG_LINEAR * ILSX_TRACE_SLOTS + 6] = clock64();
+#endif
+  }
diff --git a/ilswiss_amd/csrc/sac_phase_c_body.inc b/ilswiss_amd/csrc/sac_phase_c_body.inc
--- /dev/null
+++ b/ilswiss_amd/csrc/sac_phase_c_body.inc
@@ -0,0 +1,71 @@
+  const PhaseCArgs& P = CT ? g_phase_c_tab[slot] : Pk;
+  constexpr int GRP = 0; constexpr bool XCH = true;
+  constexpr int PH = 0;
+  extern __shared__ __attribute__((aligned(16))) float smem[];
+  const FwdGroup* GP = nullptr;
+  const int bx = blockIdx.x, cs = blockIdx.z, y = blockIdx.y;
+  if (y == 3) {
+    if (ROWS_CT > 0 && P.f3.gather.on == 2) {
+      if (cs == 0 && bx * 16 < P.f3.rows) stage_rows_tile(P.f3.gather, P.f3.tail[0].scal->gather_step + 1, bx, P.f3.rows);
+    } else if (bx == 0 && cs == 0 && threadIdx.x == 0) P.f3.tail[0].scal->gather_step += 1;
+    if (P.aslot && bx == 1 && cs == 0) alpha_slot_run(P.aslot_logp, P.aslot_B, P.aslot_te, P.aslot_invB, P.aslot, smem);
+    const float tau = P.polyak_tau;
+    for (int i = ((int)(cs * gridDim.x + bx) * (int)blockDim.x + (int)threadIdx.x) * 4; i < P.polyak_n; i += (int)(gridDim.x * gridDim.z * blockDim.x) * 4) {
+      const float4 p = *reinterpret_cast<const float4*>(P.polyak_P + i);
+      float4 t = *reinterpret_cast<const float4*>(P.polyak_T + i);
+      t.x = t.x * (1.0f - tau) + p.x * tau; t.y = t.y * (1.0f - tau) + p.y * tau;
+      t.z = t.z * (1.0f - tau) + p.z * tau; t.w = t.w * (1.0f - tau) + p.w * tau;
+      *reinterpret_cast<float4*>(P.polyak_T + i) = t;
+    }
+    return;
+  }
+  if (bx * 16 >= P.f3.rows) return;
+  unsigned* f1 = P.flags + (3 * bx) * 32;
+  unsigned* f2 = P.flags + (3 * bx + 1) * 32;
+  ILSX_STAMP(P.dbg, 0);
+  xch_mark_xcd(P.flags + PHASE_MASK_WORD(bx));
+  if (y == 2) {
+    {
+      const BwdArgs& A = P.b3;
+      const BwdTask& T = A.t[0];
+      constexpr int LOSS_CT = LOSS_SAC_POLICY, NO_CT = 0;
+#define XCH_HOOK_ACT
+#define XCH_HOOK_HEAD xch_wait(f2, 2 * CS, P.err); ILSX_STAMP(P.dbg, 4);
+#define XCH_STAMP(i) ILSX_STAMP(P.dbg, i)
+#include "bwd_split_tile.inc"
+#undef XCH_STAMP
+#undef XCH_HOOK_ACT
+#undef XCH_HOOK_HEAD
+    }
+    ILSX_STAMP(P.dbg, 5);
+    return;
+  }
+  {
+    const FwdArgs& A = P.f3;
+    const FwdTask& T = A.t[y];
+    const bool first_task = y == 0;
+    constexpr int FIN_CT = -1;
+#define XCH_HOOK_STAGE
+#define XCH_HOOK_FIN
+#define XCH_STAMP(i) ((void)0)
+#include "fwd_split_tile.inc"
+#undef XCH_STAMP
+#undef XCH_HOOK_STAGE
+#undef XCH_HOOK_FIN
+  }
+  ILSX_STAMP(P.dbg, 1);
+  xch_arrive(f1);
+  {
+    const BwdArgs& A = P.b2;
+    const BwdTask& T = A.t[y];
+    constexpr int LOSS_CT = LOSS_SAC_ACTORQ, NO_CT = 1;
+#define XCH_HOOK_ACT xch_wait(f1, 2 * CS, P.err); ILSX_STAMP(P.dbg, 2);
+#define XCH_HOOK_HEAD
+#define XCH_STAMP(i) ILSX_STAMP(P.dbg, 3 + (i))
+#include "bwd_split_tile.inc"
+#undef XCH_STAMP
+#undef XCH_HOOK_ACT
+#undef XCH_HOOK_HEAD
+  }
+  ILSX_STAMP(P.dbg, 3);
+  xch_arrive(f2);
```

New measurement: 20510, median of 6. +2.1%, better.
